# anihcsam/OpenGaussian

Measured on AMD Instinct MI355X. Metric: fwd+bwd Mpix/s at 1080p, 1M Gaussians (RGB+6-D ins_feat); k-means it/s, higher is better.
Workload: dtype f32; 1 GPU; S1M-1080p RGB(SH3)+depth+alpha (all grads) + 6-ch ins_feat (grad to ins_feat) fwd+bwd, ONE fused 9-channel pass; gaussians=1000000, width=1920, height=1080, views_cycled=8, parallelism=single

## Files before the change

include/ogs_raster.h:

```cpp
#ifndef OGS_RASTER_H
#define OGS_RASTER_H

#include <stddef.h>
#include <stdint.h>

#ifdef __cplusplus
extern "C" {
#endif

#define OGS_OK 0
#define OGS_ERR_INVALID_ARG (-1)
#define OGS_ERR_HIP (-2)
#define OGS_ERR_UNSUPPORTED (-3)
#define OGS_ERR_SCRATCH_TOO_SMALL (-4)
#define OGS_ERR_DEVICE (-5)

#define OGS_TILE 16
#define OGS_MAX_CHANNELS 12

typedef struct OgsRasterFwdArgs {
    int32_t P;
    int32_t W, H;
    int32_t C;
    int32_t sh_degree;
    int32_t sh_coeffs;
    float tanfovx, tanfovy;
    float scale_modifier;
    int32_t prefiltered;
    int32_t debug;
    const float* bg;
    const float* means3D;
    const float* colors_precomp;
    const float* shs;
    const float* opacities;
    const float* scales;
    const float* rotations;
    const float* cov3D_precomp;
    const float* viewmatrix;
    const float* projmatrix;
    const float* campos;
    float* out_color;
    float* out_depth;
    float* out_alpha;
    int32_t* radii;
    void* geom_buffer;
    void* geom_tmp;
    void* image_buffer;
    uint32_t* point_list;
    void* binning_tmp;
    void* sorted_rec;
    void* quad_list;
    const int32_t* group_ids;
    int32_t num_groups;
    int32_t full_binning;
} OgsRasterFwdArgs;

typedef struct OgsRasterBwdArgs {
    int32_t P, W, H, C, sh_degree, sh_coeffs;
    float tanfovx, tanfovy, scale_modifier;
    int32_t debug;
    int32_t num_rendered;
    int32_t geom_channels;
    const float* bg;
    const float* means3D;
    const float* colors_precomp;
    const float* shs;
    const float* opacities;
    const float* scales;
    const float* rotations;
    const float* cov3D_precomp;
    const float* viewmatrix;
    const float* projmatrix;
    const float* campos;
    const int32_t* radii;
    const float* out_alpha;
    const float* dL_dcolor;
    const float* dL_ddepth;
    const float* dL_dalpha;
    const void* geom_buffer;
    const void* image_buffer;
    const uint32_t* point_list;
    const void* sorted_rec;
    const void* quad_list;
    void* bwd_tmp;
    float* dL_dmeans2D;
    float* dL_dcolors;
    float* dL_dopacity;
    float* dL_dmeans3D;
    float* dL_dcov3D;
    float* dL_dsh;
    float* dL_dscales;
    float* dL_drotations;
    int32_t num_groups;
    float* dL_dsh_rgb;
} OgsRasterBwdArgs;

int ogs_version(void);
const char* ogs_last_error(void);

int ogs_check_async_status(void);

size_t ogs_raster_geom_bytes(int32_t P, int32_t C);
size_t ogs_raster_geom_tmp_bytes(int32_t P);
size_t ogs_raster_image_bytes(int32_t W, int32_t H);
size_t ogs_raster_image_bytes_grouped(int32_t W, int32_t H, int32_t num_groups);
size_t ogs_raster_binning_tmp_bytes(int64_t num_rendered, int32_t W, int32_t H);
size_t ogs_raster_backward_tmp_bytes(int32_t P);
size_t ogs_raster_sorted_bytes(int64_t num_rendered, int32_t C);
size_t ogs_raster_quad_list_bytes(int64_t num_rendered);

int ogs_raster_forward_geometry(const OgsRasterFwdArgs* args, void* stream, int64_t* num_rendered_host);

int ogs_raster_forward_render(const OgsRasterFwdArgs* args, int64_t num_rendered, void* stream);

int ogs_raster_read_num_rendered_async(const OgsRasterFwdArgs* args, void* stream, uint32_t* host_pinned);
int ogs_raster_forward_render_deferred(const OgsRasterFwdArgs* args, int64_t capacity, void* stream);

size_t ogs_raster_tiny_max_points(void);
int ogs_raster_forward_tiny(const OgsRasterFwdArgs* args, void* stream);

size_t ogs_raster_tile_sort_capacity(int32_t level);

int ogs_raster_forward_reblend(const OgsRasterFwdArgs* args, void* stream);

int ogs_raster_compact_kept(int32_t W, int32_t H, int32_t C, const void* image_buffer, const void* sorted_rec,
                            const void* quad_list, void* new_image_buffer, void* new_sorted_rec, void* new_quad_list,
                            void* stream);

typedef struct OgsGroupStatsArgs {
    const int32_t* labels;
    int32_t num_labels;
    float alpha_threshold;
    float* max_alpha;
    int64_t* count;
    float* feat_sum;
    void* stats_tmp;
} OgsGroupStatsArgs;

size_t ogs_raster_stats_image_bytes(int32_t W, int32_t H, int32_t num_groups);
size_t ogs_raster_stats_tmp_bytes(int32_t num_groups, int32_t num_labels, int32_t C);
int ogs_raster_forward_group_stats(const OgsRasterFwdArgs* args, const OgsGroupStatsArgs* stats, int64_t num_rendered,
                                   void* stream);

int ogs_raster_backward(const OgsRasterBwdArgs* args, void* stream);

int ogs_mark_visible(int32_t P, const float* means3D, const float* viewmatrix, const float* projmatrix,
                     uint8_t* present, void* stream);

int ogs_sh_grad_from_views(int32_t P, int32_t V, int32_t sh_degree, int32_t sh_coeffs, const float* means3D,
                           const float* campos, const float* dL_drgb, float* dL_dsh, void* stream);

int ogs_raster_export_binning(const OgsRasterFwdArgs* args, int64_t num_rendered, uint64_t* keys_out,
                              uint32_t* ranges_out, uint32_t* n_contrib_out, void* stream);

int ogs_prof_enable(int on);
int ogs_prof_filter(const char* prefix);
int ogs_prof_collect(char* buf, size_t n);

int ogs_selftest_wave_fold16(const float* in, float* out, void* stream);
int ogs_selftest_tile_order(const uint32_t* ranges, int64_t vtiles, uint32_t* order, void* stream);
size_t ogs_selftest_radix_tmp_bytes(int64_t n);
int ogs_selftest_radix_sort(uint32_t* keys0, uint32_t* vals0, uint32_t* keys1, uint32_t* vals1, int64_t n, int32_t key_bits,
                            int32_t variant, int32_t items, const uint32_t* n_dev, void* tmp, int32_t* result_buffer,
                            void* stream);

#ifdef __cplusplus
}
#endif
#endif
```

opengaussian_amd/_lib.py:

```python
from __future__ import annotations

import ctypes as C
import os

_HERE = os.path.dirname(os.path.abspath(__file__))
LIB_PATH = os.environ.get("OGS_LIB_PATH") or os.path.join(_HERE, "lib", "libogs_hip.so")

_f32p = C.POINTER(C.c_float)
_vp = C.c_void_p


class OgsRasterFwdArgs(C.Structure):
    _fields_ = [
        ("P", C.c_int32), ("W", C.c_int32), ("H", C.c_int32), ("C", C.c_int32),
        ("sh_degree", C.c_int32), ("sh_coeffs", C.c_int32),
        ("tanfovx", C.c_float), ("tanfovy", C.c_float), ("scale_modifier", C.c_float),
        ("prefiltered", C.c_int32), ("debug", C.c_int32),
        ("bg", _vp), ("means3D", _vp), ("colors_precomp", _vp), ("shs", _vp), ("opacities", _vp),
        ("scales", _vp), ("rotations", _vp), ("cov3D_precomp", _vp),
        ("viewmatrix", _vp), ("projmatrix", _vp), ("campos", _vp),
        ("out_color", _vp), ("out_depth", _vp), ("out_alpha", _vp), ("radii", _vp),
        ("geom_buffer", _vp), ("geom_tmp", _vp), ("image_buffer", _vp), ("point_list", _vp),
        ("binning_tmp", _vp), ("sorted_rec", _vp), ("quad_list", _vp), ("group_ids", _vp), ("num_groups", C.c_int32),
        ("full_binning", C.c_int32),
    ]


class OgsRasterBwdArgs(C.Structure):
    _fields_ = [
        ("P", C.c_int32), ("W", C.c_int32), ("H", C.c_int32), ("C", C.c_int32),
        ("sh_degree", C.c_int32), ("sh_coeffs", C.c_int32),
        ("tanfovx", C.c_float), ("tanfovy", C.c_float), ("scale_modifier", C.c_float),
        ("debug", C.c_int32), ("num_rendered", C.c_int32), ("geom_channels", C.c_int32),
        ("bg", _vp), ("means3D", _vp), ("colors_precomp", _vp), ("shs", _vp), ("opacities", _vp),
        ("scales", _vp), ("rotations", _vp), ("cov3D_precomp", _vp),
        ("viewmatrix", _vp), ("projmatrix", _vp), ("campos", _vp),
        ("radii", _vp), ("out_alpha", _vp), ("dL_dcolor", _vp), ("dL_ddepth", _vp), ("dL_dalpha", _vp),
        ("geom_buffer", _vp), ("image_buffer", _vp), ("point_list", _vp), ("sorted_rec", _vp), ("quad_list", _vp), ("bwd_tmp", _vp),
        ("dL_dmeans2D", _vp), ("dL_dcolors", _vp), ("dL_dopacity", _vp), ("dL_dmeans3D", _vp),
        ("dL_dcov3D", _vp), ("dL_dsh", _vp), ("dL_dscales", _vp), ("dL_drotations", _vp), ("num_groups", C.c_int32), ("dL_dsh_rgb", _vp),
    ]


class OgsAdamTensor(C.Structure):
    _fields_ = [("param", _vp), ("grad", _vp), ("exp_avg", _vp), ("exp_avg_sq", _vp), ("numel", C.c_int64),
                ("lr", C.c_double), ("step", C.c_int64)]


class OgsRowTensor(C.Structure):
    _fields_ = [("src", _vp), ("dst", _vp), ("width", C.c_int32), ("zero_new", C.c_int32)]


class OgsDensifyArgs(C.Structure):
    _fields_ = [("N", C.c_int32), ("grad_accum", _vp), ("denom", _vp), ("scaling", _vp), ("opacity", _vp),
                ("max_grad", C.c_float), ("min_opacity", C.c_float), ("extent", C.c_float), ("percent_dense", C.c_float),
                ("prune_world_size", C.c_int32)]


class OgsGroupStatsArgs(C.Structure):
    _fields_ = [("labels", _vp), ("num_labels", C.c_int32), ("alpha_threshold", C.c_float), ("max_alpha", _vp),
                ("count", _vp), ("feat_sum", _vp), ("stats_tmp", _vp)]


SIGNATURES = {
    "ogs_version": (C.c_int, []),
    "ogs_last_error": (C.c_char_p, []),
    "ogs_raster_geom_bytes": (C.c_size_t, [C.c_int32, C.c_int32]),
    "ogs_raster_geom_tmp_bytes": (C.c_size_t, [C.c_int32]),
    "ogs_raster_image_bytes": (C.c_size_t, [C.c_int32, C.c_int32]),
    "ogs_raster_image_bytes_grouped": (C.c_size_t, [C.c_int32, C.c_int32, C.c_int32]),
    "ogs_raster_binning_tmp_bytes": (C.c_size_t, [C.c_int64, C.c_int32, C.c_int32]),
    "ogs_raster_backward_tmp_bytes": (C.c_size_t, [C.c_int32]),
    "ogs_raster_sorted_bytes": (C.c_size_t, [C.c_int64, C.c_int32]),
    "ogs_raster_quad_list_bytes": (C.c_size_t, [C.c_int64]),
    "ogs_raster_forward_geometry": (C.c_int, [C.POINTER(OgsRasterFwdArgs), _vp, C.POINTER(C.c_int64)]),
    "ogs_raster_forward_render": (C.c_int, [C.POINTER(OgsRasterFwdArgs), C.c_int64, _vp]),
    "ogs_raster_read_num_rendered_async": (C.c_int, [C.POINTER(OgsRasterFwdArgs), _vp, _vp]),
    "ogs_raster_forward_render_deferred": (C.c_int, [C.POINTER(OgsRasterFwdArgs), C.c_int64, _vp]),
    "ogs_raster_stats_image_bytes": (C.c_size_t, [C.c_int32, C.c_int32, C.c_int32]),
    "ogs_raster_stats_tmp_bytes": (C.c_size_t, [C.c_int32, C.c_int32, C.c_int32]),
    "ogs_raster_forward_group_stats": (C.c_int, [C.POINTER(OgsRasterFwdArgs), C.POINTER(OgsGroupStatsArgs), C.c_int64, _vp]),
    "ogs_raster_backward": (C.c_int, [C.POINTER(OgsRasterBwdArgs), _vp]),
    "ogs_raster_tiny_max_points": (C.c_size_t, []),
    "ogs_raster_tile_sort_capacity": (C.c_size_t, [C.c_int32]),
    "ogs_raster_forward_tiny": (C.c_int, [C.POINTER(OgsRasterFwdArgs), _vp]),
    "ogs_raster_forward_reblend": (C.c_int, [C.POINTER(OgsRasterFwdArgs), _vp]),
    "ogs_raster_compact_kept": (C.c_int, [C.c_int32, C.c_int32, C.c_int32, _vp, _vp, _vp, _vp, _vp, _vp, _vp]),
    "ogs_mark_visible": (C.c_int, [C.c_int32, _vp, _vp, _vp, _vp, _vp]),
    "ogs_sh_grad_from_views": (C.c_int, [C.c_int32, C.c_int32, C.c_int32, C.c_int32, _vp, _vp, _vp, _vp, _vp]),
    "ogs_raster_export_binning": (C.c_int, [C.POINTER(OgsRasterFwdArgs), C.c_int64, _vp, _vp, _vp, _vp]),
    "ogs_selftest_wave_fold16": (C.c_int, [_vp, _vp, _vp]),
    "ogs_selftest_tile_order": (C.c_int, [_vp, C.c_int64, _vp, _vp]),
    "ogs_selftest_radix_tmp_bytes": (C.c_size_t, [C.c_int64]),
    "ogs_selftest_radix_sort": (C.c_int, [_vp, _vp, _vp, _vp, C.c_int64, C.c_int32, C.c_int32, C.c_int32, _vp, _vp, _vp, _vp]),
    "ogs_check_async_status": (C.c_int, []),
    "ogs_prof_enable": (C.c_int, [C.c_int]),
    "ogs_prof_filter": (C.c_int, [C.c_char_p]),
    "ogs_prof_collect": (C.c_int, [C.c_char_p, C.c_size_t]),
    "ogs_kmeans_tmp_bytes": (C.c_size_t, [C.c_int64, C.c_int32, C.c_int32]),
    "ogs_kmeans_lloyd": (C.c_int, [_vp, C.c_int64, C.c_int32, _vp, C.c_int32, C.c_int32, C.c_int32, C.c_int32,
                                   _vp, C.c_int64, _vp, _vp]),
    "ogs_kmeans_assign": (C.c_int, [_vp, C.c_int64, C.c_int32, _vp, C.c_int32, _vp, C.c_int64, _vp]),
    "ogs_mask_feature_sums": (C.c_int, [_vp, _vp, _vp, C.c_int32, C.c_int32, C.c_int64, C.c_int32, _vp, _vp]),
    "ogs_mask_feature_sqdev": (C.c_int, [_vp, _vp, _vp, _vp, C.c_int32, C.c_int32, C.c_int64, _vp, _vp]),
    "ogs_mask_feature_sums_backward": (C.c_int, [_vp, _vp, _vp, _vp, _vp, C.c_int32, C.c_int32, C.c_int64, _vp, _vp, _vp]),
    "ogs_mask_cohesion": (C.c_int, [_vp, _vp, _vp, C.c_int32, C.c_int32, C.c_int64, _vp, _vp]),
    "ogs_mask_cohesion_backward": (C.c_int, [_vp, _vp, _vp, _vp, C.c_int32, C.c_int32, C.c_int64, _vp, _vp, _vp]),
    "ogs_label_feature_sums": (C.c_int, [_vp, _vp, _vp, C.c_int32, C.c_int32, C.c_int64, C.c_int32, _vp, _vp]),
    "ogs_label_feature_sqdev": (C.c_int, [_vp, _vp, _vp, _vp, C.c_int32, C.c_int32, C.c_int64, _vp, _vp]),
    "ogs_label_feature_sums_backward": (C.c_int, [_vp, _vp, _vp, _vp, _vp, C.c_int32, C.c_int32, C.c_int64, _vp, _vp, _vp]),
    "ogs_label_cohesion": (C.c_int, [_vp, _vp, _vp, C.c_int32, C.c_int32, C.c_int64, _vp, _vp]),
    "ogs_label_cohesion_backward": (C.c_int, [_vp, _vp, _vp, _vp, C.c_int32, C.c_int32, C.c_int64, _vp, _vp, _vp]),
    "ogs_separation_loss": (C.c_int, [_vp, C.c_int32, C.c_int32, C.c_int32, _vp, _vp, _vp, _vp]),
    "ogs_adam_step": (C.c_int, [C.POINTER(OgsAdamTensor), C.c_int32, C.c_double, C.c_double, C.c_double, _vp]),
    "ogs_rows_gather": (C.c_int, [C.POINTER(OgsRowTensor), C.c_int32, _vp, _vp, C.c_int64, _vp]),
    "ogs_densify_tmp_bytes": (C.c_size_t, [C.c_int32]),
    "ogs_densify_plan": (C.c_int, [C.POINTER(OgsDensifyArgs), _vp, C.POINTER(C.c_uint32), _vp]),
    "ogs_densify_map": (C.c_int, [C.c_int32, _vp, _vp, _vp, _vp, _vp]),
    "ogs_densify_split_children": (C.c_int, [C.c_int64, _vp, _vp, _vp, _vp, _vp, _vp, _vp, _vp, _vp, _vp]),
    "ogs_densify_stats": (C.c_int, [C.c_int32, _vp, C.c_int32, _vp, _vp, _vp, _vp, _vp, _vp]),
    "ogs_kmeans_accumulate": (C.c_int, [_vp, C.c_int64, C.c_int32, _vp, C.c_int32, C.c_int32, _vp, _vp, _vp]),
    "ogs_kmeans_update": (C.c_int, [_vp, C.c_int32, C.c_int32, C.c_int32, _vp, _vp, _vp]),
    "ogs_kmeans_gather": (C.c_int, [_vp, _vp, C.c_int64, C.c_int32, C.c_int32, _vp, _vp]),
    "ogs_refine_wave_table_capacity": (C.c_size_t, []),
    "ogs_refine_wave_max_pixels": (C.c_size_t, []),
    "ogs_refine_block_scratch_words": (C.c_size_t, [C.c_int32]),
    "ogs_refine_visibility": (C.c_int, [C.c_int32, _vp, _vp, _vp, _vp, C.c_int32, C.c_int32, C.c_float, C.c_float, _vp,
                                        C.c_float, C.c_float, _vp, _vp]),
    "ogs_refine_footprint_labels": (C.c_int, [C.c_int32, _vp, _vp, C.c_int32, C.c_int32, C.c_int32, _vp, C.c_int32, _vp, _vp,
                                              _vp]),
    "ogs_refine_footprint_labels_block": (C.c_int, [C.c_int32, _vp, _vp, C.c_int32, C.c_int32, C.c_int32, _vp, C.c_int32, _vp,
                                                    _vp, _vp, _vp]),
    "ogs_refine_vote": (C.c_int, [C.c_int64, C.c_int32, _vp, _vp, _vp]),
    "ogs_refine_expand": (C.c_int, [C.c_int32, _vp, _vp, _vp, _vp, C.c_int32, C.c_int32, C.c_int32, _vp, C.c_int32, _vp, _vp,
                                    C.c_int32, _vp]),
    "ogs_refine_finalize": (C.c_int, [C.c_int64, C.c_int32, _vp, _vp, _vp, C.c_int32, C.c_float, _vp, _vp]),
    "ogs_loss_photometric_tmp_bytes": (C.c_size_t, [C.c_int32, C.c_int32, C.c_int32]),
    "ogs_loss_photometric_forward": (C.c_int, [_vp, _vp, C.c_int32, C.c_int32, C.c_int32, C.c_float, _vp, _vp, _vp]),
    "ogs_loss_photometric_backward": (C.c_int, [_vp, _vp, _vp, _vp, _vp, C.c_float, C.c_int32, C.c_int32, C.c_int32, _vp,
                                                _vp]),
    "ogs_loss_masked_tmp_bytes": (C.c_size_t, []),
    "ogs_loss_masked_forward": (C.c_int, [_vp, _vp, _vp, _vp, C.c_int32, C.c_int32, C.c_int32, C.c_int64, _vp, _vp, _vp]),
    "ogs_loss_masked_backward": (C.c_int, [_vp, _vp, _vp, _vp, C.c_int32, C.c_int32, C.c_int32, C.c_int64, _vp, _vp, _vp,
                                           _vp]),
    "ogs_knn_tile_points": (C.c_size_t, []),
    "ogs_knn_group_ksum": (C.c_int, [C.c_int64, _vp, C.c_int32, _vp, _vp, _vp, _vp, _vp, _vp]),
}

_lib = None


class OgsError(RuntimeError):
    pass


def lib() -> C.CDLL:
    global _lib
    if _lib is None:
        if not os.path.exists(LIB_PATH):
            raise OgsError(f"{LIB_PATH} not found -- build it with `python -m opengaussian_amd.build` "
                           "(the product path has no CPU fallback)")
        l = C.CDLL(LIB_PATH)
        for name, (res, args) in SIGNATURES.items():
            fn = getattr(l, name)
            fn.restype = res
            fn.argtypes = args
        _lib = l
    return _lib


def check(rc: int, what: str):
    if rc != 0:
        raise OgsError(f"{what} failed (code {rc}): {lib().ogs_last_error().decode()}")


def prof_filter(prefix: str):
    check(lib().ogs_prof_filter(prefix.encode()), "ogs_prof_filter")


def prof_enable(mode):
    check(lib().ogs_prof_enable(int(mode)), "ogs_prof_enable")


def prof_collect() -> dict:
    import json
    buf = C.create_string_buffer(1 << 16)
    check(lib().ogs_prof_collect(buf, len(buf)), "ogs_prof_collect")
    return json.loads(buf.value.decode())


def ptr(t):
    return None if t is None else t.data_ptr()
```

opengaussian_amd/csrc/blend_fwd.hip:

```cpp
#include "ogs_common.h"

namespace ogs {

namespace {

constexpr float kAlphaMin = 1.0f / 255.0f;
typedef float v2f __attribute__((ext_vector_type(2)));

__device__ __forceinline__ uint64_t shfl_up_u64(uint64_t v, int d) {
    const uint32_t lo = __shfl_up((uint32_t)v, d, kWave), hi = __shfl_up((uint32_t)(v >> 32), d, kWave);
    return ((uint64_t)hi << 32) | lo;
}


template <int C>
struct RowRec {
    static constexpr int NV4 = stream_vec4(C);
    float4 v[NV4];
    __device__ __forceinline__ void load_lds(const float4* __restrict__ p) {
#pragma unroll
        for (int k = 0; k < NV4; ++k) v[k] = p[k];
    }
    __device__ __forceinline__ float at(int i) const {
        const float4 q = v[i >> 2];
        return (i & 3) == 0 ? q.x : (i & 3) == 1 ? q.y : (i & 3) == 2 ? q.z : q.w;
    }
    __device__ __forceinline__ float feat(int c) const { return at(8 + c); }
};

constexpr int kRowSlots = 65;
constexpr int kRowListLen = 72;
template <int C>
struct RowsLds {
    float4 s_rec[kBlock / kWave][kRowSlots * stream_vec4(C)];
    uint32_t s_list[kBlock / kWave][4][kRowListLen];
};

template <int C, int RF = -1>
__device__ __forceinline__ void blend_rows_tile(
    const uint2 range, int n, int n_kept, const float* __restrict__ stream,
    const uint32_t* __restrict__ quad_list, int W, int H, int gx, int img, int timg, const float* __restrict__ bg, float* __restrict__ out_color,
    float* __restrict__ out_depth, float* __restrict__ out_alpha, uint32_t* __restrict__ n_contrib,
    float* __restrict__ final_T, int pf_lines, RowsLds<C>& lds, const float* __restrict__ feats = nullptr) {
    constexpr int NV4 = stream_vec4(C);
    constexpr int RS = NV4 * 4;
    constexpr int kListLen = kRowListLen;
    auto& s_rec = lds.s_rec;
    auto& s_list = lds.s_list;
    const int tx = timg % gx, ty = timg / gx;
    const int tid = threadIdx.x, lane = tid & 63, wave = __builtin_amdgcn_readfirstlane(tid >> 6);
    const int row = lane >> 4, l16 = lane & 15;
    const int qx0 = tx * kTile + (wave & 1) * 8, qy0 = ty * kTile + (wave >> 1) * 8;
    const int px = qx0 + 4 * (row & 1) + (l16 & 3);
    const int py = qy0 + 4 * (row >> 1) + (l16 >> 2);
    const bool inside = px < W && py < H;
    const float fy = (float)py;

    const int n_tile = (int)(range.y - range.x);
    const float* __restrict__ tb = stream + (size_t)range.x * RS;
    const uint32_t* __restrict__ qi = quad_list + ((size_t)range.x * 5 + (size_t)wave * n_tile);
    const uint32_t lim = n_kept > 0 ? (uint32_t)n_kept - 1u : 0u;
    RecordPrefetch pf;
    pf.issue(tb, n_kept, RS, tid, pf_lines);

    float4* __restrict__ recs = s_rec[wave];
    uint32_t* __restrict__ mylist = s_list[wave][row];
    if (lane == 0) {
#pragma unroll
        for (int k = 0; k < NV4; ++k) recs[64 * NV4 + k] = float4{0.f, 0.f, 0.f, 0.f};
        recs[64 * NV4 + 1] = float4{0.f, -1.f, 0.f, 0.f};
    }
    float fxe = inside ? (float)px : kFar;
    float T = 1.0f;
    constexpr int NPF = (C + 2) / 2;
    v2f accp[NPF];
#pragma unroll
    for (int k = 0; k < NPF; ++k) accp[k] = (v2f){0.f, 0.f};
    float wacc = 0.f;
    uint32_t last = 0;
    bool all_done = false;

    constexpr uint32_t kNoEntry = 0xFFFFFFFFu;
    uint32_t last_e = kNoEntry;
    auto consume = [&](const RowRec<C>& rec, uint32_t entry) {
        const v2f d = (v2f){rec.at(0), rec.at(1)} - (v2f){fxe, fy};
        const v2f m = (v2f){rec.at(2), rec.at(3)} * d;
        const float u = fmaf(rec.at(4), d.y, m.x);
        const float power = fmaf(m.y, d.y, u * d.x);
        const float h = rec.at(5);
        const bool cand = fabsf(power + h) <= h;
        if (__ballot(cand) != 0ull) {
            const float araw = fminf(0.99f, rec.at(6) * __expf(power));
            const bool act = cand && araw >= kAlphaMin;
            const float alpha = act ? araw : 0.f;
            const float test_T = T * (1.0f - alpha);
            const bool stop = test_T < 0.0001f;
            const float w = stop ? 0.f : alpha * T;
            const v2f w2 = {w, w};
#pragma unroll
            for (int k = 0; k < NPF; ++k)
                accp[k] = __builtin_elementwise_fma((v2f){rec.feat(2 * k), rec.feat(2 * k + 1)}, w2, accp[k]);
            wacc += w;
            T = stop ? T : test_T;
            last_e = (act && !stop) ? entry : last_e;
            fxe = stop ? kFar : fxe;
            if (__ballot(stop) != 0ull) all_done = __ballot(fxe < kFarTest) == 0ull;
        }
    };

    const float bx0 = (float)(qx0 + 4 * 0), by0 = (float)qy0;
    for (int c0 = 0; c0 < n && !all_done; c0 += kWave) {
        const int cnt = min(kWave, n - c0);
        const bool have = lane < cnt;
        const uint32_t ridx = have ? min(qi[c0 + lane], lim) : 0u;
        const float4* __restrict__ rp = reinterpret_cast<const float4*>(tb + (size_t)ridx * RS);
        float4 r[NV4];
#pragma unroll
        for (int k = 0; k < NV4; ++k) r[k] = rp[k];
        if constexpr (RF >= 0) {
            constexpr int E = C - RF;
            const float* __restrict__ fp = feats + (size_t)__float_as_uint(r[1].w) * E;
            float fv[E];
#pragma unroll
            for (int k = 0; k < E; ++k) fv[k] = fp[k];
            float* rf = reinterpret_cast<float*>(r);
#pragma unroll
            for (int k = 0; k < E; ++k) rf[8 + RF + k] = fv[k];
        }
#pragma unroll
        for (int k = 0; k < NV4; ++k) recs[lane * NV4 + k] = r[k];
        bool reach[4];
        {
            const float gxp = r[0].x, gyp = r[0].y;
            const float A = -2.f * r[0].z, B = -r[1].x, Cc = -2.f * r[0].w, thr = -2.f * r[1].y;
            const float nbA = -B / A, nbC = -B / Cc;
#pragma unroll
            for (int b = 0; b < 4; ++b) {
                const float ox = bx0 + 4.f * (float)(b & 1), oy = by0 + 4.f * (float)(b >> 1);
                const float m = max_power_in_box(A, B, Cc, nbA, nbC, gxp - ox - 3.f, gxp - ox, gyp - oy - 3.f, gyp - oy);
                reach[b] = have && m >= thr;
            }
        }
        constexpr uint32_t kDummy = (64u << 16) | (64u * NV4 * 16u);
#pragma unroll
        for (int b = 0; b < 4; ++b) s_list[wave][b][lane] = kDummy;
        if (lane < kListLen - kWave) {
#pragma unroll
            for (int b = 0; b < 4; ++b) s_list[wave][b][kWave + lane] = kDummy;
        }
        int maxlen = 0;
#pragma unroll
        for (int b = 0; b < 4; ++b) {
            const uint64_t mask = __ballot(reach[b]);
            const int pos = (int)__builtin_amdgcn_mbcnt_hi((uint32_t)(mask >> 32), __builtin_amdgcn_mbcnt_lo((uint32_t)mask, 0u));
            if (reach[b]) s_list[wave][b][pos] = ((uint32_t)lane << 16) | ((uint32_t)lane * NV4 * 16u);
            maxlen = max(maxlen, (int)__popcll(mask));
        }
        __builtin_amdgcn_fence(__ATOMIC_RELEASE, "wavefront");
        __builtin_amdgcn_wave_barrier();
        RowRec<C> ra, rb;
        auto rec_of = [&](uint32_t e) {
            return reinterpret_cast<const float4*>(reinterpret_cast<const char*>(recs) + (e & 0xFFFFu));
        };
        uint32_t e0 = mylist[0], e1 = mylist[1];
        ra.load_lds(rec_of(e0));
        for (int t = 0; t < maxlen && !all_done; t += 2) {
            const uint32_t e2 = mylist[t + 2], e3 = mylist[t + 3];
            rb.load_lds(rec_of(e1));
            consume(ra, e0);
            ra.load_lds(rec_of(e2));
            if (t + 1 < maxlen) consume(rb, e1);
            e0 = e2; e1 = e3;
        }
        if (last_e != kNoEntry) last = (uint32_t)c0 + (last_e >> 16) + 1u;
        last_e = kNoEntry;
        __builtin_amdgcn_wave_barrier();
    }

    if (inside) {
        const size_t plane = (size_t)W * H;
        const size_t pix = (size_t)img * plane + (size_t)py * W + px;
        float* oc = out_color + (size_t)img * (C - 1) * plane;
#pragma unroll
        for (int c = 0; c < C; ++c) oc[c * plane + pix] = ((c & 1) ? accp[c / 2].y : accp[c / 2].x) + T * bg[c];
        out_depth[pix] = (C & 1) ? accp[C / 2].y : accp[C / 2].x;
        out_alpha[pix] = wacc;
        n_contrib[pix] = last;
        final_T[pix] = T;
    }
    pf.retire(n_contrib, W);
}

template <int C, int RF = -1>
__global__ __launch_bounds__(kBlock) void blend_forward_rows_kernel(
    const uint2* __restrict__ ranges, const uint32_t* __restrict__ qcount, const float* __restrict__ stream,
    const uint32_t* __restrict__ quad_list, int W, int H, int gx, int tiles, const float* __restrict__ bg, float* __restrict__ out_color,
    float* __restrict__ out_depth, float* __restrict__ out_alpha, uint32_t* __restrict__ n_contrib,
    float* __restrict__ final_T, int pf_lines, const uint32_t* __restrict__ tile_order, const float* __restrict__ feats) {
    __shared__ RowsLds<C> lds;
    const int tile = tile_order ? (int)tile_order[blockIdx.x] : (int)blockIdx.x;
    const int img = tile / tiles, timg = tile - img * tiles;
    const int wave = __builtin_amdgcn_readfirstlane((int)threadIdx.x >> 6);
    blend_rows_tile<C, RF>(ranges[tile], (int)qcount[tile * 5 + wave], (int)qcount[tile * 5 + 4], stream, quad_list, W, H, gx, img, timg,
                           bg, out_color, out_depth, out_alpha, n_contrib, final_T, pf_lines, lds, feats);
}

template <int C>
struct ChunkLds {
    static constexpr int SV = stream_vec4(C);
    uint64_t wave_tot[kBlock / kWave];
    uint32_t done[kBlock / kWave];
    float4 s_rec[(kBlock + 1) * SV];
    uint32_t s_list[kBlock / kWave][4][kRowListLen];
    uint8_t s_qnew[4][kBlock];
};

struct GroupStatsOut {
    const int32_t* labels;
    int32_t L;
    float thr;
    uint32_t* max_alpha;
    unsigned long long* count;
    unsigned long long* fsum;
};

constexpr float kFixedScale = 4294967296.0f;

__device__ __forceinline__ unsigned long long shfl_xor_u64(unsigned long long v, int m) {
    const uint32_t lo = __shfl_xor((uint32_t)v, m, kWave), hi = __shfl_xor((uint32_t)(v >> 32), m, kWave);
    return ((unsigned long long)hi << 32) | lo;
}

template <int C>
__device__ __forceinline__ void group_stats_epilogue(const GroupStatsOut& st, float* __restrict__ s_buf, int img, int W, int pix,
                                                     float alpha, const float (&colour)[C]) {
    float* s_val = s_buf;
    float* s_alpha = s_buf + C * kBlock;
    int* s_key = reinterpret_cast<int*>(s_buf + (C + 1) * kBlock);
    const int tid = threadIdx.x, lane = tid & 63;
    int key = -1;
    if (pix >= 0 && alpha > st.thr) {
        const int l = st.labels[pix];
        key = (l >= 0 && l < st.L) ? l : st.L;
    }
    s_key[tid] = key;
    s_alpha[tid] = pix >= 0 ? alpha : 0.f;
#pragma unroll
    for (int c = 0; c < C; ++c) s_val[c * kBlock + tid] = colour[c];
    lds_barrier();
    if (tid >= kWave) return;
    int k[kBlock / kWave];
    float m = 0.f;
#pragma unroll
    for (int j = 0; j < kBlock / kWave; ++j) {
        k[j] = s_key[lane + kWave * j];
        m = fmaxf(m, s_alpha[lane + kWave * j]);
    }
#pragma unroll
    for (int off = kWave / 2; off > 0; off >>= 1) m = fmaxf(m, __shfl_xor(m, off, kWave));
    if (lane == 0 && m > 0.f) atomicMax(st.max_alpha + img, __float_as_uint(m));
    const size_t row0 = (size_t)img * (size_t)(st.L + 1);
    for (;;) {
        int cand = -1;
#pragma unroll
        for (int j = kBlock / kWave - 1; j >= 0; --j) cand = k[j] >= 0 ? k[j] : cand;
        const uint64_t pending = __ballot(cand >= 0);
        if (pending == 0ull) break;
        const int K = __shfl(cand, __ffsll((unsigned long long)pending) - 1, kWave);
        unsigned long long cnt = 0, sum[C];
#pragma unroll
        for (int c = 0; c < C; ++c) sum[c] = 0ull;
#pragma unroll
        for (int j = 0; j < kBlock / kWave; ++j) {
            if (k[j] == K) {
                ++cnt;
#pragma unroll
                for (int c = 0; c < C; ++c) sum[c] += (unsigned long long)__float2ll_rn(s_val[c * kBlock + lane + kWave * j] * kFixedScale);
                k[j] = -1;
            }
        }
#pragma unroll
        for (int off = kWave / 2; off > 0; off >>= 1) {
            cnt += (unsigned long long)__shfl_xor((uint32_t)cnt, off, kWave);
#pragma unroll
            for (int c = 0; c < C; ++c) sum[c] += shfl_xor_u64(sum[c], off);
        }
        if (lane == 0) {
            const size_t r = row0 + (size_t)K;
            atomicAdd(st.count + r, cnt);
#pragma unroll
            for (int c = 0; c < C; ++c) atomicAdd(st.fsum + r * C + c, sum[c]);
        }
    }
}

__global__ __launch_bounds__(256) void group_stats_finish_kernel(const long long* __restrict__ fsum, float* __restrict__ out, size_t n) {
    const size_t i = (size_t)blockIdx.x * 256 + threadIdx.x;
    if (i < n) out[i] = (float)((double)fsum[i] * (1.0 / 4294967296.0));
}

template <int C, bool STATS = false>
__global__ __launch_bounds__(kBlock) __attribute__((amdgpu_waves_per_eu(6, 8)))
void pack_blend_chunked_kernel(
    const uint2* __restrict__ ranges, const uint32_t* __restrict__ point_list, const float4* __restrict__ rec,
    float4* __restrict__ stream, uint32_t* __restrict__ quad_list, uint32_t* __restrict__ qcount, int W, int H, int gx, int tiles,
    const float* __restrict__ bg, float* __restrict__ out_color, float* __restrict__ out_depth, float* __restrict__ out_alpha,
    uint32_t* __restrict__ n_contrib, float* __restrict__ final_T, const uint32_t* __restrict__ tile_order,
    GroupStatsOut st = GroupStatsOut{}) {
    constexpr int NV = rec_vec4(C);
    constexpr int SV = stream_vec4(C);
    constexpr int kListLen = kRowListLen;
    __shared__ ChunkLds<C> lds;
    const int tile = tile_order ? (int)tile_order[blockIdx.x] : (int)blockIdx.x;
    const int img = tile / tiles, timg = tile - img * tiles;
    const uint2 range = ranges[tile];
    const int n = (int)(range.y - range.x);
    const int tx = timg % gx, ty = timg / gx;
    const int tid = threadIdx.x, lane = tid & 63, wave = __builtin_amdgcn_readfirstlane(tid >> 6);
    const float X0 = (float)(tx * kTile), Y0 = (float)(ty * kTile);
    const int row = lane >> 4, l16 = lane & 15;
    const int qx0 = tx * kTile + (wave & 1) * 8, qy0 = ty * kTile + (wave >> 1) * 8;
    const int px = qx0 + 4 * (row & 1) + (l16 & 3);
    const int py = qy0 + 4 * (row >> 1) + (l16 >> 2);
    const bool inside = px < W && py < H;
    const float fy = (float)py;
    float fxe = inside ? (float)px : kFar;
    float T = 1.0f;
    constexpr int NPF = (C + 2) / 2;
    v2f accp[NPF];
#pragma unroll
    for (int k = 0; k < NPF; ++k) accp[k] = (v2f){0.f, 0.f};
    float wacc = 0.f;
    uint32_t last = 0;
    uint64_t alive = __ballot(inside);

    const float4* __restrict__ recs = lds.s_rec;
    uint32_t* __restrict__ mylist = lds.s_list[wave][row];
    if (tid == 0) {
#pragma unroll
        for (int k = 0; k < SV; ++k) lds.s_rec[kBlock * SV + k] = float4{0.f, 0.f, 0.f, 0.f};
        lds.s_rec[kBlock * SV + 1] = float4{0.f, -1.f, 0.f, 0.f};
    }

    constexpr uint32_t kNoEntry = 0xFFFFFFFFu;
    uint32_t last_e = kNoEntry;
    auto consume = [&](const RowRec<C>& r, uint32_t entry) {
        const v2f d = (v2f){r.at(0), r.at(1)} - (v2f){fxe, fy};
        const v2f m = (v2f){r.at(2), r.at(3)} * d;
        const float u = fmaf(r.at(4), d.y, m.x);
        const float power = fmaf(m.y, d.y, u * d.x);
        const float h = r.at(5);
        const bool cand = fabsf(power + h) <= h;
        if (__ballot(cand) != 0ull) {
            const float araw = fminf(0.99f, r.at(6) * __expf(power));
            const bool act = cand && araw >= kAlphaMin;
            const float alpha = act ? araw : 0.f;
            const float test_T = T * (1.0f - alpha);
            const bool stop = test_T < 0.0001f;
            float w = alpha * T;
            bool contributes = act;
            if (__ballot(stop) != 0ull) {
                w = stop ? 0.f : w;
                T = stop ? T : test_T;
                fxe = stop ? kFar : fxe;
                alive = __ballot(fxe < kFarTest);
                contributes = act && !stop;
            } else {
                T = test_T;
            }
            const v2f w2 = {w, w};
#pragma unroll
            for (int k = 0; k < NPF; ++k)
                accp[k] = __builtin_elementwise_fma((v2f){r.feat(2 * k), r.feat(2 * k + 1)}, w2, accp[k]);
            wacc += w;
            last_e = contributes ? entry : last_e;
        }
    };

    uint32_t running[5];
#pragma unroll
    for (int q = 0; q < 5; ++q) running[q] = 0u;
    const float bx0 = (float)qx0, by0 = (float)qy0;

    for (int base = 0; base < n; base += kBlock) {
        const int i = base + tid;
        uint32_t mask = 0;
        float4 a = make_float4(0, 0, 0, 0), b = a;
        float h = 0.f;
        uint32_t gid_of_thread = 0;
        const uint32_t sv = i < n ? point_list[range.x + i] : 0u;
        if (sv >> kReachBit) {
            const uint32_t gid = sv & kGidMask;
            gid_of_thread = gid;
            const float4* src = rec + (size_t)gid * NV;
            a = src[0]; b = src[1];
            h = 0.5f * (__logf(255.0f * b.w) + kThrMargin);
            const float thr = -2.0f * h;
            const float nbA = -b.y / b.x, nbC = -b.y / b.z;
#pragma unroll
            for (int q = 0; q < 4; ++q) {
                const float qx = X0 + (float)((q & 1) * 8), qy = Y0 + (float)((q >> 1) * 8);
                const float m = max_power_in_box(b.x, b.y, b.z, nbA, nbC, a.x - qx - 7.f, a.x - qx, a.y - qy - 7.f, a.y - qy);
                if (m >= thr) mask |= 1u << q;
            }
        }
        const uint64_t mine = (uint64_t)(mask & 1u) | ((uint64_t)((mask >> 1) & 1u) << 12) |
                              ((uint64_t)((mask >> 2) & 1u) << 24) | ((uint64_t)((mask >> 3) & 1u) << 36) |
                              ((uint64_t)(mask != 0u ? 1u : 0u) << 48);
        uint64_t inc = mine;
#pragma unroll
        for (int d = 1; d < kWave; d <<= 1) {
            const uint64_t t = shfl_up_u64(inc, d);
            if (lane >= d) inc += t;
        }
        if (lane == kWave - 1) lds.wave_tot[wave] = inc;
        lds_barrier();
        uint64_t before = 0, total = 0;
#pragma unroll
        for (int w = 0; w < kBlock / kWave; ++w) {
            const uint64_t t = lds.wave_tot[w];
            if (w < wave) before += t;
            total += t;
        }
        const uint64_t pos = before + inc - mine;
        if (mask) {
            const uint32_t c_loc = (uint32_t)(pos >> 48) & 0xFFFu;
            const uint32_t c_idx = running[4] + c_loc;
            float4* dst = lds.s_rec + c_loc * SV;
            dst[0] = make_float4(a.x, a.y, -0.5f * b.x, -0.5f * b.z);
            dst[1] = make_float4(-b.y, h, b.w, __uint_as_float(gid_of_thread));
            const float4* src = rec + (size_t)gid_of_thread * NV;
            float f[(SV - 2) * 4];
#pragma unroll
            for (int k = 0; k < (SV - 2) * 4; ++k) f[k] = 0.f;
#pragma unroll
            for (int v = 0; v < NV - 2; ++v) {
                const float4 t = src[2 + v];
                f[4 * v] = t.x; f[4 * v + 1] = t.y; f[4 * v + 2] = t.z; f[4 * v + 3] = t.w;
            }
            f[C] = a.z;
#pragma unroll
            for (int v = 0; v < SV - 2; ++v) dst[2 + v] = make_float4(f[4 * v], f[4 * v + 1], f[4 * v + 2], f[4 * v + 3]);
#pragma unroll
            for (int q = 0; q < 4; ++q) {
                if (mask & (1u << q)) {
                    const uint32_t pq = (uint32_t)(pos >> (12 * q)) & 0xFFFu;
                    if constexpr (!STATS) quad_list[(size_t)range.x * 5 + (size_t)q * n + running[q] + pq] = c_idx;
                    lds.s_qnew[q][pq] = (uint8_t)c_loc;
                }
            }
            if constexpr (!STATS) quad_list[(size_t)range.x * 5 + (size_t)4 * n + c_idx] = (uint32_t)i;
        }
        lds_barrier();
        if constexpr (!STATS) {
            const int kept4 = (int)((uint32_t)(total >> 48) & 0xFFFu) * SV;
            float4* __restrict__ out = stream + ((size_t)range.x + (size_t)running[4]) * SV;
            for (int e = tid; e < kept4; e += kBlock) out[e] = lds.s_rec[e];
        }
        const int cnt_q = (int)((uint32_t)(total >> (12 * wave)) & 0xFFFu);
        const uint32_t j0 = wave == 0 ? running[0] : wave == 1 ? running[1] : wave == 2 ? running[2] : running[3];
        for (int c0 = 0; c0 < cnt_q && alive != 0ull; c0 += kWave) {
            const int cnt = min(kWave, cnt_q - c0);
            const bool have = lane < cnt;
            const uint32_t cl = have ? (uint32_t)lds.s_qnew[wave][c0 + lane] : (uint32_t)kBlock;
            const float4 r0 = recs[cl * SV], r1 = recs[cl * SV + 1];
            bool reach[4];
            {
                const float gxp = r0.x, gyp = r0.y;
                const float A = -2.f * r0.z, B = -r1.x, Cc = -2.f * r0.w, thr = -2.f * r1.y;
                const float nbA = -B / A, nbC = -B / Cc;
#pragma unroll
                for (int bb = 0; bb < 4; ++bb) {
                    const float ox = bx0 + 4.f * (float)(bb & 1), oy = by0 + 4.f * (float)(bb >> 1);
                    const float m = max_power_in_box(A, B, Cc, nbA, nbC, gxp - ox - 3.f, gxp - ox, gyp - oy - 3.f, gyp - oy);
                    reach[bb] = have && m >= thr;
                }
            }
            constexpr uint32_t kDummy = (64u << 16) | ((uint32_t)kBlock * SV * 16u);
#pragma unroll
            for (int bb = 0; bb < 4; ++bb) lds.s_list[wave][bb][lane] = kDummy;
            if (lane < kListLen - kWave) {
#pragma unroll
                for (int bb = 0; bb < 4; ++bb) lds.s_list[wave][bb][kWave + lane] = kDummy;
            }
            int maxlen = 0;
#pragma unroll
            for (int bb = 0; bb < 4; ++bb) {
                const uint64_t m64 = __ballot(reach[bb]);
                const int p = (int)__builtin_amdgcn_mbcnt_hi((uint32_t)(m64 >> 32), __builtin_amdgcn_mbcnt_lo((uint32_t)m64, 0u));
                if (reach[bb]) lds.s_list[wave][bb][p] = ((uint32_t)lane << 16) | (cl * SV * 16u);
                maxlen = max(maxlen, (int)__popcll(m64));
            }
            __builtin_amdgcn_fence(__ATOMIC_RELEASE, "wavefront");
            __builtin_amdgcn_wave_barrier();
            RowRec<C> ra, rb;
            auto rec_of = [&](uint32_t e) {
                return reinterpret_cast<const float4*>(reinterpret_cast<const char*>(recs) + (e & 0xFFFFu));
            };
            uint32_t e0 = mylist[0], e1 = mylist[1];
            ra.load_lds(rec_of(e0));
            const uint32_t jbase = j0 + (uint32_t)c0 + 1u;
            for (int t = 0; t < maxlen && alive != 0ull; t += 2) {
                const uint32_t e2 = mylist[t + 2], e3 = mylist[t + 3];
                rb.load_lds(rec_of(e1));
                consume(ra, e0);
                ra.load_lds(rec_of(e2));
                if (t + 1 < maxlen) consume(rb, e1);
                e0 = e2; e1 = e3;
            }
            if (last_e != kNoEntry) last = jbase + (last_e >> 16);
            last_e = kNoEntry;
            __builtin_amdgcn_wave_barrier();
        }
#pragma unroll
        for (int q = 0; q < 5; ++q) running[q] += (uint32_t)(total >> (12 * q)) & 0xFFFu;
        if (lane == 0) lds.done[wave] = alive == 0ull ? 1u : 0u;
        lds_barrier();
        if ((lds.done[0] & lds.done[1] & lds.done[2] & lds.done[3]) != 0u) break;
    }
    if constexpr (STATS) {
        float colour[C];
#pragma unroll
        for (int c = 0; c < C; ++c) colour[c] = ((c & 1) ? accp[c / 2].y : accp[c / 2].x) + T * bg[c];
        group_stats_epilogue<C>(st, reinterpret_cast<float*>(lds.s_rec), img, W, inside ? py * W + px : -1, wacc, colour);
    } else {
        if (tid == 0) {
#pragma unroll
            for (int q = 0; q < 5; ++q) qcount[tile * 5 + q] = running[q];
        }
        if (inside) {
            const size_t plane = (size_t)W * H;
            const size_t pix = (size_t)img * plane + (size_t)py * W + px;
            float* oc = out_color + (size_t)img * (C - 1) * plane;
#pragma unroll
            for (int c = 0; c < C; ++c) oc[c * plane + pix] = ((c & 1) ? accp[c / 2].y : accp[c / 2].x) + T * bg[c];
            out_depth[pix] = (C & 1) ? accp[C / 2].y : accp[C / 2].x;
            out_alpha[pix] = wacc;
            n_contrib[pix] = last;
            final_T[pix] = T;
        }
    }
}

template <int C>
__global__ __launch_bounds__(kBlock) void export_n_contrib_kernel(const uint2* __restrict__ ranges,
                                                                  const uint32_t* __restrict__ point_list,
                                                                  const uint32_t* __restrict__ quad_list, int W, int H,
                                                                  int gx, int tiles, const uint32_t* __restrict__ n_contrib,
                                                                  uint32_t* __restrict__ out) {
    const int tile = blockIdx.x;
    const int img = tile / tiles, timg = tile - img * tiles;
    const int tx = timg % gx, ty = timg / gx;
    const int tid = threadIdx.x, lane = tid & 63, wave = tid >> 6;
    const int px = tx * kTile + (wave & 1) * 8 + (lane & 7);
    const int py = ty * kTile + (wave >> 1) * 8 + (lane >> 3);
    if (px >= W || py >= H) return;
    const uint2 range = ranges[tile];
    const int n_tile = (int)(range.y - range.x);
    n_contrib += (size_t)img * W * H;
    out += (size_t)img * W * H;
    const uint32_t last = n_contrib[(size_t)py * W + px];
    uint32_t res = 0;
    if (last > 0) {
        const uint32_t c_idx = quad_list[(size_t)range.x * 5 + (size_t)wave * n_tile + (last - 1)];
        res = quad_list[(size_t)range.x * 5 + (size_t)4 * n_tile + c_idx] + 1u;
    }
    out[(size_t)py * W + px] = res;
}

template <int C>
__global__ __launch_bounds__(kBlock) void tiny_blend_kernel(int P, const uint32_t* __restrict__ order,
                                                            const float4* __restrict__ rec, int W, int H, int gx,
                                                            const float* __restrict__ bg, float* __restrict__ out_color,
                                                            float* __restrict__ out_depth, float* __restrict__ out_alpha) {
    constexpr int NV = rec_vec4(C);
    constexpr int RS = 8 + (C + 1 + 3) / 4 * 4;
    static_assert(kTinyMaxP == kBlock, "one staging round");
    __shared__ float s_rec[kTinyMaxP * RS];
    __shared__ uint32_t s_wave_cnt[kBlock / kWave];
    const int tile = blockIdx.x;
    const int tx = tile % gx, ty = tile / gx;
    const int tid = threadIdx.x, lane = tid & 63, wave = tid >> 6;
    const int gy = (H + kTile - 1) / kTile;

    bool keep = false;
    float4 a = make_float4(0, 0, 0, 0), b = a;
    uint32_t gid = 0;
    if (tid < P) {
        gid = order[tid];
        const float4* src = rec + (size_t)gid * NV;
        a = src[0]; b = src[1];
        const int radius = __float_as_int(a.w);
        if (radius > 0) {
            const float rf = (float)radius;
            auto tr = [](float v) -> int {
                if (!(fabsf(v) < 3.0e38f)) v = 0.f;
                v = fminf(fmaxf(v, -2.0e9f), 2.0e9f);
                return (int)v;
            };
            const int rminx = min(gx, max(0, tr((a.x - rf) / (float)kTile)));
            const int rminy = min(gy, max(0, tr((a.y - rf) / (float)kTile)));
            const int rmaxx = min(gx, max(0, tr((a.x + rf + (float)kTile - 1.0f) / (float)kTile)));
            const int rmaxy = min(gy, max(0, tr((a.y + rf + (float)kTile - 1.0f) / (float)kTile)));
            keep = tx >= rminx && tx < rmaxx && ty >= rminy && ty < rmaxy;
        }
    }
    const uint64_t bal = __ballot(keep);
    if (lane == 0) s_wave_cnt[wave] = (uint32_t)__popcll(bal);
    __syncthreads();
    uint32_t before = 0, n = 0;
#pragma unroll
    for (int w = 0; w < kBlock / kWave; ++w) {
        const uint32_t c = s_wave_cnt[w];
        if (w < wave) before += c;
        n += c;
    }
    if (keep) {
        const uint32_t pos = before + (uint32_t)__popcll(bal & ((1ull << lane) - 1ull));
        float* dst = s_rec + pos * RS;
        dst[0] = a.x; dst[1] = a.y; dst[2] = -0.5f * b.x; dst[3] = -b.y; dst[4] = -0.5f * b.z;
        dst[5] = 0.5f * (__logf(255.0f * b.w) + kThrMargin);
        dst[6] = b.w; dst[7] = __uint_as_float(gid);
        const float4* src = rec + (size_t)gid * NV;
        float f[(NV - 2) * 4 + 4];
#pragma unroll
        for (int v = 0; v < NV - 2; ++v) {
            const float4 t = src[2 + v];
            f[4 * v] = t.x; f[4 * v + 1] = t.y; f[4 * v + 2] = t.z; f[4 * v + 3] = t.w;
        }
#pragma unroll
        for (int c = 0; c < C; ++c) dst[8 + c] = f[c];
        dst[8 + C] = a.z;
    }
    __syncthreads();

    const int px = tx * kTile + (wave & 1) * 8 + (lane & 7);
    const int py = ty * kTile + (wave >> 1) * 8 + (lane >> 3);
    const bool inside = px < W && py < H;
    const float fx = (float)px, fy = (float)py;
    float T = 1.0f, wacc = 0.f;
    float acc[C + 1];
#pragma unroll
    for (int c = 0; c <= C; ++c) acc[c] = 0.f;
    bool done = !inside;
    for (uint32_t j = 0; j < n; ++j) {
        if (__ballot(!done) == 0ull) break;
        const float* r = s_rec + j * RS;
        const float dx = r[0] - fx, dy = r[1] - fy;
        const float power = blend_power(r[2], r[3], r[4], dx, dy);
        const bool cand = !done && fabsf(power + r[5]) <= r[5];
        if (cand) {
            float alpha = fminf(0.99f, r[6] * __expf(power));
            alpha = alpha >= kAlphaMin ? alpha : 0.f;
            const float test_T = T * (1.0f - alpha);
            const bool stop = test_T < 0.0001f;
            const float w = stop ? 0.f : alpha * T;
#pragma unroll
            for (int c = 0; c <= C; ++c) acc[c] = fmaf(r[8 + c], w, acc[c]);
            wacc += w;
            T = stop ? T : test_T;
            done = stop;
        }
    }
    if (inside) {
        const size_t plane = (size_t)W * H;
        const size_t pix = (size_t)py * W + px;
#pragma unroll
        for (int c = 0; c < C; ++c) out_color[c * plane + pix] = acc[c] + T * bg[c];
        out_depth[pix] = acc[C];
        out_alpha[pix] = wacc;
    }
}

template <int C>
int tiny_c(const OgsRasterFwdArgs& a, const GeomState& gs, const uint32_t* order, hipStream_t s) {
    const int gx = (a.W + kTile - 1) / kTile, gy = (a.H + kTile - 1) / kTile;
    OGS_LAUNCH(tiny_blend_kernel<C>, dim3((unsigned)(gx * gy)), dim3(kBlock), 0, s, a.P, order, (const float4*)gs.rec, a.W, a.H,
               gx, a.bg, a.out_color, a.out_depth, a.out_alpha);
    OGS_LAUNCH_CHECK(a.debug, s);
    return OGS_OK;
}


constexpr int kOrderThreads = 1024;
constexpr int64_t kOrderMaxTiles = 1 << 16;
__device__ __forceinline__ uint32_t work_class(uint32_t n) {
    if (n < 8u) return 255u - n;
    const uint32_t e = 31u - (uint32_t)__builtin_clz(n);
    const uint32_t v = e * 8u + ((n >> (e - 3u)) & 7u);
    return 255u - min(v, 255u);
}
__device__ __forceinline__ uint32_t class_counter_add(uint32_t* bins, uint32_t cls, bool valid, int lane) {
    uint32_t pos = 0u;
    uint64_t todo = __ballot(valid);
    while (todo != 0ull) {
        const int leader = __ffsll((unsigned long long)todo) - 1;
        const uint32_t c0 = (uint32_t)__shfl((int)cls, leader, kWave);
        const uint64_t same = __ballot(valid && cls == c0) & todo;
        uint32_t base = 0u;
        if (lane == leader) base = atomicAdd(&bins[c0], (uint32_t)__popcll(same));
        base = (uint32_t)__shfl((int)base, leader, kWave);
        if ((same >> lane) & 1ull) pos = base + (uint32_t)__popcll(same & ((1ull << lane) - 1ull));
        todo &= ~same;
    }
    return pos;
}
__global__ __launch_bounds__(kOrderThreads) void tile_order_kernel(const uint2* __restrict__ ranges, uint32_t vtiles,
                                                                   uint32_t* __restrict__ order) {
    __shared__ uint32_t bins[256];
    __shared__ uint32_t wave_max[kOrderThreads / kWave], wave_sum[kOrderThreads / kWave];
    const uint32_t tid = threadIdx.x;
    uint32_t my_max = 0u, my_sum = 0u;
    for (uint32_t t0 = 0; t0 < vtiles; t0 += 8u * kOrderThreads) {
        uint2 r[8];
#pragma unroll
        for (int k = 0; k < 8; ++k) {
            const uint32_t t = t0 + (uint32_t)k * kOrderThreads + tid;
            r[k] = t < vtiles ? ranges[t] : make_uint2(0u, 0u);
        }
#pragma unroll
        for (int k = 0; k < 8; ++k) { my_max = max(my_max, r[k].y - r[k].x); my_sum += r[k].y - r[k].x; }
    }
#pragma unroll
    for (int d = 32; d >= 1; d >>= 1) {
        my_max = max(my_max, (uint32_t)__shfl_xor((int)my_max, d, kWave));
        my_sum += (uint32_t)__shfl_xor((int)my_sum, d, kWave);
    }
    if ((tid & 63u) == 0u) { wave_max[tid >> 6] = my_max; wave_sum[tid >> 6] = my_sum; }
    if (tid < 256u) bins[tid] = 0u;
    __syncthreads();
    uint32_t longest = 0u;
    unsigned long long total = 0ull;
#pragma unroll
    for (int w = 0; w < kOrderThreads / kWave; ++w) { longest = max(longest, wave_max[w]); total += wave_sum[w]; }
    if ((unsigned long long)longest * vtiles <= 2ull * total) {
        for (uint32_t t = tid; t < vtiles; t += kOrderThreads) order[t] = t;
        return;
    }
    for (uint32_t t0 = 0; t0 < vtiles; t0 += kOrderThreads) {
        const uint32_t t = t0 + tid;
        const bool valid = t < vtiles;
        const uint2 r = valid ? ranges[t] : make_uint2(0u, 0u);
        (void)class_counter_add(bins, work_class(r.y - r.x), valid, (int)(tid & 63u));
    }
    __syncthreads();
    if (tid < 64u) {
        uint32_t c[4], sum = 0u;
#pragma unroll
        for (int k = 0; k < 4; ++k) { c[k] = bins[tid * 4u + k]; sum += c[k]; }
        uint32_t incl = sum;
#pragma unroll
        for (int d = 1; d < 64; d <<= 1) {
            const uint32_t o = __shfl_up(incl, d, kWave);
            if ((int)tid >= d) incl += o;
        }
        uint32_t base = incl - sum;
#pragma unroll
        for (int k = 0; k < 4; ++k) { bins[tid * 4u + k] = base; base += c[k]; }
    }
    __syncthreads();
    for (uint32_t t0 = 0; t0 < vtiles; t0 += kOrderThreads) {
        const uint32_t t = t0 + tid;
        const bool valid = t < vtiles;
        const uint2 r = valid ? ranges[t] : make_uint2(0u, 0u);
        const uint32_t pos = class_counter_add(bins, work_class(r.y - r.x), valid, (int)(tid & 63u));
        if (valid) order[pos] = t;
    }
}

template <int C>
int launch_c(const OgsRasterFwdArgs& a, const GeomState& gs, const ImageState& is, int64_t D, hipStream_t s, bool order_ready) {
    const int gx = (a.W + kTile - 1) / kTile, gy = (a.H + kTile - 1) / kTile;
    const int tiles = gx * gy;
    const unsigned vtiles = (unsigned)tiles * (unsigned)num_groups_of(a.num_groups);
    if (D > 0) {
        const uint32_t* order = order_ready ? tile_order_of(is, vtiles, a.P) : launch_tile_order(is, vtiles, a.P, s, a.debug);
        static constexpr const char* const kChunked[4] = {"pack_blend_chunked_kernel<3>", "pack_blend_chunked_kernel<6>",
                                                          "pack_blend_chunked_kernel<9>", "pack_blend_chunked_kernel<12>"};
        OGS_LAUNCH_NAMED(chan_name<C>(kChunked), pack_blend_chunked_kernel<C>, dim3(vtiles), dim3(kBlock), 0, s,
                         (const uint2*)is.ranges, (const uint32_t*)a.point_list, (const float4*)gs.rec, stream_base<C>(a.sorted_rec),
                         quad_base(a.quad_list), is.qcount, a.W, a.H, gx, tiles, a.bg, a.out_color, a.out_depth, a.out_alpha,
                         is.n_contrib, is.final_T, order);
        OGS_LAUNCH_CHECK(a.debug, s);
        return OGS_OK;
    }
    OGS_HIP_CHECK(hipMemsetAsync(is.qcount, 0, (size_t)vtiles * 5 * sizeof(uint32_t), s));
    static constexpr const char* const kRows[4] = {"blend_forward_rows_kernel<3>", "blend_forward_rows_kernel<6>",
                                                   "blend_forward_rows_kernel<9>", "blend_forward_rows_kernel<12>"};
    OGS_LAUNCH_NAMED(chan_name<C>(kRows), blend_forward_rows_kernel<C>, dim3(vtiles), dim3(kBlock), 0, s,
                     (const uint2*)is.ranges, (const uint32_t*)is.qcount, (const float*)stream_base<C>(a.sorted_rec),
                     (const uint32_t*)quad_base(a.quad_list), a.W, a.H, gx, tiles, a.bg, a.out_color, a.out_depth,
                     a.out_alpha, is.n_contrib, is.final_T, blend_prefetch_lines(), (const uint32_t*)nullptr, (const float*)nullptr);
    OGS_LAUNCH_CHECK(a.debug, s);
    return OGS_OK;
}

template <int C>
int stats_c(const OgsRasterFwdArgs& a, const OgsGroupStatsArgs& sa, const GeomState& gs, const ImageState& is, hipStream_t s,
            bool order_ready) {
    const int gx = (a.W + kTile - 1) / kTile, gy = (a.H + kTile - 1) / kTile;
    const int tiles = gx * gy;
    const int G = num_groups_of(a.num_groups);
    const unsigned vtiles = (unsigned)tiles * (unsigned)G;
    const size_t rows = (size_t)G * (size_t)(sa.num_labels + 1);
    long long* fixed = static_cast<long long*>(sa.stats_tmp);
    OGS_HIP_CHECK(hipMemsetAsync(sa.max_alpha, 0, (size_t)G * sizeof(float), s));
    OGS_HIP_CHECK(hipMemsetAsync(sa.count, 0, rows * sizeof(int64_t), s));
    OGS_HIP_CHECK(hipMemsetAsync(fixed, 0, rows * C * sizeof(long long), s));
    const uint32_t* order = order_ready ? tile_order_of(is, vtiles, a.P) : launch_tile_order(is, vtiles, a.P, s, a.debug);
    GroupStatsOut st;
    st.labels = sa.labels;
    st.L = sa.num_labels;
    st.thr = sa.alpha_threshold;
    st.max_alpha = reinterpret_cast<uint32_t*>(sa.max_alpha);
    st.count = reinterpret_cast<unsigned long long*>(sa.count);
    st.fsum = reinterpret_cast<unsigned long long*>(fixed);
    static constexpr const char* const kStats[4] = {"pack_blend_chunked_kernel<3, stats>", "pack_blend_chunked_kernel<6, stats>",
                                                    "pack_blend_chunked_kernel<9, stats>", "pack_blend_chunked_kernel<12, stats>"};
    OGS_LAUNCH_NAMED(chan_name<C>(kStats), (pack_blend_chunked_kernel<C, true>), dim3(vtiles), dim3(kBlock), 0, s,
                     (const uint2*)is.ranges, (const uint32_t*)a.point_list, (const float4*)gs.rec, (float4*)nullptr,
                     (uint32_t*)nullptr, (uint32_t*)nullptr, a.W, a.H, gx, tiles, a.bg, (float*)nullptr, (float*)nullptr,
                     (float*)nullptr, (uint32_t*)nullptr, (float*)nullptr, order, st);
    OGS_LAUNCH_CHECK(a.debug, s);
    const size_t n = rows * C;
    OGS_LAUNCH(group_stats_finish_kernel, dim3((unsigned)((n + 255) / 256)), dim3(256), 0, s, (const long long*)fixed,
               sa.feat_sum, n);
    OGS_LAUNCH_CHECK(a.debug, s);
    return OGS_OK;
}

template <int C>
int reblend_c(const OgsRasterFwdArgs& a, const ImageState& is, hipStream_t s) {
    const int gx = (a.W + kTile - 1) / kTile, gy = (a.H + kTile - 1) / kTile;
    const int tiles = gx * gy;
    const unsigned vtiles = (unsigned)tiles;
    const uint32_t* order = tile_order_of(is, vtiles, a.P);
    static constexpr const char* const kRows[4] = {"blend_forward_rows_kernel<3, refresh>", "blend_forward_rows_kernel<6, refresh>",
                                                   "blend_forward_rows_kernel<9, refresh>", "blend_forward_rows_kernel<12, refresh>"};
    const float* stream = reinterpret_cast<const float*>(stream_base<C>(a.sorted_rec));
#define OGS_REBLEND(RFV)                                                                                                    \
    OGS_LAUNCH_NAMED(chan_name<C>(kRows), (blend_forward_rows_kernel<C, RFV>), dim3(vtiles), dim3(kBlock), 0, s,           \
                     (const uint2*)is.ranges, (const uint32_t*)is.qcount, stream, (const uint32_t*)quad_base(a.quad_list), a.W,  \
                     a.H, gx, tiles, a.bg, a.out_color, a.out_depth, a.out_alpha, is.n_contrib, is.final_T,                  \
                     blend_prefetch_lines(), order, a.colors_precomp)
    if (a.sh_coeffs != 0) {
        if constexpr (C > 3) {
            OGS_REBLEND(3);
        } else {
            set_error("forward_reblend: a 3-channel SH pass has no channel to replace");
            return OGS_ERR_INVALID_ARG;
        }
    } else {
        OGS_REBLEND(0);
    }
#undef OGS_REBLEND
    OGS_LAUNCH_CHECK(a.debug, s);
    return OGS_OK;
}

template <int C>
__global__ __launch_bounds__(kBlock) void compact_kept_kernel(const uint2* __restrict__ old_ranges, const uint2* __restrict__ new_ranges,
                                                              const uint32_t* __restrict__ qcount, const float4* __restrict__ old_rec,
                                                              const uint32_t* __restrict__ old_quad, float4* __restrict__ new_rec,
                                                              uint32_t* __restrict__ new_quad) {
    constexpr int SV = stream_vec4(C);
    const int tile = blockIdx.x;
    const uint2 ro = old_ranges[tile], rn = new_ranges[tile];
    const uint32_t n_old = ro.y - ro.x, k = qcount[tile * 5 + 4];
    const float4* __restrict__ src = old_rec + (size_t)ro.x * SV;
    float4* __restrict__ dst = new_rec + (size_t)rn.x * SV;
    for (uint32_t e = threadIdx.x; e < k * SV; e += kBlock) dst[e] = src[e];
#pragma unroll
    for (int q = 0; q < 4; ++q) {
        const uint32_t nq = qcount[tile * 5 + q];
        const uint32_t* __restrict__ qs = old_quad + ((size_t)ro.x * 5 + (size_t)q * n_old);
        uint32_t* __restrict__ qd = new_quad + ((size_t)rn.x * 5 + (size_t)q * k);
        for (uint32_t e = threadIdx.x; e < nq; e += kBlock) qd[e] = qs[e];
    }
}

template <int C>
int compact_c(int W, int H, const ImageState& is_old, const ImageState& is_new, const void* old_rec, const void* old_quad,
              void* new_rec, void* new_quad, hipStream_t s) {
    const int gx = (W + kTile - 1) / kTile, gy = (H + kTile - 1) / kTile;
    OGS_LAUNCH(compact_kept_kernel<C>, dim3((unsigned)(gx * gy)), dim3(kBlock), 0, s, (const uint2*)is_old.ranges,
               (const uint2*)is_new.ranges, (const uint32_t*)is_old.qcount, (const float4*)stream_base<C>(const_cast<void*>(old_rec)),
               (const uint32_t*)quad_base(const_cast<void*>(old_quad)), stream_base<C>(new_rec), quad_base(new_quad));
    OGS_LAUNCH_CHECK(0, s);
    return OGS_OK;
}

template <int C>
int export_c(const OgsRasterFwdArgs& a, const ImageState& is, uint32_t* out, hipStream_t s) {
    const int gx = (a.W + kTile - 1) / kTile, gy = (a.H + kTile - 1) / kTile;
    OGS_LAUNCH(export_n_contrib_kernel<C>, dim3((unsigned)(gx * gy) * (unsigned)num_groups_of(a.num_groups)), dim3(kBlock), 0,
               s, (const uint2*)is.ranges, (const uint32_t*)a.point_list, (const uint32_t*)quad_base(a.quad_list), a.W,
               a.H, gx, gx * gy, (const uint32_t*)is.n_contrib, out);
    OGS_LAUNCH_CHECK(0, s);
    return OGS_OK;
}

}

static bool tile_order_enabled() {
    static const bool v = [] { const char* e = getenv("OGS_TILE_ORDER"); return !(e && atoi(e) == 0); }();
    return v;
}
const uint32_t* tile_order_of(const ImageState& is, int64_t vtiles, int P) {
    return (tile_order_enabled() && vtiles > 1 && vtiles <= kOrderMaxTiles && (int64_t)P >= 4 * vtiles) ? is.tile_order : nullptr;
}
const uint32_t* launch_tile_order(const ImageState& is, int64_t vtiles, int P, hipStream_t s, int debug) {
    const uint32_t* order = tile_order_of(is, vtiles, P);
    if (!order) return nullptr;
    OGS_LAUNCH(tile_order_kernel, dim3(1), dim3(kOrderThreads), 0, s, (const uint2*)is.ranges, (uint32_t)vtiles, is.tile_order);
    if (debug) (void)hipStreamSynchronize(s);
    return order;
}

int launch_tile_order_test(const uint32_t* ranges, int64_t vtiles, uint32_t* order, hipStream_t s) {
    if (vtiles > kOrderMaxTiles) { set_error("selftest: more than %lld tiles", (long long)kOrderMaxTiles); return OGS_ERR_UNSUPPORTED; }
    OGS_LAUNCH(tile_order_kernel, dim3(1), dim3(kOrderThreads), 0, s, (const uint2*)ranges, (uint32_t)vtiles, order);
    OGS_LAUNCH_CHECK(1, s);
    return OGS_OK;
}

int launch_blend_forward(const OgsRasterFwdArgs& a, const GeomState& gs, const ImageState& is, int64_t D,
                         hipStream_t s, bool order_ready) {
    switch (a.C) {
        case 3: return launch_c<3>(a, gs, is, D, s, order_ready);
        case 6: return launch_c<6>(a, gs, is, D, s, order_ready);
        case 9: return launch_c<9>(a, gs, is, D, s, order_ready);
        case 12: return launch_c<12>(a, gs, is, D, s, order_ready);
        default: set_error("unsupported channel count C=%d", a.C); return OGS_ERR_UNSUPPORTED;
    }
}

int launch_group_stats(const OgsRasterFwdArgs& a, const OgsGroupStatsArgs& st, const GeomState& gs, const ImageState& is,
                       hipStream_t s, bool order_ready) {
    switch (a.C) {
        case 3: return stats_c<3>(a, st, gs, is, s, order_ready);
        case 6: return stats_c<6>(a, st, gs, is, s, order_ready);
        case 9: return stats_c<9>(a, st, gs, is, s, order_ready);
        case 12: return stats_c<12>(a, st, gs, is, s, order_ready);
        default: set_error("unsupported channel count C=%d", a.C); return OGS_ERR_UNSUPPORTED;
    }
}

int launch_compact_kept(int W, int H, int C, const ImageState& is_old, const ImageState& is_new, const void* old_rec,
                        const void* old_quad, void* new_rec, void* new_quad, hipStream_t s) {
    switch (C) {
        case 3: return compact_c<3>(W, H, is_old, is_new, old_rec, old_quad, new_rec, new_quad, s);
        case 6: return compact_c<6>(W, H, is_old, is_new, old_rec, old_quad, new_rec, new_quad, s);
        case 9: return compact_c<9>(W, H, is_old, is_new, old_rec, old_quad, new_rec, new_quad, s);
        case 12: return compact_c<12>(W, H, is_old, is_new, old_rec, old_quad, new_rec, new_quad, s);
        default: set_error("unsupported channel count C=%d", C); return OGS_ERR_UNSUPPORTED;
    }
}

int launch_reblend(const OgsRasterFwdArgs& a, const ImageState& is, hipStream_t s) {
    switch (a.C) {
        case 3: return reblend_c<3>(a, is, s);
        case 6: return reblend_c<6>(a, is, s);
        case 9: return reblend_c<9>(a, is, s);
        case 12: return reblend_c<12>(a, is, s);
        default: set_error("unsupported channel count C=%d", a.C); return OGS_ERR_UNSUPPORTED;
    }
}

int launch_tiny_blend(const OgsRasterFwdArgs& a, const GeomState& gs, const uint32_t* order, hipStream_t s) {
    switch (a.C) {
        case 3: return tiny_c<3>(a, gs, order, s);
        case 6: return tiny_c<6>(a, gs, order, s);
        case 9: return tiny_c<9>(a, gs, order, s);
        case 12: return tiny_c<12>(a, gs, order, s);
        default: set_error("unsupported channel count C=%d", a.C); return OGS_ERR_UNSUPPORTED;
    }
}

int launch_export_n_contrib(const OgsRasterFwdArgs& a, const ImageState& is, uint32_t* out, hipStream_t s) {
    switch (a.C) {
        case 3: return export_c<3>(a, is, out, s);
        case 6: return export_c<6>(a, is, out, s);
        case 9: return export_c<9>(a, is, out, s);
        case 12: return export_c<12>(a, is, out, s);
        default: set_error("unsupported channel count C=%d", a.C); return OGS_ERR_UNSUPPORTED;
    }
}

}
```

opengaussian_amd/csrc/capi.hip:

```cpp
#include <stdarg.h>
#include <stdlib.h>
#include <string.h>

#include <map>
#include <mutex>
#include <string>
#include <vector>

#include "ogs_common.h"

namespace ogs {

static thread_local char g_err[512] = "";

void set_error(const char* fmt, ...) {
    va_list ap;
    va_start(ap, fmt);
    vsnprintf(g_err, sizeof(g_err), fmt, ap);
    va_end(ap);
}

namespace {
struct ProfRec { const char* name; hipEvent_t start, stop; };
int g_prof_mode = 0;
char g_prof_prefix[64] = "blend_";
std::vector<ProfRec> g_prof;
std::vector<hipEvent_t> g_event_pool;
std::mutex g_prof_mu;
hipEvent_t take_event() {
    if (!g_event_pool.empty()) { hipEvent_t e = g_event_pool.back(); g_event_pool.pop_back(); return e; }
    hipEvent_t e = nullptr;
    (void)hipEventCreate(&e);
    return e;
}
}

ProfScope::ProfScope(const char* n, hipStream_t s) : name(n), stream(s), slot(-1) {
    if (g_prof_mode == 0) return;
    if (g_prof_mode == 2 && strncmp(n, g_prof_prefix, strlen(g_prof_prefix)) != 0) return;
    std::lock_guard<std::mutex> lk(g_prof_mu);
    ProfRec r{n, take_event(), take_event()};
    (void)hipEventRecord(r.start, s);
    g_prof.push_back(r);
    slot = (int)g_prof.size() - 1;
}
ProfScope::~ProfScope() {
    if (slot < 0) return;
    std::lock_guard<std::mutex> lk(g_prof_mu);
    (void)hipEventRecord(g_prof[slot].stop, stream);
}

namespace {
uint32_t* g_async_status = nullptr;
std::mutex g_async_mu;
}
uint32_t* async_status_word() {
    std::lock_guard<std::mutex> lk(g_async_mu);
    if (!g_async_status) {
        void* p = nullptr;
        const hipError_t e = hipHostMalloc(&p, 64, hipHostMallocMapped | hipHostMallocPortable);
        if (e != hipSuccess || !p) {
            set_error("hipHostMalloc of the async status word failed: %s", hipGetErrorString(e));
            return nullptr;
        }
        memset(p, 0, 64);
        g_async_status = static_cast<uint32_t*>(p);
    }
    return g_async_status;
}
int take_async_status() {
    std::lock_guard<std::mutex> lk(g_async_mu);
    if (!g_async_status) return 0;
    return (int)__atomic_exchange_n(g_async_status, 0u, __ATOMIC_ACQ_REL);
}
int check_async_status(const char* where) {
    const int st = take_async_status();
    if (st == 0) return OGS_OK;
    set_error("%s: a kernel of an earlier launch reported status 0x%x%s -- the results of the passes since the last check "
              "are not valid", where, st,
              (st & (int)kAsyncRadixSpin) ? " (one-launch radix pass: a look-back wait exceeded its bound)" : "");
    return OGS_ERR_DEVICE;
}

}
int ogs::blend_prefetch_lines() {
    static const int v = [] {
        const char* e = getenv("OGS_BLEND_PREFETCH");
        const int n = e ? atoi(e) : kPrefetchMax;
        const int lines = (n & 0xFF) > kPrefetchMax ? kPrefetchMax : (n & 0xFF);
#ifdef OGS_EXPERIMENTS
        return n < 0 ? 0 : (lines | (n & 0x300));
#else
        return n < 0 ? 0 : lines;
#endif
    }();
    return v;
}
namespace ogs {

static int bit_length(uint32_t v) {
    int n = 0;
    while (v) { ++n; v >>= 1; }
    return n;
}

static int validate_fwd(const OgsRasterFwdArgs* a, bool images = true) {
    if (!a) { set_error("args == NULL"); return OGS_ERR_INVALID_ARG; }
    if (a->P < 0 || a->W <= 0 || a->H <= 0) { set_error("bad sizes P=%d W=%d H=%d", a->P, a->W, a->H); return OGS_ERR_INVALID_ARG; }
    if (a->C != 3 && a->C != 6 && a->C != 9 && a->C != 12) { set_error("C=%d unsupported (3, 6, 9, 12)", a->C); return OGS_ERR_UNSUPPORTED; }
    if (a->shs == nullptr && a->colors_precomp == nullptr) {
        set_error("provide shs or colors_precomp"); return OGS_ERR_INVALID_ARG;
    }
    if (a->shs != nullptr && (a->colors_precomp != nullptr) != (a->C > 3)) {
        set_error("with shs: C == 3 and no colors_precomp, or C > 3 with colors_precomp holding the C-3 extra channels");
        return OGS_ERR_INVALID_ARG;
    }
    const bool sr = a->scales != nullptr && a->rotations != nullptr;
    if (sr == (a->cov3D_precomp != nullptr) || (a->scales != nullptr) != (a->rotations != nullptr)) {
        set_error("provide exactly one of (scales, rotations) / cov3D_precomp"); return OGS_ERR_INVALID_ARG;
    }
    if (a->shs) {
        if (a->sh_degree < 0 || a->sh_degree > 3 || a->sh_coeffs < (a->sh_degree + 1) * (a->sh_degree + 1)) {
            set_error("sh_degree=%d needs >= %d coefficients, got %d", a->sh_degree, (a->sh_degree + 1) * (a->sh_degree + 1), a->sh_coeffs);
            return OGS_ERR_INVALID_ARG;
        }
    }
    if (!a->bg || !a->viewmatrix || !a->projmatrix || !a->campos || (images && (!a->out_color || !a->out_depth || !a->out_alpha))) {
        set_error("NULL required pointer"); return OGS_ERR_INVALID_ARG;
    }
    if (a->P > 0 && (!a->means3D || !a->opacities || !a->radii || !a->geom_buffer || !a->geom_tmp)) {
        set_error("NULL required per-Gaussian pointer"); return OGS_ERR_INVALID_ARG;
    }
    if (a->num_groups < 0 || (a->num_groups > 1 && a->P > 0 && !a->group_ids)) {
        set_error("num_groups=%d needs group_ids", a->num_groups); return OGS_ERR_INVALID_ARG;
    }
    return OGS_OK;
}

}

using namespace ogs;

extern "C" {

int ogs_version(void) { return 403; }

int ogs_check_async_status(void) { return check_async_status("ogs_check_async_status"); }

int ogs_prof_enable(int on) {
    std::lock_guard<std::mutex> lk(g_prof_mu);
    for (auto& r : g_prof) { g_event_pool.push_back(r.start); g_event_pool.push_back(r.stop); }
    g_prof.clear();
    g_prof_mode = on;
    return OGS_OK;
}

int ogs_prof_filter(const char* prefix) {
    std::lock_guard<std::mutex> lk(g_prof_mu);
    if (!prefix || strlen(prefix) >= sizeof(g_prof_prefix)) { set_error("prof_filter: prefix NULL or longer than %zu", sizeof(g_prof_prefix) - 1); return OGS_ERR_INVALID_ARG; }
    strcpy(g_prof_prefix, prefix);
    return OGS_OK;
}

int ogs_prof_collect(char* buf, size_t n) {
    std::lock_guard<std::mutex> lk(g_prof_mu);
    std::map<std::string, std::pair<long, double>> agg;
    for (auto& r : g_prof) {
        OGS_HIP_CHECK(hipEventSynchronize(r.stop));
        float ms = 0.f;
        OGS_HIP_CHECK(hipEventElapsedTime(&ms, r.start, r.stop));
        auto& a = agg[r.name];
        a.first += 1;
        a.second += ms;
    }
    std::string out = "{";
    bool first = true;
    for (auto& kv : agg) {
        char line[384];
        std::string nm = kv.first;
        for (auto& ch : nm) if (ch == '"') ch = '\'';
        snprintf(line, sizeof(line), "%s\"%s\": {\"calls\": %ld, \"total_ms\": %.6f}", first ? "" : ", ", nm.c_str(),
                 kv.second.first, kv.second.second);
        out += line;
        first = false;
    }
    out += "}";
    if (!buf || out.size() + 1 > n) { set_error("prof_collect: buffer too small (%zu needed)", out.size() + 1); return OGS_ERR_SCRATCH_TOO_SMALL; }
    memcpy(buf, out.c_str(), out.size() + 1);
    return OGS_OK;
}
const char* ogs_last_error(void) { return g_err; }

size_t ogs_raster_geom_bytes(int32_t P, int32_t C) { return GeomState::bytes(P > 0 ? P : 1, C); }
size_t ogs_raster_geom_tmp_bytes(int32_t P) { return GeomTmp::bytes(P > 0 ? P : 1); }
size_t ogs_raster_image_bytes(int32_t W, int32_t H) { return ImageState::bytes(W, H); }
size_t ogs_raster_image_bytes_grouped(int32_t W, int32_t H, int32_t G) { return ImageState::bytes(W, H, num_groups_of(G)); }
size_t ogs_raster_binning_tmp_bytes(int64_t D, int32_t, int32_t) { return BinTmp::bytes(D > 0 ? D : 1); }
size_t ogs_raster_sorted_bytes(int64_t D, int32_t C) {
    return align_up((size_t)(D > 0 ? D : 1) * stream_vec4(C) * sizeof(float4));
}
size_t ogs_raster_quad_list_bytes(int64_t D) {
    return align_up((size_t)(5 * (D > 0 ? D : 1) + 2 * kQuadPad) * sizeof(uint32_t));
}
size_t ogs_raster_backward_tmp_bytes(int32_t P) { return align_up((size_t)(P > 0 ? P : 1) * 16 * sizeof(double)); }

int ogs_raster_forward_geometry(const OgsRasterFwdArgs* a, void* stream_, int64_t* num_rendered_host) {
    int rc = validate_fwd(a, false);
    if (rc != OGS_OK) return rc;
    hipStream_t s = static_cast<hipStream_t>(stream_);
    if (num_rendered_host) *num_rendered_host = 0;
    if (a->P == 0) return OGS_OK;
    rc = check_async_status("forward (entry)");
    if (rc != OGS_OK) return rc;
    const GeomState gs = GeomState::carve(a->geom_buffer, a->P, a->C);
    const GeomTmp gt = GeomTmp::carve(a->geom_tmp, a->P);
    if (a->P <= kSmallMaxP) {
        rc = launch_small_geometry(*a, gs, gt, s);
        if (rc != OGS_OK) return rc;
    } else if (per_tile_depth_order(*a)) {
        rc = launch_preprocess(*a, gs, gt, s);
        if (rc != OGS_OK) return rc;
        rc = exclusive_scan_u32(gt.tiles_touched, nullptr, gt.offsets, a->P, gt.num_rendered, gt.sort_tmp, s, a->debug);
        if (rc != OGS_OK) return rc;
    } else {
        rc = launch_preprocess(*a, gs, gt, s);
        if (rc != OGS_OK) return rc;
        const bool sweep = radix_onesweep_enabled(a->P);
        if (sweep) {
            const int shifts[4] = {0, 8, 16, 24}, nbits[4] = {8, 8, 8, 8};
            rc = radix_sort_begin(gt.keys[0], a->P, nullptr, 4, shifts, nbits, gt.sort_tmp, s, a->debug, true);
            if (rc != OGS_OK) return rc;
        }
        for (int pass = 0; pass < 4; ++pass) {
            const int in = pass & 1, out = in ^ 1;
            const bool drop = pass == 0;
            const uint32_t* n_pass = drop ? nullptr : gt.visible();
            rc = sweep ? radix_sort_pass(pass, 4, gt.keys[in], gt.order[in], gt.keys[out], gt.order[out], a->P, 8 * pass, 8, gt.sort_tmp, s, a->debug, n_pass, drop, drop ? gt.visible() : nullptr)
                       : radix_pass(gt.keys[in], gt.order[in], gt.keys[out], gt.order[out], a->P, 8 * pass, 8, gt.sort_tmp, s, a->debug, n_pass, drop, drop ? gt.visible() : nullptr);
            if (rc != OGS_OK) return rc;
        }
        rc = exclusive_scan_u32(gt.tiles_touched, gt.order[0], gt.offsets, a->P, gt.num_rendered, gt.sort_tmp, s, a->debug, gt.visible());
        if (rc != OGS_OK) return rc;
    }
    if (num_rendered_host) {
        uint32_t d = 0;
        OGS_HIP_CHECK(hipMemcpyAsync(&d, gt.num_rendered, sizeof(uint32_t), hipMemcpyDeviceToHost, s));
        OGS_HIP_CHECK(hipStreamSynchronize(s));
        *num_rendered_host = (int64_t)d;
        rc = check_async_status("forward geometry phase");
        if (rc != OGS_OK) return rc;
    }
    return OGS_OK;
}

int ogs_raster_read_num_rendered_async(const OgsRasterFwdArgs* a, void* stream_, uint32_t* host_pinned) {
    if (!a || !host_pinned) { set_error("read_num_rendered_async: NULL pointer"); return OGS_ERR_INVALID_ARG; }
    if (a->P == 0) { *host_pinned = 0; return OGS_OK; }
    const GeomTmp gt = GeomTmp::carve(a->geom_tmp, a->P);
    OGS_HIP_CHECK(hipMemcpyAsync(host_pinned, gt.num_rendered, sizeof(uint32_t), hipMemcpyDeviceToHost,
                                 static_cast<hipStream_t>(stream_)));
    return OGS_OK;
}

static int render_impl(const OgsRasterFwdArgs* a, int64_t D, bool deferred, hipStream_t s,
                       const OgsGroupStatsArgs* stats = nullptr) {
    int rc = validate_fwd(a, stats == nullptr);
    if (rc != OGS_OK) return rc;
    if (!a->image_buffer) { set_error("image_buffer == NULL"); return OGS_ERR_INVALID_ARG; }
    const int G = num_groups_of(a->num_groups);
    const ImageState is = stats ? ImageState::carve_stats(a->image_buffer, a->W, a->H, G)
                                : ImageState::carve(a->image_buffer, a->W, a->H, G);
    const int gx = (a->W + kTile - 1) / kTile, gy = (a->H + kTile - 1) / kTile;
    const int64_t tiles = (int64_t)gx * gy * G;
    if (tiles >= (1ll << 31)) { set_error("%d groups x %d tiles exceed 2^31 virtual tiles", G, gx * gy); return OGS_ERR_UNSUPPORTED; }
    const GeomState gs = GeomState::carve(a->geom_buffer, a->P > 0 ? a->P : 1, a->C);
    const bool per_tile = per_tile_depth_order(*a);
    bool order_ready = false;
    if (D > 0) {
        if (!a->point_list || !a->binning_tmp) { set_error("point_list / binning_tmp == NULL with num_rendered=%lld", (long long)D); return OGS_ERR_INVALID_ARG; }
        if (D >= (1ll << 31)) { set_error("num_rendered=%lld exceeds 2^31", (long long)D); return OGS_ERR_UNSUPPORTED; }
        const GeomTmp gt = GeomTmp::carve(a->geom_tmp, a->P);
        const BinTmp bt = BinTmp::carve(a->binning_tmp, D);
        const int bits = bit_length((uint32_t)(tiles - 1));
        const int passes = bits == 0 ? 1 : (bits + 7) / 8;
        const int per = bits == 0 ? 1 : (bits + passes - 1) / passes;
        uint32_t* vbuf[2];
        vbuf[passes & 1] = a->point_list;
        vbuf[(passes & 1) ^ 1] = bt.vals;
        const uint32_t* n_dev = deferred ? gt.num_rendered : nullptr;
        const bool cull = a->full_binning == 0;
        const bool zero_in_dup = tiles <= (int64_t)a->P;
        rc = launch_duplicate(*a, gs, gt, bt.tile_keys[0], vbuf[0], (uint32_t)D, cull, !per_tile, s,
                              zero_in_dup ? is.ranges : nullptr, zero_in_dup ? (int)tiles : 0);
        if (rc != OGS_OK) return rc;
        const bool sweep = radix_onesweep_enabled(D);
        int shifts[4], nbits[4];
        for (int p = 0; p < passes; ++p) {
            shifts[p] = p * per;
            nbits[p] = (p == passes - 1) ? (bits == 0 ? 1 : bits - shifts[p]) : per;
        }
        if (passes == 2 && (bits & 1)) {
            nbits[0] = bits / 2; shifts[1] = nbits[0]; nbits[1] = bits - nbits[0];
        }
        if (sweep) {
            rc = radix_sort_begin(bt.tile_keys[0], D, n_dev, passes, shifts, nbits, bt.sort_tmp, s, a->debug, cull);
            if (rc != OGS_OK) return rc;
        }
        for (int p = 0; p < passes; ++p) {
            const int in = p & 1, out = in ^ 1;
            const bool drop = cull && p == 0;
            const uint32_t* n_pass = (cull && p > 0) ? bt.kept : n_dev;
            rc = sweep ? radix_sort_pass(p, passes, bt.tile_keys[in], vbuf[in], bt.tile_keys[out], vbuf[out], D, shifts[p], nbits[p], bt.sort_tmp, s, a->debug, n_pass, drop, drop ? bt.kept : nullptr)
                       : radix_pass(bt.tile_keys[in], vbuf[in], bt.tile_keys[out], vbuf[out], D, shifts[p], nbits[p], bt.sort_tmp, s, a->debug, n_pass, drop, drop ? bt.kept : nullptr);
            if (rc != OGS_OK) return rc;
        }
        rc = launch_tile_ranges(bt.tile_keys[passes & 1], D, is.ranges, tiles, s, a->debug, cull ? bt.kept : n_dev, zero_in_dup);
        if (rc != OGS_OK) return rc;
        if (per_tile) {
            const uint32_t* order = launch_tile_order(is, tiles, a->P, s, a->debug);
            order_ready = true;
            rc = launch_tile_depth_sort(is.ranges, tiles, order, a->point_list, gt.keys[0], bt.vals, s, a->debug);
            if (rc != OGS_OK) return rc;
        }
    } else {
        OGS_HIP_CHECK(hipMemsetAsync(is.ranges, 0, (size_t)tiles * sizeof(uint2), s));
    }
    if (stats) return launch_group_stats(*a, *stats, gs, is, s, order_ready);
    if (!a->sorted_rec || !a->quad_list) { set_error("sorted_rec / quad_list == NULL"); return OGS_ERR_INVALID_ARG; }
    return launch_blend_forward(*a, gs, is, D, s, order_ready);
}

int ogs_raster_forward_render(const OgsRasterFwdArgs* a, int64_t D, void* stream_) {
    return render_impl(a, D, false, static_cast<hipStream_t>(stream_));
}

size_t ogs_raster_stats_image_bytes(int32_t W, int32_t H, int32_t G) {
    return ImageState::stats_bytes(W > 0 ? W : 1, H > 0 ? H : 1, num_groups_of(G));
}
size_t ogs_raster_stats_tmp_bytes(int32_t G, int32_t L, int32_t C) {
    return align_up((size_t)num_groups_of(G) * (size_t)((L > 0 ? L : 0) + 1) * (size_t)(C > 0 ? C : 1) * sizeof(int64_t));
}

int ogs_raster_forward_group_stats(const OgsRasterFwdArgs* a, const OgsGroupStatsArgs* st, int64_t D, void* stream_) {
    if (!a || !st) { set_error("forward_group_stats: NULL argument"); return OGS_ERR_INVALID_ARG; }
    if (st->num_labels < 0) { set_error("forward_group_stats: num_labels=%d < 0", st->num_labels); return OGS_ERR_INVALID_ARG; }
    if (!st->labels || !st->max_alpha || !st->count || !st->feat_sum || !st->stats_tmp) {
        set_error("forward_group_stats: NULL labels / output / stats_tmp pointer"); return OGS_ERR_INVALID_ARG;
    }
    if (D < 0) { set_error("forward_group_stats: num_rendered=%lld < 0", (long long)D); return OGS_ERR_INVALID_ARG; }
    if (a->P == 0) D = 0;
    return render_impl(a, D, false, static_cast<hipStream_t>(stream_), st);
}

int ogs_raster_forward_render_deferred(const OgsRasterFwdArgs* a, int64_t capacity, void* stream_) {
    if (capacity <= 0) { set_error("forward_render_deferred: capacity must be > 0"); return OGS_ERR_INVALID_ARG; }
    return render_impl(a, capacity, true, static_cast<hipStream_t>(stream_));
}

int ogs_raster_forward_reblend(const OgsRasterFwdArgs* a, void* stream_) {
    if (!a) { set_error("args == NULL"); return OGS_ERR_INVALID_ARG; }
    if (a->P <= 0 || a->W <= 0 || a->H <= 0) { set_error("forward_reblend: bad sizes P=%d W=%d H=%d", a->P, a->W, a->H); return OGS_ERR_INVALID_ARG; }
    if (a->C != 3 && a->C != 6 && a->C != 9 && a->C != 12) { set_error("C=%d unsupported (3, 6, 9, 12)", a->C); return OGS_ERR_UNSUPPORTED; }
    if (a->num_groups > 1) { set_error("forward_reblend: grouped passes are not kept"); return OGS_ERR_UNSUPPORTED; }
    if (!a->colors_precomp || !a->bg || !a->out_color || !a->out_depth || !a->out_alpha || !a->image_buffer || !a->sorted_rec ||
        !a->quad_list) {
        set_error("forward_reblend: NULL required pointer (colors_precomp, bg, out_*, image_buffer, sorted_rec, quad_list)");
        return OGS_ERR_INVALID_ARG;
    }
    const int rc = check_async_status("forward_reblend (entry)");
    if (rc != OGS_OK) return rc;
    const ImageState is = ImageState::carve(a->image_buffer, a->W, a->H, 1);
    return launch_reblend(*a, is, static_cast<hipStream_t>(stream_));
}

int ogs_raster_compact_kept(int32_t W, int32_t H, int32_t C, const void* image_buffer, const void* sorted_rec, const void* quad_list,
                            void* new_image_buffer, void* new_sorted_rec, void* new_quad_list, void* stream_) {
    if (W <= 0 || H <= 0) { set_error("compact_kept: bad sizes W=%d H=%d", W, H); return OGS_ERR_INVALID_ARG; }
    if (!image_buffer || !sorted_rec || !quad_list || !new_image_buffer || !new_sorted_rec || !new_quad_list) {
        set_error("compact_kept: NULL pointer"); return OGS_ERR_INVALID_ARG;
    }
    const ImageState is_old = ImageState::carve(const_cast<void*>(image_buffer), W, H, 1);
    const ImageState is_new = ImageState::carve(new_image_buffer, W, H, 1);
    return launch_compact_kept(W, H, C, is_old, is_new, sorted_rec, quad_list, new_sorted_rec, new_quad_list,
                               static_cast<hipStream_t>(stream_));
}

size_t ogs_raster_tiny_max_points(void) { return (size_t)kTinyMaxP; }

size_t ogs_raster_tile_sort_capacity(int32_t level) {
    return level == 0 ? (size_t)kWaveSortCap : level == 1 ? (size_t)kTileSortCap : 0;
}

int ogs_raster_forward_tiny(const OgsRasterFwdArgs* a, void* stream_) {
    int rc = validate_fwd(a);
    if (rc != OGS_OK) return rc;
    if (a->P <= 0 || a->P > kTinyMaxP) { set_error("forward_tiny: P=%d outside [1, %d]", a->P, kTinyMaxP); return OGS_ERR_INVALID_ARG; }
    if (a->num_groups > 1) { set_error("forward_tiny: grouped passes use the streaming path"); return OGS_ERR_UNSUPPORTED; }
    hipStream_t s = static_cast<hipStream_t>(stream_);
    const GeomState gs = GeomState::carve(a->geom_buffer, a->P, a->C);
    uint32_t* order = static_cast<uint32_t*>(a->geom_tmp);
    rc = launch_tiny_geometry(*a, gs, order, s);
    if (rc != OGS_OK) return rc;
    return launch_tiny_blend(*a, gs, order, s);
}

int ogs_raster_backward(const OgsRasterBwdArgs* a, void* stream_) {
    if (!a) { set_error("args == NULL"); return OGS_ERR_INVALID_ARG; }
    if (a->C != 3 && a->C != 6 && a->C != 9) { set_error("backward: C=%d unsupported (3, 6, 9)", a->C); return OGS_ERR_UNSUPPORTED; }
    if (a->P == 0) return OGS_OK;
    const bool feat_only = backward_is_features_only(*a);
    if (!a->dL_dcolor || !a->image_buffer || !a->bwd_tmp || !a->radii) {
        set_error("backward: NULL required pointer"); return OGS_ERR_INVALID_ARG;
    }
    if (!feat_only && (!a->geom_buffer || !a->bg || !a->means3D || !a->viewmatrix || !a->projmatrix || !a->campos)) {
        set_error("backward: NULL required pointer"); return OGS_ERR_INVALID_ARG;
    }
    if (!feat_only && a->num_rendered > 0 && !a->point_list) { set_error("backward: point_list == NULL"); return OGS_ERR_INVALID_ARG; }
    if ((int64_t)a->P * grad_stride(a->C) >= (1ll << 32)) {
        set_error("backward: P=%d exceeds the %lld Gaussians the 32-bit gradient-record offsets address", a->P,
                  (long long)((1ll << 32) / grad_stride(a->C)) - 1);
        return OGS_ERR_UNSUPPORTED;
    }
    {
        const int st = check_async_status("backward (entry)");
        if (st != OGS_OK) return st;
    }
    hipStream_t s = static_cast<hipStream_t>(stream_);
    const GeomState gs = GeomState::carve(const_cast<void*>(a->geom_buffer), a->P, a->C);
    if (a->num_groups < 0) { set_error("backward: num_groups=%d", a->num_groups); return OGS_ERR_INVALID_ARG; }
    const ImageState is = ImageState::carve(const_cast<void*>(a->image_buffer), a->W, a->H, num_groups_of(a->num_groups));
    void* grad_rec = a->bwd_tmp;
    const int rec_doubles = feat_only ? feat_grad_stride(a->C, a->shs ? 3 : 0) : grad_stride(a->C);
    OGS_HIP_CHECK(hipMemsetAsync(grad_rec, 0, (size_t)a->P * rec_doubles * sizeof(double), s));
    if (a->num_rendered > 0 && (!a->sorted_rec || !a->quad_list)) { set_error("backward: sorted_rec / quad_list == NULL"); return OGS_ERR_INVALID_ARG; }
    int rc = launch_blend_backward(*a, is, grad_rec, s);
    if (rc != OGS_OK) return rc;
    return launch_preprocess_backward(*a, gs, grad_rec, s);
}

int ogs_mark_visible(int32_t P, const float* means3D, const float* viewmatrix, const float*, uint8_t* present,
                     void* stream_) {
    if (P == 0) return OGS_OK;
    if (!means3D || !viewmatrix || !present) { set_error("mark_visible: NULL pointer"); return OGS_ERR_INVALID_ARG; }
    return launch_mark_visible(P, means3D, viewmatrix, present, static_cast<hipStream_t>(stream_));
}

int ogs_sh_grad_from_views(int32_t P, int32_t V, int32_t sh_degree, int32_t sh_coeffs, const float* means3D,
                           const float* campos, const float* dL_drgb, float* dL_dsh, void* stream_) {
    if (P == 0) return OGS_OK;
    if (P < 0 || V < 1 || sh_degree < 0 || sh_degree > 3 || sh_coeffs < (sh_degree + 1) * (sh_degree + 1)) {
        set_error("sh_grad_from_views: bad sizes P=%d V=%d degree=%d coeffs=%d", P, V, sh_degree, sh_coeffs);
        return OGS_ERR_INVALID_ARG;
    }
    if (!means3D || !campos || !dL_drgb || !dL_dsh) { set_error("sh_grad_from_views: NULL pointer"); return OGS_ERR_INVALID_ARG; }
    return launch_sh_grad_from_views(P, V, sh_degree, sh_coeffs, means3D, campos, dL_drgb, dL_dsh,
                                     static_cast<hipStream_t>(stream_));
}

int ogs_selftest_wave_fold16(const float* in, float* out, void* stream_) {
    if (!in || !out) { set_error("selftest: NULL pointer"); return OGS_ERR_INVALID_ARG; }
    return launch_wave_fold16_test(in, out, static_cast<hipStream_t>(stream_));
}

int ogs_selftest_tile_order(const uint32_t* ranges, int64_t vtiles, uint32_t* order, void* stream_) {
    if (!ranges || !order || vtiles <= 0) { set_error("selftest: NULL pointer / no tiles"); return OGS_ERR_INVALID_ARG; }
    return launch_tile_order_test(ranges, vtiles, order, static_cast<hipStream_t>(stream_));
}

size_t ogs_selftest_radix_tmp_bytes(int64_t n) { return sort_tmp_bytes(n > 0 ? n : 1); }

int ogs_selftest_radix_sort(uint32_t* keys0, uint32_t* vals0, uint32_t* keys1, uint32_t* vals1, int64_t n, int32_t key_bits,
                            int32_t variant, int32_t items, const uint32_t* n_dev, void* tmp, int32_t* result_buffer,
                            void* stream_) {
    if (!result_buffer) { set_error("selftest_radix_sort: NULL result_buffer"); return OGS_ERR_INVALID_ARG; }
    *result_buffer = 0;
    if (n <= 0) return OGS_OK;
    if (items != 0 && items != 4 && items != 16) { set_error("selftest_radix_sort: items=%d (0, 4 or 16)", items); return OGS_ERR_INVALID_ARG; }
    if (!keys0 || !vals0 || !keys1 || !vals1 || !tmp || key_bits < 1 || key_bits > 32) {
        set_error("selftest_radix_sort: bad arguments"); return OGS_ERR_INVALID_ARG;
    }
    hipStream_t s = static_cast<hipStream_t>(stream_);
    uint32_t* k[2] = {keys0, keys1};
    uint32_t* v[2] = {vals0, vals1};
    const int passes = (key_bits + 7) / 8, per = (key_bits + passes - 1) / passes;
    int shifts[4], nbits[4];
    for (int p = 0; p < passes; ++p) { shifts[p] = p * per; nbits[p] = p == passes - 1 ? key_bits - shifts[p] : per; }
    const bool sweep = (variant & 1) != 0, drop = (variant & 2) != 0;
    const int spin_limit = (variant & 4) ? 0 : -1;
    (void)take_async_status();
    uint32_t* kept = nullptr;
    if (drop) {
        OGS_HIP_CHECK(hipMalloc(&kept, sizeof(uint32_t)));
        OGS_HIP_CHECK(hipMemsetAsync(kept, 0xA5, sizeof(uint32_t), s));
    }
    int rc = OGS_OK;
    if (sweep) rc = radix_sort_begin(k[0], n, n_dev, passes, shifts, nbits, tmp, s, 0, drop, items);
    for (int p = 0; p < passes && rc == OGS_OK; ++p) {
        const int in = p & 1, out = in ^ 1;
        const bool d0 = drop && p == 0;
        const uint32_t* n_pass = (drop && p > 0) ? kept : n_dev;
        rc = sweep ? radix_sort_pass(p, passes, k[in], v[in], k[out], v[out], n, shifts[p], nbits[p], tmp, s, 0, n_pass, d0, d0 ? kept : nullptr, items, spin_limit)
                   : radix_pass(k[in], v[in], k[out], v[out], n, shifts[p], nbits[p], tmp, s, 0, n_pass, d0, d0 ? kept : nullptr);
    }
    uint32_t kept_host = 0;
    if (drop) {
        if (rc == OGS_OK && hipMemcpyAsync(&kept_host, kept, sizeof(uint32_t), hipMemcpyDeviceToHost, s) != hipSuccess) rc = OGS_ERR_HIP;
        (void)hipStreamSynchronize(s);
        (void)hipFree(kept);
    } else {
        (void)hipStreamSynchronize(s);
    }
    if (rc != OGS_OK) return rc;
    *result_buffer = (passes & 1) | (drop ? (int32_t)(kept_host << 1) : 0);
    return check_async_status("selftest_radix_sort");
}

int ogs_raster_export_binning(const OgsRasterFwdArgs* a, int64_t D, uint64_t* keys_out, uint32_t* ranges_out,
                              uint32_t* n_contrib_out, void* stream_) {
    if (!a) { set_error("args == NULL"); return OGS_ERR_INVALID_ARG; }
    hipStream_t s = static_cast<hipStream_t>(stream_);
    const int G = num_groups_of(a->num_groups);
    const ImageState is = ImageState::carve(a->image_buffer, a->W, a->H, G);
    const int gx = (a->W + kTile - 1) / kTile, gy = (a->H + kTile - 1) / kTile;
    if (keys_out && D > 0) {
        const GeomState gs = GeomState::carve(a->geom_buffer, a->P, a->C);
        int rc = launch_export_keys(is.ranges, gx * gy * G, a->point_list, gs.rec, rec_vec4(a->C), keys_out, s);
        if (rc != OGS_OK) return rc;
    }
    if (ranges_out)
        OGS_HIP_CHECK(hipMemcpyAsync(ranges_out, is.ranges, (size_t)gx * gy * G * sizeof(uint2), hipMemcpyDeviceToDevice, s));
    if (n_contrib_out) {
        if (D > 0) {
            int rc = launch_export_n_contrib(*a, is, n_contrib_out, s);
            if (rc != OGS_OK) return rc;
        } else {
            OGS_HIP_CHECK(hipMemsetAsync(n_contrib_out, 0, (size_t)G * a->W * a->H * sizeof(uint32_t), s));
        }
    }
    return OGS_OK;
}

}
```

opengaussian_amd/csrc/ogs_common.h:

```cpp
#pragma once

#include <hip/hip_runtime.h>
#include <stdint.h>
#include <stddef.h>
#include <stdio.h>

#include "../../include/ogs_raster.h"

namespace ogs {

constexpr int kTile = OGS_TILE;
constexpr int kBlock = 256;
constexpr int kWave = 64;
constexpr int kTinyMaxP = 256;
constexpr int kSmallMaxP = 1024;

void set_error(const char* fmt, ...);

#define OGS_HIP_CHECK(expr)                                                              \
    do {                                                                                 \
        hipError_t _e = (expr);                                                          \
        if (_e != hipSuccess) {                                                          \
            ogs::set_error("%s failed: %s (%s:%d)", #expr, hipGetErrorString(_e), __FILE__, __LINE__); \
            return OGS_ERR_HIP;                                                          \
        }                                                                                \
    } while (0)

#define OGS_LAUNCH_CHECK(debug, stream)                                                  \
    do {                                                                                 \
        OGS_HIP_CHECK(hipGetLastError());                                                \
        if (debug) OGS_HIP_CHECK(hipStreamSynchronize(stream));                          \
    } while (0)

constexpr uint32_t kAsyncRadixSpin = 1u;
uint32_t* async_status_word();
int take_async_status();
int check_async_status(const char* where);

struct ProfScope {
    const char* name;
    hipStream_t stream;
    int slot;
    ProfScope(const char* name, hipStream_t s);
    ~ProfScope();
};
#define OGS_LAUNCH(kernel, grid, block, lds, stream, ...)                      \
    do {                                                                       \
        ogs::ProfScope _ps(#kernel, stream);                                   \
        hipLaunchKernelGGL(kernel, grid, block, lds, stream, __VA_ARGS__);     \
    } while (0)

#define OGS_LAUNCH_NAMED(name, kernel, grid, block, lds, stream, ...)          \
    do {                                                                       \
        ogs::ProfScope _ps(name, stream);                                      \
        hipLaunchKernelGGL(kernel, grid, block, lds, stream, __VA_ARGS__);     \
    } while (0)
template <int C>
constexpr const char* chan_name(const char* const (&names)[4]) {
    return C == 3 ? names[0] : C == 6 ? names[1] : C == 9 ? names[2] : names[3];
}

constexpr size_t kAlign = 256;
inline size_t align_up(size_t v, size_t a = kAlign) { return (v + a - 1) / a * a; }

struct Carver {
    char* base;
    size_t off = 0;
    explicit Carver(void* p) : base(static_cast<char*>(p)) {}
    template <typename T>
    T* take(size_t n) {
        T* r = reinterpret_cast<T*>(base ? base + off : nullptr);
        off = align_up(off + n * sizeof(T));
        return r;
    }
};

__host__ __device__ constexpr int rec_vec4(int C) { return 2 + (C + 3) / 4; }

__host__ __device__ constexpr int stream_vec4(int C) { return (8 + C + 1 + 3) / 4; }

constexpr int kQuadPad = 16;
template <int C>
inline float4* stream_base(void* buf) { return static_cast<float4*>(buf); }
inline uint32_t* quad_base(void* buf) { return static_cast<uint32_t*>(buf) + kQuadPad; }
constexpr float kFar = 3.0e18f;
constexpr float kFarTest = 1.0e18f;

typedef float f8 __attribute__((ext_vector_type(8)));
template <int C>
struct StreamRec {
    static constexpr int NF4 = stream_vec4(C) - 2;
    f8 g;
    float4 f[NF4];
    __device__ __forceinline__ void load(const float* __restrict__ p) {
        g = *reinterpret_cast<const f8*>(p);
#pragma unroll
        for (int k = 0; k < NF4; ++k) f[k] = *reinterpret_cast<const float4*>(p + 8 + 4 * k);
    }
    __device__ __forceinline__ float feat(int c) const {
        const float4 v = f[c >> 2];
        return (c & 3) == 0 ? v.x : (c & 3) == 1 ? v.y : (c & 3) == 2 ? v.z : v.w;
    }
};

constexpr int kSlotDepth = 9, kSlotMoments = 10;
__host__ __device__ constexpr int grad_stride(int C) { return (C + 7 <= 16) ? 16 : 32; }
__host__ __device__ constexpr int feat_grad_stride(int C, int F0) { return (C - F0 <= 8) ? 8 : grad_stride(C); }

struct GeomState {
    float4* rec;
    uint32_t* clamped;
    static GeomState carve(void* p, int P, int C) {
        Carver c(p);
        GeomState g;
        g.rec = c.take<float4>((size_t)P * rec_vec4(C));
        g.clamped = c.take<uint32_t>(P);
        return g;
    }
    static size_t bytes(int P, int C) {
        Carver c(nullptr);
        c.take<float4>((size_t)P * rec_vec4(C));
        c.take<uint32_t>(P);
        return c.off;
    }
};

struct ImageState {
    uint2* ranges;
    uint32_t* n_contrib;
    uint32_t* qcount;
    float* final_T;
    uint32_t* tile_order;
    static ImageState carve(void* p, int W, int H, int G = 1) {
        Carver c(p);
        ImageState s;
        const size_t tiles = (size_t)G * ((W + kTile - 1) / kTile) * ((H + kTile - 1) / kTile);
        s.ranges = c.take<uint2>(tiles);
        s.n_contrib = c.take<uint32_t>((size_t)G * W * H);
        s.qcount = c.take<uint32_t>(tiles * 5);
        s.final_T = c.take<float>((size_t)G * W * H);
        s.tile_order = c.take<uint32_t>(tiles);
        return s;
    }
    static size_t bytes(int W, int H, int G = 1) {
        Carver c(nullptr);
        const size_t tiles = (size_t)G * ((W + kTile - 1) / kTile) * ((H + kTile - 1) / kTile);
        c.take<uint2>(tiles);
        c.take<uint32_t>((size_t)G * W * H);
        c.take<uint32_t>(tiles * 5);
        c.take<float>((size_t)G * W * H);
        c.take<uint32_t>(tiles);
        return c.off;
    }
    static ImageState carve_stats(void* p, int W, int H, int G) {
        Carver c(p);
        ImageState s{};
        const size_t tiles = (size_t)G * ((W + kTile - 1) / kTile) * ((H + kTile - 1) / kTile);
        s.ranges = c.take<uint2>(tiles);
        s.tile_order = c.take<uint32_t>(tiles);
        return s;
    }
    static size_t stats_bytes(int W, int H, int G) {
        Carver c(nullptr);
        const size_t tiles = (size_t)G * ((W + kTile - 1) / kTile) * ((H + kTile - 1) / kTile);
        c.take<uint2>(tiles);
        c.take<uint32_t>(tiles);
        return c.off;
    }
};
const uint32_t* launch_tile_order(const ImageState& is, int64_t vtiles, int P, hipStream_t s, int debug);
const uint32_t* tile_order_of(const ImageState& is, int64_t vtiles, int P);
int launch_export_n_contrib(const OgsRasterFwdArgs& a, const ImageState& is, uint32_t* out, hipStream_t s);

constexpr int kSortItemsLarge = 8;
inline int sort_items_for(int64_t n) { return n <= (int64_t)(3 << 20) ? 4 : kSortItemsLarge; }
inline int sort_blocks_for(int64_t n) {
    const int64_t tile = (int64_t)kBlock * sort_items_for(n);
    return (int)((n + tile - 1) / tile);
}
size_t scan_tmp_bytes(int64_t n);
size_t sort_tmp_bytes(int64_t n);

int exclusive_scan_u32(const uint32_t* in, const uint32_t* gather, uint32_t* out, int64_t n,
                       uint32_t* total, void* tmp, hipStream_t stream, int debug, const uint32_t* n_dev = nullptr);
constexpr uint32_t kDropKey = 0xFFFFFFFFu;
bool radix_onesweep_enabled(int64_t n);
int radix_sort_begin(const uint32_t* keys, int64_t n, const uint32_t* n_dev, int npass, const int* shifts, const int* bits,
                     void* tmp, hipStream_t stream, int debug, bool drop = false, int items = 0);
int radix_sort_pass(int pass, int npass, const uint32_t* keys_in, const uint32_t* vals_in, uint32_t* keys_out,
                    uint32_t* vals_out, int64_t n, int shift, int bits, void* tmp, hipStream_t stream, int debug,
                    const uint32_t* n_dev = nullptr, bool drop = false, uint32_t* kept_out = nullptr, int items = 0,
                    int spin_limit = -1);
int radix_pass(const uint32_t* keys_in, const uint32_t* vals_in, uint32_t* keys_out, uint32_t* vals_out,
               int64_t n, int shift, int bits, void* tmp, hipStream_t stream, int debug,
               const uint32_t* n_dev = nullptr, bool drop = false, uint32_t* kept_out = nullptr);

struct GeomTmp {
    uint32_t* tiles_touched;
    uint32_t* keys[2];
    uint32_t* order[2];
    uint32_t* offsets;
    uint32_t* num_rendered;
    void* sort_tmp;
    uint32_t* visible() const { return num_rendered + 1; }
    static GeomTmp carve(void* p, int P) {
        Carver c(p);
        GeomTmp g;
        g.tiles_touched = c.take<uint32_t>(P);
        g.keys[0] = c.take<uint32_t>(P);
        g.keys[1] = c.take<uint32_t>(P);
        g.order[0] = c.take<uint32_t>(P);
        g.order[1] = c.take<uint32_t>(P);
        g.offsets = c.take<uint32_t>(P);
        g.num_rendered = c.take<uint32_t>(64);
        g.sort_tmp = c.take<char>(sort_tmp_bytes(P));
        return g;
    }
    static size_t bytes(int P) {
        Carver c(nullptr);
        for (int i = 0; i < 6; ++i) c.take<uint32_t>(P);
        c.take<uint32_t>(64);
        c.take<char>(sort_tmp_bytes(P));
        return c.off;
    }
};

struct BinTmp {
    uint32_t* tile_keys[2];
    uint32_t* vals;
    uint32_t* kept;
    void* sort_tmp;
    static BinTmp carve(void* p, int64_t D) {
        Carver c(p);
        BinTmp b;
        b.tile_keys[0] = c.take<uint32_t>(D);
        b.tile_keys[1] = c.take<uint32_t>(D);
        b.vals = c.take<uint32_t>(D);
        b.kept = c.take<uint32_t>(1);
        b.sort_tmp = c.take<char>(sort_tmp_bytes(D));
        return b;
    }
    static size_t bytes(int64_t D) {
        Carver c(nullptr);
        for (int i = 0; i < 3; ++i) c.take<uint32_t>(D);
        c.take<uint32_t>(1);
        c.take<char>(sort_tmp_bytes(D));
        return c.off;
    }
};

int launch_preprocess(const OgsRasterFwdArgs& a, const GeomState& gs, const GeomTmp& gt, hipStream_t s);
int launch_tiny_geometry(const OgsRasterFwdArgs& a, const GeomState& gs, uint32_t* order, hipStream_t s);
int launch_small_geometry(const OgsRasterFwdArgs& a, const GeomState& gs, const GeomTmp& gt, hipStream_t s);
int launch_tiny_blend(const OgsRasterFwdArgs& a, const GeomState& gs, const uint32_t* order, hipStream_t s);
int launch_reblend(const OgsRasterFwdArgs& a, const ImageState& is, hipStream_t s);
int launch_compact_kept(int W, int H, int C, const ImageState& is_old, const ImageState& is_new, const void* old_rec,
                        const void* old_quad, void* new_rec, void* new_quad, hipStream_t s);
int launch_duplicate(const OgsRasterFwdArgs& a, const GeomState& gs, const GeomTmp& gt, uint32_t* tile_keys,
                     uint32_t* vals, uint32_t capacity, bool drop_unreachable, bool depth_order, hipStream_t s,
                     uint2* zero_ranges = nullptr, int n_zero = 0);
int launch_tile_ranges(const uint32_t* tile_keys_sorted, int64_t D, uint2* ranges, int64_t tiles, hipStream_t s,
                       int debug, const uint32_t* n_dev = nullptr, bool already_zeroed = false);
inline bool per_tile_depth_order(const OgsRasterFwdArgs& a) { return a.num_groups <= 1 && a.P > kSmallMaxP; }
constexpr int kTileSortItems = 16;
constexpr int kTileSortCap = kBlock * kTileSortItems;
constexpr int kWaveSortCap = kTileSortCap / (kBlock / kWave);
int launch_tile_depth_sort(const uint2* ranges, int64_t tiles, const uint32_t* tile_order, uint32_t* point_list,
                           const uint32_t* depth_keys, uint32_t* scratch, hipStream_t s, int debug);
inline int num_groups_of(int g) { return g > 1 ? g : 1; }
int launch_group_stats(const OgsRasterFwdArgs& a, const OgsGroupStatsArgs& st, const GeomState& gs, const ImageState& is,
                       hipStream_t s, bool order_ready = false);
int launch_blend_forward(const OgsRasterFwdArgs& a, const GeomState& gs, const ImageState& is, int64_t D,
                         hipStream_t s, bool order_ready = false);
int launch_blend_backward(const OgsRasterBwdArgs& a, const ImageState& is, void* grad_rec, hipStream_t s);
int launch_preprocess_backward(const OgsRasterBwdArgs& a, const GeomState& gs, const void* grad_rec, hipStream_t s);
inline bool backward_is_features_only(const OgsRasterBwdArgs& a) {
    return a.dL_dcolors != nullptr && a.colors_precomp != nullptr && !a.dL_dmeans2D && !a.dL_dopacity &&
           !a.dL_dmeans3D && !a.dL_dcov3D && !a.dL_dsh && !a.dL_dscales && !a.dL_drotations && !a.dL_dsh_rgb;
}
int launch_sh_grad_from_views(int P, int V, int sh_degree, int sh_coeffs, const float* means3D, const float* campos,
                              const float* dL_drgb, float* dL_dsh, hipStream_t s);
int launch_wave_fold16_test(const float* in, float* out, hipStream_t s);
int launch_tile_order_test(const uint32_t* ranges, int64_t vtiles, uint32_t* order, hipStream_t s);
int launch_mark_visible(int P, const float* means3D, const float* viewmatrix, uint8_t* present, hipStream_t s);
int launch_export_keys(const uint2* ranges, int tiles, const uint32_t* point_list, const float4* rec, int recv4,
                       uint64_t* keys_out, hipStream_t s);

__device__ __forceinline__ float blend_power(float a2, float b2, float c2, float dx, float dy) {
    const float u = fmaf(b2, dy, a2 * dx);
    return fmaf(c2 * dy, dy, u * dx);
}

constexpr int kPrefetchMax = 4;
struct RecordPrefetch {
    uint32_t v[kPrefetchMax];
    __device__ __forceinline__ void issue(const float* __restrict__ tile_records, int n_tile, int rec_floats, int tid,
                                          int lines) {
        const uint32_t total = (uint32_t)n_tile * (uint32_t)rec_floats;
#pragma unroll
        for (int k = 0; k < kPrefetchMax; ++k) {
            v[k] = 0u;
            const uint32_t off = ((uint32_t)(k * kBlock + tid)) * 32u;
            if (k < lines && off < total) v[k] = __float_as_uint(tile_records[off]);
        }
    }
    __device__ __forceinline__ void retire(uint32_t* __restrict__ sink, int never) const {
        const uint32_t x = v[0] ^ v[1] ^ v[2] ^ v[3];
        if (never < 0 && x == 0x7FC12345u) sink[0] = x;
    }
};
int blend_prefetch_lines();

constexpr float kThrMargin = 0.01f;
constexpr int kReachBit = 31;
constexpr uint32_t kGidMask = (1u << kReachBit) - 1u;
__device__ __forceinline__ float max_power_in_box(float A, float B, float Cc, float nbA, float nbC, float xlo, float xhi,
                                                  float ylo, float yhi) {
    if (xlo <= 0.f && xhi >= 0.f && ylo <= 0.f && yhi >= 0.f) return 0.f;
    auto q = [&](float dx, float dy) { return -0.5f * (A * dx * dx + Cc * dy * dy) - B * dx * dy; };
    float m = q(xlo, fminf(fmaxf(nbC * xlo, ylo), yhi));
    m = fmaxf(m, q(xhi, fminf(fmaxf(nbC * xhi, ylo), yhi)));
    m = fmaxf(m, q(fminf(fmaxf(nbA * ylo, xlo), xhi), ylo));
    m = fmaxf(m, q(fminf(fmaxf(nbA * yhi, xlo), xhi), yhi));
    const float X = fmaxf(fabsf(xlo), fabsf(xhi)), Y = fmaxf(fabsf(ylo), fabsf(yhi));
    return m + 8e-7f * (0.5f * (A * X * X + Cc * Y * Y) + fabsf(B) * X * Y);
}
__device__ __forceinline__ float max_power_in_box(float A, float B, float Cc, float xlo, float xhi, float ylo,
                                                  float yhi) {
    return max_power_in_box(A, B, Cc, -B / A, -B / Cc, xlo, xhi, ylo, yhi);
}

__device__ __forceinline__ void wait_scalar_loads() {
    __builtin_amdgcn_sched_barrier(0);
    __builtin_amdgcn_s_waitcnt(0xC07F);
    __builtin_amdgcn_sched_barrier(0);
}
__device__ __forceinline__ int lane_id() { return threadIdx.x & (kWave - 1); }
__device__ __forceinline__ void lds_barrier() { asm volatile("s_waitcnt lgkmcnt(0)\n\ts_barrier" ::: "memory"); }

}
```

opengaussian_amd/csrc/preprocess_fwd.hip:

```cpp
#include "ogs_common.h"

namespace ogs {

namespace {

__constant__ const float kC0 = 0.28209479177387814f;
__constant__ const float kC1 = 0.4886025119029199f;
__constant__ const float kC2[5] = {1.0925484305920792f, -1.0925484305920792f, 0.31539156525252005f,
                                   -1.0925484305920792f, 0.5462742152960396f};
__constant__ const float kC3[7] = {-0.5900435899266435f, 2.890611442640554f, -0.4570457994644658f,
                                   0.3731763325901154f, -0.4570457994644658f, 1.445305721320277f,
                                   -0.5900435899266435f};

struct Cam {
    float V[16];
    float M[16];
    float campos[3];
};

__device__ __forceinline__ void cov3d_from_scale_rot(const float* __restrict__ scales,
                                                     const float* __restrict__ rots, int idx, float mod,
                                                     float cov[6]) {
    const float sx = mod * scales[3 * idx + 0], sy = mod * scales[3 * idx + 1], sz = mod * scales[3 * idx + 2];
    const float4 q = reinterpret_cast<const float4*>(rots)[idx];
    const float r = q.x, x = q.y, y = q.z, z = q.w;
    const float R00 = 1.f - 2.f * (y * y + z * z), R01 = 2.f * (x * y - r * z), R02 = 2.f * (x * z + r * y);
    const float R10 = 2.f * (x * y + r * z), R11 = 1.f - 2.f * (x * x + z * z), R12 = 2.f * (y * z - r * x);
    const float R20 = 2.f * (x * z - r * y), R21 = 2.f * (y * z + r * x), R22 = 1.f - 2.f * (x * x + y * y);
    const float M00 = R00 * sx, M01 = R01 * sy, M02 = R02 * sz;
    const float M10 = R10 * sx, M11 = R11 * sy, M12 = R12 * sz;
    const float M20 = R20 * sx, M21 = R21 * sy, M22 = R22 * sz;
    cov[0] = M00 * M00 + M01 * M01 + M02 * M02;
    cov[1] = M00 * M10 + M01 * M11 + M02 * M12;
    cov[2] = M00 * M20 + M01 * M21 + M02 * M22;
    cov[3] = M10 * M10 + M11 * M11 + M12 * M12;
    cov[4] = M10 * M20 + M11 * M21 + M12 * M22;
    cov[5] = M20 * M20 + M21 * M21 + M22 * M22;
}

__device__ __forceinline__ void sh_to_rgb(int idx, int deg, int M, const float* __restrict__ shs, float px,
                                          float py, float pz, const float* campos, float rgb[3],
                                          uint32_t& clamped) {
    const float* sh = shs + (size_t)idx * M * 3;
    float dx = px - campos[0], dy = py - campos[1], dz = pz - campos[2];
    const float ln = sqrtf(dx * dx + dy * dy + dz * dz);
    const float x = dx / ln, y = dy / ln, z = dz / ln;
    float res[3];
#pragma unroll
    for (int c = 0; c < 3; ++c) res[c] = kC0 * sh[c];
    if (deg > 0) {
#pragma unroll
        for (int c = 0; c < 3; ++c)
            res[c] = res[c] - kC1 * y * sh[3 + c] + kC1 * z * sh[6 + c] - kC1 * x * sh[9 + c];
        if (deg > 1) {
            const float xx = x * x, yy = y * y, zz = z * z, xy = x * y, yz = y * z, xz = x * z;
#pragma unroll
            for (int c = 0; c < 3; ++c)
                res[c] = res[c] + kC2[0] * xy * sh[12 + c] + kC2[1] * yz * sh[15 + c] +
                         kC2[2] * (2.f * zz - xx - yy) * sh[18 + c] + kC2[3] * xz * sh[21 + c] +
                         kC2[4] * (xx - yy) * sh[24 + c];
            if (deg > 2) {
#pragma unroll
                for (int c = 0; c < 3; ++c)
                    res[c] = res[c] + kC3[0] * y * (3.f * xx - yy) * sh[27 + c] + kC3[1] * xy * z * sh[30 + c] +
                             kC3[2] * y * (4.f * zz - xx - yy) * sh[33 + c] +
                             kC3[3] * z * (2.f * zz - 3.f * xx - 3.f * yy) * sh[36 + c] +
                             kC3[4] * x * (4.f * zz - xx - yy) * sh[39 + c] + kC3[5] * z * (xx - yy) * sh[42 + c] +
                             kC3[6] * x * (xx - 3.f * yy) * sh[45 + c];
            }
        }
    }
    clamped = 0;
#pragma unroll
    for (int c = 0; c < 3; ++c) {
        res[c] = res[c] + 0.5f;
        if (res[c] < 0.f) clamped |= 1u << c;
        rgb[c] = fmaxf(res[c], 0.f);
    }
}

template <int C>
__device__ __forceinline__ uint32_t preprocess_one(
    int idx, int W, int H, int sh_degree, int sh_coeffs, float tanfovx, float tanfovy, float focal_x, float focal_y,
    float scale_modifier, const float* __restrict__ means3D, const float* __restrict__ colors_precomp,
    const float* __restrict__ shs, const float* __restrict__ opacities, const float* __restrict__ scales,
    const float* __restrict__ rotations, const float* __restrict__ cov3D_precomp, const float* __restrict__ viewmatrix,
    const float* __restrict__ projmatrix, const float* __restrict__ campos, float4* __restrict__ rec_row,
    uint32_t* __restrict__ clamped_out, int32_t* __restrict__ radii, uint32_t* __restrict__ tiles_touched,
    const int32_t* __restrict__ group_ids, int num_groups) {
    constexpr int NV = rec_vec4(C);
    float V[16], M[16];
#pragma unroll
    for (int i = 0; i < 16; ++i) { V[i] = viewmatrix[i]; M[i] = projmatrix[i]; }

    const float x = means3D[3 * idx + 0], y = means3D[3 * idx + 1], z = means3D[3 * idx + 2];
    const float opacity = opacities[idx];

    float feat[(C + 3) / 4 * 4];
#pragma unroll
    for (int c = 0; c < (C + 3) / 4 * 4; ++c) feat[c] = 0.f;
    uint32_t clamped = 0;

    int radius = 0;
    uint32_t touched = 0;
    float pxl = 0.f, pyl = 0.f, depth = 0.f, cA = 0.f, cB = 0.f, cC = 0.f;

    const float pvx = V[0] * x + V[4] * y + V[8] * z + V[12];
    const float pvy = V[1] * x + V[5] * y + V[9] * z + V[13];
    const float pvz = V[2] * x + V[6] * y + V[10] * z + V[14];
    bool ok = pvz > 0.2f;
    if (group_ids != nullptr) ok = ok && (uint32_t)group_ids[idx] < (uint32_t)num_groups;
    if (ok) {
        const float hx = M[0] * x + M[4] * y + M[8] * z + M[12];
        const float hy = M[1] * x + M[5] * y + M[9] * z + M[13];
        const float hw = M[3] * x + M[7] * y + M[11] * z + M[15];
        const float p_w = 1.0f / (hw + 0.0000001f);
        const float projx = hx * p_w, projy = hy * p_w;
        float cov[6];
        if (cov3D_precomp != nullptr) {
#pragma unroll
            for (int i = 0; i < 6; ++i) cov[i] = cov3D_precomp[6 * idx + i];
        } else {
            cov3d_from_scale_rot(scales, rotations, idx, scale_modifier, cov);
        }
        const float limx = 1.3f * tanfovx, limy = 1.3f * tanfovy;
        const float txtz = pvx / pvz, tytz = pvy / pvz;
        const float tx = fminf(limx, fmaxf(-limx, txtz)) * pvz;
        const float ty = fminf(limy, fmaxf(-limy, tytz)) * pvz;
        const float tz = pvz;
        const float J00 = focal_x / tz;
        const float J02 = -(focal_x * tx) / (tz * tz);
        const float J11 = focal_y / tz;
        const float J12 = -(focal_y * ty) / (tz * tz);
        const float T00 = J00 * V[0] + J02 * V[2];
        const float T01 = J00 * V[4] + J02 * V[6];
        const float T02 = J00 * V[8] + J02 * V[10];
        const float T10 = J11 * V[1] + J12 * V[2];
        const float T11 = J11 * V[5] + J12 * V[6];
        const float T12 = J11 * V[9] + J12 * V[10];
        const float a0 = T00 * cov[0] + T01 * cov[1] + T02 * cov[2];
        const float a1 = T00 * cov[1] + T01 * cov[3] + T02 * cov[4];
        const float a2 = T00 * cov[2] + T01 * cov[4] + T02 * cov[5];
        const float b0 = T10 * cov[0] + T11 * cov[1] + T12 * cov[2];
        const float b1 = T10 * cov[1] + T11 * cov[3] + T12 * cov[4];
        const float b2 = T10 * cov[2] + T11 * cov[4] + T12 * cov[5];
        const float ca = a0 * T00 + a1 * T01 + a2 * T02 + 0.3f;
        const float cb = a0 * T10 + a1 * T11 + a2 * T12;
        const float cc = b0 * T10 + b1 * T11 + b2 * T12 + 0.3f;
        const float det = ca * cc - cb * cb;
        ok = det != 0.f;
        if (ok) {
            const float det_inv = 1.f / det;
            cA = cc * det_inv;
            cB = -cb * det_inv;
            cC = ca * det_inv;
            const float mid = 0.5f * (ca + cc);
            const float sq = sqrtf(fmaxf(0.1f, mid * mid - det));
            const float lam = fmaxf(mid + sq, mid - sq);
            float rad_f = ceilf(3.f * sqrtf(lam));
            if (!(fabsf(rad_f) < 3.0e38f)) rad_f = 0.f;
            const int my_radius = (int)rad_f;
            pxl = ((projx + 1.0f) * (float)W - 1.0f) * 0.5f;
            pyl = ((projy + 1.0f) * (float)H - 1.0f) * 0.5f;
            const int gx = (W + kTile - 1) / kTile, gy = (H + kTile - 1) / kTile;
            const float rf = (float)my_radius;
            auto tr = [](float v) -> int {
                if (!(fabsf(v) < 3.0e38f)) v = 0.f;
                v = fminf(fmaxf(v, -2.0e9f), 2.0e9f);
                return (int)v;
            };
            const int rminx = min(gx, max(0, tr((pxl - rf) / (float)kTile)));
            const int rminy = min(gy, max(0, tr((pyl - rf) / (float)kTile)));
            const int rmaxx = min(gx, max(0, tr((pxl + rf + (float)kTile - 1.0f) / (float)kTile)));
            const int rmaxy = min(gy, max(0, tr((pyl + rf + (float)kTile - 1.0f) / (float)kTile)));
            const int area = (rmaxx - rminx) * (rmaxy - rminy);
            ok = area != 0 && my_radius > 0;
            if (ok) {
                radius = my_radius;
                touched = (uint32_t)area;
                depth = pvz;
            }
        }
    }

    const int coff = shs != nullptr ? 3 : 0;
    if (colors_precomp != nullptr) {
#pragma unroll
        for (int c = 0; c < C; ++c)
            if (c >= coff) feat[c] = colors_precomp[(size_t)idx * (C - coff) + (c - coff)];
    }
    if (shs != nullptr && ok) {
        float rgb[3];
        float cp[3] = {campos[0], campos[1], campos[2]};
        sh_to_rgb(idx, sh_degree, sh_coeffs, shs, x, y, z, cp, rgb, clamped);
        feat[0] = rgb[0]; feat[1] = rgb[1]; feat[2] = rgb[2];
    }

    if (!ok) { pxl = 0.f; pyl = 0.f; cA = cB = cC = 0.f; depth = 0.f; }

    float4* r = rec_row;
    r[0] = make_float4(pxl, pyl, depth, __int_as_float(radius));
    r[1] = make_float4(cA, cB, cC, opacity);
#pragma unroll
    for (int v = 0; v < NV - 2; ++v) r[2 + v] = make_float4(feat[4 * v], feat[4 * v + 1], feat[4 * v + 2], feat[4 * v + 3]);
    clamped_out[idx] = clamped;
    radii[idx] = radius;
    if (tiles_touched) tiles_touched[idx] = touched;
    return ok ? __float_as_uint(depth) : 0xFFFFFFFFu;
}

template <int C>
__global__ __launch_bounds__(kBlock) void preprocess_kernel(
    int P, int W, int H, int sh_degree, int sh_coeffs, float tanfovx, float tanfovy, float focal_x, float focal_y,
    float scale_modifier, const float* __restrict__ means3D, const float* __restrict__ colors_precomp,
    const float* __restrict__ shs, const float* __restrict__ opacities, const float* __restrict__ scales,
    const float* __restrict__ rotations, const float* __restrict__ cov3D_precomp, const float* __restrict__ viewmatrix,
    const float* __restrict__ projmatrix, const float* __restrict__ campos, float4* __restrict__ rec,
    uint32_t* __restrict__ clamped_out, int32_t* __restrict__ radii, uint32_t* __restrict__ tiles_touched,
    uint32_t* __restrict__ depth_keys, uint32_t* __restrict__ order, const int32_t* __restrict__ group_ids,
    int num_groups) {
    constexpr int NV = rec_vec4(C);
    __shared__ float4 s_rec[kBlock * NV];
    const int tid = threadIdx.x;
    const int idx = blockIdx.x * kBlock + tid;
    if (idx < P) {
        depth_keys[idx] = preprocess_one<C>(idx, W, H, sh_degree, sh_coeffs, tanfovx, tanfovy, focal_x, focal_y, scale_modifier,
                                            means3D, colors_precomp, shs, opacities, scales, rotations, cov3D_precomp, viewmatrix,
                                            projmatrix, campos, s_rec + tid * NV, clamped_out, radii, tiles_touched, group_ids,
                                            num_groups);
        if (order) order[idx] = (uint32_t)idx;
    }
    __syncthreads();
    const size_t row0 = (size_t)blockIdx.x * kBlock;
    const int n4 = min(kBlock, P - (int)row0) * NV;
    float4* __restrict__ out = rec + row0 * NV;
    for (int e = tid; e < n4; e += kBlock) out[e] = s_rec[e];
}

template <int C>
__global__ __launch_bounds__(kTinyMaxP) void tiny_geometry_kernel(
    int P, int W, int H, int sh_degree, int sh_coeffs, float tanfovx, float tanfovy, float focal_x, float focal_y,
    float scale_modifier, const float* __restrict__ means3D, const float* __restrict__ colors_precomp,
    const float* __restrict__ shs, const float* __restrict__ opacities, const float* __restrict__ scales,
    const float* __restrict__ rotations, const float* __restrict__ cov3D_precomp, const float* __restrict__ viewmatrix,
    const float* __restrict__ projmatrix, const float* __restrict__ campos, float4* __restrict__ rec,
    uint32_t* __restrict__ clamped_out, int32_t* __restrict__ radii, uint32_t* __restrict__ order) {
    __shared__ uint32_t s_key[kTinyMaxP];
    const int idx = threadIdx.x;
    uint32_t key = 0xFFFFFFFFu;
    if (idx < P)
        key = preprocess_one<C>(idx, W, H, sh_degree, sh_coeffs, tanfovx, tanfovy, focal_x, focal_y, scale_modifier, means3D,
                                colors_precomp, shs, opacities, scales, rotations, cov3D_precomp, viewmatrix, projmatrix,
                                campos, rec + (size_t)idx * rec_vec4(C), clamped_out, radii, nullptr, nullptr, 0);
    s_key[idx] = key;
    __syncthreads();
    if (idx < P) {
        int rank = 0;
        for (int j = 0; j < P; ++j) {
            const uint32_t kj = s_key[j];
            rank += (kj < key || (kj == key && j < idx)) ? 1 : 0;
        }
        order[rank] = (uint32_t)idx;
    }
}

template <int C>
__global__ __launch_bounds__(kSmallMaxP) void small_geometry_kernel(
    int P, int W, int H, int sh_degree, int sh_coeffs, float tanfovx, float tanfovy, float focal_x, float focal_y,
    float scale_modifier, const float* __restrict__ means3D, const float* __restrict__ colors_precomp,
    const float* __restrict__ shs, const float* __restrict__ opacities, const float* __restrict__ scales,
    const float* __restrict__ rotations, const float* __restrict__ cov3D_precomp, const float* __restrict__ viewmatrix,
    const float* __restrict__ projmatrix, const float* __restrict__ campos, float4* __restrict__ rec,
    uint32_t* __restrict__ clamped_out, int32_t* __restrict__ radii, uint32_t* __restrict__ order,
    uint32_t* __restrict__ offsets, uint32_t* __restrict__ num_rendered, const int32_t* __restrict__ group_ids,
    int num_groups) {
    __shared__ uint32_t s_key[kSmallMaxP];
    __shared__ uint32_t s_touched[kSmallMaxP];
    __shared__ uint32_t s_sorted[kSmallMaxP];
    __shared__ uint32_t s_wave[kSmallMaxP / kWave];
    const int idx = threadIdx.x, lane = idx & 63, wave = idx >> 6;
    uint32_t key = 0xFFFFFFFFu;
    s_touched[idx] = 0u;
    if (idx < P)
        key = preprocess_one<C>(idx, W, H, sh_degree, sh_coeffs, tanfovx, tanfovy, focal_x, focal_y, scale_modifier, means3D,
                                colors_precomp, shs, opacities, scales, rotations, cov3D_precomp, viewmatrix, projmatrix,
                                campos, rec + (size_t)idx * rec_vec4(C), clamped_out, radii, s_touched, group_ids, num_groups);
    s_key[idx] = key;
    __syncthreads();
    int rank = idx;
    if (idx < P) {
        rank = 0;
        for (int j = 0; j < P; ++j) {
            const uint32_t kj = s_key[j];
            rank += (kj < key || (kj == key && j < idx)) ? 1 : 0;
        }
        order[rank] = (uint32_t)idx;
    }
    s_sorted[rank] = s_touched[idx];
    __syncthreads();
    const uint32_t v = s_sorted[idx];
    uint32_t incl = v;
#pragma unroll
    for (int d = 1; d < kWave; d <<= 1) {
        const uint32_t o = __shfl_up(incl, d, kWave);
        if (lane >= d) incl += o;
    }
    if (lane == kWave - 1) s_wave[wave] = incl;
    __syncthreads();
    uint32_t before = 0u, total = 0u;
#pragma unroll
    for (int w = 0; w < kSmallMaxP / kWave; ++w) {
        const uint32_t t = s_wave[w];
        if (w < wave) before += t;
        total += t;
    }
    if (idx < P) offsets[idx] = before + incl - v;
    if (idx == 0) { num_rendered[0] = total; num_rendered[1] = (uint32_t)P; }
}

template <int NV>
__global__ __launch_bounds__(kBlock) void duplicate_kernel(int P_cap, const uint32_t* __restrict__ n_visible, int W, int H,
                                                           const float4* __restrict__ rec,
                                                           const uint32_t* __restrict__ order,
                                                           const uint32_t* __restrict__ offsets,
                                                           uint32_t* __restrict__ tile_keys,
                                                           uint32_t* __restrict__ vals, uint32_t capacity,
                                                           const int32_t* __restrict__ group_ids, bool drop_unreachable,
                                                           uint2* __restrict__ zero_ranges, int n_zero) {
    __shared__ uint32_t s_off[kBlock];
    __shared__ uint32_t s_gid[kBlock];
    __shared__ uint32_t s_rect[kBlock];
    __shared__ uint32_t s_first, s_total;
    __shared__ uint32_t s_key0[kBlock];
    __shared__ float4 s_ctr[kBlock];
    __shared__ float4 s_con[kBlock];
    const int tid = threadIdx.x;
    const int r = blockIdx.x * kBlock + tid;
    if (zero_ranges != nullptr && r < n_zero) zero_ranges[r] = make_uint2(0u, 0u);
    const int P = n_visible ? min(P_cap, (int)*n_visible) : P_cap;
    if ((int)blockIdx.x * kBlock >= P) return;
    const int gx = (W + kTile - 1) / kTile, gy = (H + kTile - 1) / kTile;
    uint32_t off = 0, cnt = 0, gid = 0, rect = 1u << 24, key0 = 0;
    float4 ctr = make_float4(0.f, 0.f, 0.f, 0.f);
    float4 con = make_float4(1.f, 1.f, 0.f, 0.f);
    if (r < P) {
        gid = order ? order[r] : (uint32_t)r;
        off = offsets[r];
        if (group_ids != nullptr) key0 = (uint32_t)max(group_ids[gid], 0) * (uint32_t)(gx * gy);
        const float4 a = rec[(size_t)gid * NV];
        const int radius = __float_as_int(a.w);
        if (radius > 0) {
            const float4 b = rec[(size_t)gid * NV + 1];
            ctr = make_float4(a.x, a.y, -(__logf(255.0f * b.w) + kThrMargin), b.y);
            con = make_float4(b.x, b.z, -b.y / b.x, -b.y / b.z);
            const float rf = (float)radius;
            auto tr = [](float v) -> int {
                if (!(fabsf(v) < 3.0e38f)) v = 0.f;
                v = fminf(fmaxf(v, -2.0e9f), 2.0e9f);
                return (int)v;
            };
            const int rminx = min(gx, max(0, tr((a.x - rf) / (float)kTile)));
            const int rminy = min(gy, max(0, tr((a.y - rf) / (float)kTile)));
            const int rmaxx = min(gx, max(0, tr((a.x + rf + (float)kTile - 1.0f) / (float)kTile)));
            const int rmaxy = min(gy, max(0, tr((a.y + rf + (float)kTile - 1.0f) / (float)kTile)));
            const int w = rmaxx - rminx, h = rmaxy - rminy;
            if (w > 0 && h > 0) {
                cnt = (uint32_t)(w * h);
                rect = (uint32_t)rminx | ((uint32_t)rminy << 12) | ((uint32_t)min(w, 255) << 24);
                if (w > 255) {
                    uint32_t o = off;
                    for (int ty = rminy; ty < rmaxy; ++ty)
                        for (int tx = rminx; tx < rmaxx; ++tx) {
                            if (o < capacity) { tile_keys[o] = key0 + (uint32_t)(ty * gx + tx); vals[o] = gid | (1u << kReachBit); }
                            ++o;
                        }
                    rect |= 0u;
                    gid |= 0x80000000u;
                }
            }
        }
    }
    if (tid == 0) s_first = off;
    __syncthreads();
    const uint32_t first = s_first;
    s_off[tid] = (r < P) ? off - first : 0xFFFFFFFFu;
    s_gid[tid] = gid;
    s_rect[tid] = rect;
    s_key0[tid] = key0;
    s_ctr[tid] = ctr;
    s_con[tid] = con;
    const int last = min(P - 1 - blockIdx.x * kBlock, kBlock - 1);
    if (tid == last) s_total = off - first + cnt;
    __syncthreads();
    const uint32_t total = s_total;
    for (uint32_t j = tid; j < total; j += kBlock) {
        int lo = 0, hi = kBlock;
#pragma unroll
        for (int step = kBlock / 2; step >= 1; step >>= 1) {
            const int mid = lo + step;
            if (mid < hi && s_off[mid] <= j) lo = mid;
        }
        const uint32_t g = s_gid[lo];
        if (g & 0x80000000u) continue;
        const uint32_t rc = s_rect[lo];
        const uint32_t local = j - s_off[lo];
        const uint32_t w = rc >> 24;
        const uint32_t row = local / w, col = local - row * w;
        const uint32_t o = first + j;
        if (o < capacity) {
            const uint32_t tx = (rc & 0xFFFu) + col, ty = (rc >> 12 & 0xFFFu) + row;
            const uint32_t key = s_key0[lo] + ty * (uint32_t)gx + tx;
            const float4 c = s_ctr[lo];
            const float4 k = s_con[lo];
            const float X0 = (float)(tx * kTile), Y0 = (float)(ty * kTile);
            const float m = max_power_in_box(k.x, c.w, k.y, k.z, k.w, c.x - X0 - 15.f, c.x - X0, c.y - Y0 - 15.f, c.y - Y0);
            const bool reach = m >= c.z;
            tile_keys[o] = (drop_unreachable && !reach) ? kDropKey : key;
            vals[o] = g | ((reach ? 1u : 0u) << kReachBit);
        }
    }
}

__global__ __launch_bounds__(kBlock) void mark_visible_kernel(int P, const float* __restrict__ means3D,
                                                              const float* __restrict__ V,
                                                              uint8_t* __restrict__ present) {
    const int idx = blockIdx.x * kBlock + threadIdx.x;
    if (idx >= P) return;
    const float x = means3D[3 * idx], y = means3D[3 * idx + 1], z = means3D[3 * idx + 2];
    const float pvz = V[2] * x + V[6] * y + V[10] * z + V[14];
    present[idx] = pvz > 0.2f ? 1 : 0;
}

template <int C>
int launch_preprocess_c(const OgsRasterFwdArgs& a, const GeomState& gs, const GeomTmp& gt, hipStream_t s) {
    const float focal_x = (float)a.W / (2.0f * a.tanfovx);
    const float focal_y = (float)a.H / (2.0f * a.tanfovy);
    const int grid = (a.P + kBlock - 1) / kBlock;
    static constexpr const char* const kNames[4] = {"preprocess_kernel<3>", "preprocess_kernel<6>", "preprocess_kernel<9>", "preprocess_kernel<12>"};
    OGS_LAUNCH_NAMED(chan_name<C>(kNames), preprocess_kernel<C>, dim3(grid), dim3(kBlock), 0, s, a.P, a.W, a.H, a.sh_degree, a.sh_coeffs,
                       a.tanfovx, a.tanfovy, focal_x, focal_y, a.scale_modifier, a.means3D, a.colors_precomp, a.shs,
                       a.opacities, a.scales, a.rotations, a.cov3D_precomp, a.viewmatrix, a.projmatrix, a.campos,
                       gs.rec, gs.clamped, a.radii, gt.tiles_touched, gt.keys[0],
                       per_tile_depth_order(a) ? (uint32_t*)nullptr : gt.order[0], a.num_groups > 1 ? a.group_ids : (const int32_t*)nullptr, a.num_groups);
    OGS_LAUNCH_CHECK(a.debug, s);
    return OGS_OK;
}

template <int C>
int launch_tiny_geometry_c(const OgsRasterFwdArgs& a, const GeomState& gs, uint32_t* order, hipStream_t s) {
    const float focal_x = (float)a.W / (2.0f * a.tanfovx);
    const float focal_y = (float)a.H / (2.0f * a.tanfovy);
    OGS_LAUNCH(tiny_geometry_kernel<C>, dim3(1), dim3(kTinyMaxP), 0, s, a.P, a.W, a.H, a.sh_degree, a.sh_coeffs, a.tanfovx,
               a.tanfovy, focal_x, focal_y, a.scale_modifier, a.means3D, a.colors_precomp, a.shs, a.opacities, a.scales,
               a.rotations, a.cov3D_precomp, a.viewmatrix, a.projmatrix, a.campos, gs.rec, gs.clamped, a.radii, order);
    OGS_LAUNCH_CHECK(a.debug, s);
    return OGS_OK;
}

template <int C>
int launch_small_geometry_c(const OgsRasterFwdArgs& a, const GeomState& gs, const GeomTmp& gt, hipStream_t s) {
    const float focal_x = (float)a.W / (2.0f * a.tanfovx);
    const float focal_y = (float)a.H / (2.0f * a.tanfovy);
    OGS_LAUNCH(small_geometry_kernel<C>, dim3(1), dim3(kSmallMaxP), 0, s, a.P, a.W, a.H, a.sh_degree, a.sh_coeffs, a.tanfovx,
               a.tanfovy, focal_x, focal_y, a.scale_modifier, a.means3D, a.colors_precomp, a.shs, a.opacities, a.scales,
               a.rotations, a.cov3D_precomp, a.viewmatrix, a.projmatrix, a.campos, gs.rec, gs.clamped, a.radii, gt.order[0],
               gt.offsets, gt.num_rendered, a.num_groups > 1 ? a.group_ids : (const int32_t*)nullptr, a.num_groups);
    OGS_LAUNCH_CHECK(a.debug, s);
    return OGS_OK;
}

}

int launch_small_geometry(const OgsRasterFwdArgs& a, const GeomState& gs, const GeomTmp& gt, hipStream_t s) {
    switch (a.C) {
        case 3: return launch_small_geometry_c<3>(a, gs, gt, s);
        case 6: return launch_small_geometry_c<6>(a, gs, gt, s);
        case 9: return launch_small_geometry_c<9>(a, gs, gt, s);
        case 12: return launch_small_geometry_c<12>(a, gs, gt, s);
        default: set_error("unsupported channel count C=%d (3, 6, 9 or 12)", a.C); return OGS_ERR_UNSUPPORTED;
    }
}

int launch_tiny_geometry(const OgsRasterFwdArgs& a, const GeomState& gs, uint32_t* order, hipStream_t s) {
    switch (a.C) {
        case 3: return launch_tiny_geometry_c<3>(a, gs, order, s);
        case 6: return launch_tiny_geometry_c<6>(a, gs, order, s);
        case 9: return launch_tiny_geometry_c<9>(a, gs, order, s);
        case 12: return launch_tiny_geometry_c<12>(a, gs, order, s);
        default: set_error("unsupported channel count C=%d (3, 6, 9 or 12)", a.C); return OGS_ERR_UNSUPPORTED;
    }
}

int launch_preprocess(const OgsRasterFwdArgs& a, const GeomState& gs, const GeomTmp& gt, hipStream_t s) {
    switch (a.C) {
        case 3: return launch_preprocess_c<3>(a, gs, gt, s);
        case 6: return launch_preprocess_c<6>(a, gs, gt, s);
        case 9: return launch_preprocess_c<9>(a, gs, gt, s);
        case 12: return launch_preprocess_c<12>(a, gs, gt, s);
        default: set_error("unsupported channel count C=%d (3, 6, 9 or 12)", a.C); return OGS_ERR_UNSUPPORTED;
    }
}

int launch_duplicate(const OgsRasterFwdArgs& a, const GeomState& gs, const GeomTmp& gt, uint32_t* tile_keys,
                     uint32_t* vals, uint32_t capacity, bool drop_unreachable, bool depth_order, hipStream_t s, uint2* zero_ranges,
                     int n_zero) {
    if (n_zero > a.P) { set_error("duplicate: %d ranges to clear with %d threads", n_zero, a.P); return OGS_ERR_INVALID_ARG; }
    const int grid = (a.P + kBlock - 1) / kBlock;
    const int32_t* grp = a.num_groups > 1 ? a.group_ids : nullptr;
    if ((a.W + kTile - 1) / kTile > 4095 || (a.H + kTile - 1) / kTile > 4095) {
        set_error("image %dx%d exceeds 4095 tiles per side", a.W, a.H);
        return OGS_ERR_UNSUPPORTED;
    }
    const uint32_t* order = depth_order ? gt.order[0] : nullptr;
    const uint32_t* n_visible = depth_order ? gt.visible() : nullptr;
    switch (rec_vec4(a.C)) {
        case 3: OGS_LAUNCH(duplicate_kernel<3>, dim3(grid), dim3(kBlock), 0, s, a.P, n_visible, a.W, a.H, gs.rec, order, gt.offsets, tile_keys, vals, capacity, grp, drop_unreachable, zero_ranges, n_zero); break;
        case 4: OGS_LAUNCH(duplicate_kernel<4>, dim3(grid), dim3(kBlock), 0, s, a.P, n_visible, a.W, a.H, gs.rec, order, gt.offsets, tile_keys, vals, capacity, grp, drop_unreachable, zero_ranges, n_zero); break;
        case 5: OGS_LAUNCH(duplicate_kernel<5>, dim3(grid), dim3(kBlock), 0, s, a.P, n_visible, a.W, a.H, gs.rec, order, gt.offsets, tile_keys, vals, capacity, grp, drop_unreachable, zero_ranges, n_zero); break;
        default: set_error("unsupported record size"); return OGS_ERR_UNSUPPORTED;
    }
    OGS_LAUNCH_CHECK(a.debug, s);
    return OGS_OK;
}

int launch_mark_visible(int P, const float* means3D, const float* viewmatrix, uint8_t* present, hipStream_t s) {
    const int grid = (P + kBlock - 1) / kBlock;
    OGS_LAUNCH(mark_visible_kernel, dim3(grid), dim3(kBlock), 0, s, P, means3D, viewmatrix, present);
    OGS_LAUNCH_CHECK(0, s);
    return OGS_OK;
}

}
```

opengaussian_amd/rasterizer.py:

```python
from __future__ import annotations

import ctypes as C
import functools
import os
from typing import NamedTuple, Optional

import torch
from torch import nn

from . import _lib
from ._lib import OgsRasterBwdArgs, OgsRasterFwdArgs, check, ptr

SUPPORTED_CHANNELS = (3, 6, 9, 12)
BACKWARD_CHANNELS = (3, 6, 9)
TINY_MAX_P = 256
_DEBUG_KEEP_BWD_TMP = None
_LAST_NUM_RENDERED: dict = {}
_HINT_WINDOW = 32
PASS_STATS = {"blocking": 0, "deferred": 0, "overflow": 0, "tiny": 0, "tiny_rerendered_for_backward": 0, "reblend": 0}


def _hint_capacity(key):
    hist = _LAST_NUM_RENDERED.get(key)
    if not hist:
        return None
    return int(max(hist) * 1.25) + 4096


def _hint_record(key, D):
    from collections import deque
    if len(_LAST_NUM_RENDERED) > 256:
        _LAST_NUM_RENDERED.clear()
    hist = _LAST_NUM_RENDERED.get(key)
    if hist is None:
        hist = _LAST_NUM_RENDERED[key] = deque(maxlen=_HINT_WINDOW)
    hist.append(int(D))


class GaussianRasterizationSettings(NamedTuple):
    image_height: int
    image_width: int
    tanfovx: float
    tanfovy: float
    bg: torch.Tensor
    scale_modifier: float
    viewmatrix: torch.Tensor
    projmatrix: torch.Tensor
    sh_degree: int
    campos: torch.Tensor
    prefiltered: bool
    debug: bool


_READBACK: dict = {}


def _readback_slot(dev):
    slot = _READBACK.get(dev)
    if slot is None:
        slot = (torch.empty(1, dtype=torch.int32, pin_memory=True), torch.cuda.Event())
        _READBACK[dev] = slot
    return slot


def _stream() -> int:
    return torch.cuda.current_stream().cuda_stream


def _f32c(t: Optional[torch.Tensor]) -> Optional[torch.Tensor]:
    if t is None or t.numel() == 0:
        return None
    if t.dtype is torch.float32 and t.is_contiguous():
        return t.detach() if t.requires_grad else t
    return t.detach().to(torch.float32).contiguous()


_TINY_LIMIT = None
_TINY_SCRATCH: dict = {}


def _tiny_limit() -> int:
    global _TINY_LIMIT
    if _TINY_LIMIT is None:
        _TINY_LIMIT = int(_lib.lib().ogs_raster_tiny_max_points())
    return min(TINY_MAX_P, _TINY_LIMIT)


def _tiny_scratch(dev, stream: int, lib):
    key = (dev, stream)
    sc = _TINY_SCRATCH.get(key)
    if sc is None:
        n = int(lib.ogs_raster_tiny_max_points())
        sc = (torch.empty(int(lib.ogs_raster_geom_bytes(n, 12)), dtype=torch.uint8, device=dev),
              torch.empty(int(lib.ogs_raster_geom_tmp_bytes(n)), dtype=torch.uint8, device=dev))
        _TINY_SCRATCH[key] = sc
    return sc


_BG_TILED: dict = {}


def _tiled_bg(bg: torch.Tensor, Cn: int) -> torch.Tensor:
    key = (bg.data_ptr(), bg._version, Cn, bg.device)
    hit = _BG_TILED.get(key)
    if hit is None:
        if len(_BG_TILED) > 16:
            _BG_TILED.clear()
        hit = (bg, bg.repeat(Cn // 3))
        _BG_TILED[key] = hit
    return hit[1]


def _require_gpu(t: torch.Tensor, name: str):
    if not t.is_cuda:
        raise RuntimeError(f"{name} must live on the GPU (got {t.device}); the MI355X rasterizer has no CPU path")


FULL_BINNING = os.environ.get("OGS_FULL_BINNING", "0") == "1"


class full_binning:

    def __enter__(self):
        global FULL_BINNING
        self._prev, FULL_BINNING = FULL_BINNING, True
        return self

    def __exit__(self, *exc):
        global FULL_BINNING
        FULL_BINNING = self._prev
        return False


def _fwd_args(rs, P, Cn, m3, shs, cols, opac, scl, rot, cov, bg, view, proj, campos, color, depth, alpha, radii, group_ids, G):
    a = OgsRasterFwdArgs()
    a.P, a.W, a.H, a.C = P, int(rs.image_width), int(rs.image_height), Cn
    a.sh_degree = int(rs.sh_degree)
    a.sh_coeffs = 0 if shs is None else int(shs.shape[1])
    a.tanfovx, a.tanfovy, a.scale_modifier = float(rs.tanfovx), float(rs.tanfovy), float(rs.scale_modifier)
    a.prefiltered, a.debug = int(bool(rs.prefiltered)), int(bool(rs.debug))
    a.bg, a.means3D, a.colors_precomp, a.shs, a.opacities = ptr(bg), ptr(m3), ptr(cols), ptr(shs), ptr(opac)
    a.scales, a.rotations, a.cov3D_precomp = ptr(scl), ptr(rot), ptr(cov)
    a.viewmatrix, a.projmatrix, a.campos = ptr(view), ptr(proj), ptr(campos)
    a.out_color, a.out_depth, a.out_alpha, a.radii = ptr(color), ptr(depth), ptr(alpha), ptr(radii)
    a.group_ids, a.num_groups = ptr(group_ids), G
    a.full_binning = int(FULL_BINNING)
    return a


@functools.lru_cache(maxsize=256)
def _geom_sizes(P, W, H, Cn, G):
    lib = _lib.lib()
    return (int(lib.ogs_raster_geom_bytes(P, Cn)), int(lib.ogs_raster_geom_tmp_bytes(P)),
            int(lib.ogs_raster_image_bytes_grouped(W, H, G)))


@functools.lru_cache(maxsize=1024)
def _render_sizes(count, W, H, Cn):
    lib = _lib.lib()
    return (int(lib.ogs_raster_binning_tmp_bytes(count, W, H)), int(lib.ogs_raster_sorted_bytes(count, Cn)),
            int(lib.ogs_raster_quad_list_bytes(count)))


def _streaming_render(a: OgsRasterFwdArgs, dev, lib, debug: bool):
    P, W, H, Cn, G = int(a.P), int(a.W), int(a.H), int(a.C), max(int(a.num_groups), 1)
    u8 = lambda n: torch.empty(int(n), dtype=torch.uint8, device=dev)
    gb, gtb, ib = _geom_sizes(P, W, H, Cn, G)
    geom, geom_tmp, image = u8(gb), u8(gtb), u8(ib)
    a.geom_buffer, a.geom_tmp, a.image_buffer = ptr(geom), ptr(geom_tmp), ptr(image)
    stream = _stream()

    def alloc_render(count):
        btb, srb, qlb = _render_sizes(count, W, H, Cn)
        pl = torch.empty(max(count, 1), dtype=torch.int32, device=dev)
        bt, sr, ql = u8(btb), u8(srb), u8(qlb)
        a.point_list, a.binning_tmp, a.sorted_rec, a.quad_list = ptr(pl), ptr(bt), ptr(sr), ptr(ql)
        return pl, bt, sr, ql

    key = (P, W, H, G)
    cap = None if (G > 1 or debug) else _hint_capacity(key)
    if cap is None:
        PASS_STATS["blocking"] += 1
        n = C.c_int64(0)
        check(lib.ogs_raster_forward_geometry(C.byref(a), stream, C.byref(n)), "ogs_raster_forward_geometry")
        D = int(n.value)
        point_list, bin_tmp, sorted_rec, quad_list = alloc_render(D)
        check(lib.ogs_raster_forward_render(C.byref(a), D, stream), "ogs_raster_forward_render")
    else:
        check(lib.ogs_raster_forward_geometry(C.byref(a), stream, None), "ogs_raster_forward_geometry")
        pinned, ev = _readback_slot(dev)
        check(lib.ogs_raster_read_num_rendered_async(C.byref(a), stream, pinned.data_ptr()),
              "ogs_raster_read_num_rendered_async")
        ev.record()
        PASS_STATS["deferred"] += 1
        point_list, bin_tmp, sorted_rec, quad_list = alloc_render(cap)
        check(lib.ogs_raster_forward_render_deferred(C.byref(a), cap, stream), "ogs_raster_forward_render_deferred")
        ev.synchronize()
        check(lib.ogs_check_async_status(), "ogs_check_async_status")
        D = int(pinned.item()) & 0xFFFFFFFF
        if D > cap:
            PASS_STATS["overflow"] += 1
            point_list, bin_tmp, sorted_rec, quad_list = alloc_render(D)
            check(lib.ogs_raster_forward_render(C.byref(a), D, stream), "ogs_raster_forward_render")
    _hint_record(key, D)
    return geom, image, point_list, sorted_rec, quad_list, D


class _RasterizeGaussians(torch.autograd.Function):
    @staticmethod
    def forward(ctx, means3D, means2D, sh, colors_precomp, opacities, scales, rotations, cov3Ds_precomp,
                raster_settings: GaussianRasterizationSettings, geom_channels: int = 0, sh_rgb_sink=None,
                group_ids=None, num_groups: int = 1, keep_sink=None):
        rs = raster_settings
        ctx.geom_channels = int(geom_channels)
        ctx.sh_rgb_sink = sh_rgb_sink
        ctx.set_materialize_grads(False)
        G = max(int(num_groups), 1)
        ctx.num_groups = G
        if G > 1:
            if group_ids is None or group_ids.shape[0] != means3D.shape[0]:
                raise RuntimeError("a grouped pass needs group_ids [P]")
            group_ids = group_ids.detach().to(device=means3D.device, dtype=torch.int32).contiguous()
        else:
            group_ids = None
        _require_gpu(means3D, "means3D")
        dev = means3D.device
        lib = _lib.lib()
        P = int(means3D.shape[0])
        H, W = int(rs.image_height), int(rs.image_width)
        if means3D.dim() != 2 or means3D.shape[1] != 3:
            raise RuntimeError("means3D must have dimensions (num_points, 3)")

        m3 = _f32c(means3D)
        shs = _f32c(sh)
        cols = _f32c(colors_precomp)
        opac = _f32c(opacities)
        scl = _f32c(scales)
        rot = _f32c(rotations)
        cov = _f32c(cov3Ds_precomp)
        if shs is not None and cols is not None:
            Cn = 3 + int(cols.shape[1])
        else:
            Cn = 3 if cols is None else int(cols.shape[1])
        if Cn not in SUPPORTED_CHANNELS:
            raise RuntimeError(f"the blended channel count must be 3, 6, 9 or 12, got {Cn}")
        if Cn not in BACKWARD_CHANNELS and any(ctx.needs_input_grad[:8]):
            raise RuntimeError(f"a {Cn}-channel pass is forward-only (backward supports {BACKWARD_CHANNELS} channels): "
                               "detach the inputs or split the pass")
        bg = _f32c(rs.bg.to(dev))
        if bg is None or bg.numel() != Cn:
            if bg is not None and bg.numel() == 3 and Cn > 3:
                bg = _tiled_bg(bg, Cn)
            else:
                raise RuntimeError(f"bg must have {Cn} entries")
        view = _f32c(rs.viewmatrix.to(dev))
        proj = _f32c(rs.projmatrix.to(dev))
        campos = _f32c(rs.campos.to(dev))

        alloc = torch.zeros if P == 0 else torch.empty
        lead = (G,) if G > 1 else ()
        color = alloc(*lead, Cn, H, W, dtype=torch.float32, device=dev)
        depth = alloc(*lead, 1, H, W, dtype=torch.float32, device=dev)
        alpha = alloc(*lead, 1, H, W, dtype=torch.float32, device=dev)
        radii = alloc(P, dtype=torch.int32, device=dev)
        ctx.raster_settings = rs
        ctx.P, ctx.Cn, ctx.num_rendered, ctx.tiny = P, Cn, 0, False
        ctx.full_binning = bool(FULL_BINNING)
        if P == 0:
            ctx.save_for_backward()
            ctx.mark_non_differentiable(radii)
            return color, radii, depth, alpha

        a = _fwd_args(rs, P, Cn, m3, shs, cols, opac, scl, rot, cov, bg, view, proj, campos, color, depth, alpha, radii,
                      group_ids, G)

        if G == 1 and not rs.debug and P <= _tiny_limit():
            stream = _stream()
            geom, geom_tmp = _tiny_scratch(dev, stream, lib)
            a.geom_buffer, a.geom_tmp = geom.data_ptr(), geom_tmp.data_ptr()
            check(lib.ogs_raster_forward_tiny(C.byref(a), stream), "ogs_raster_forward_tiny")
            PASS_STATS["tiny"] += 1
            ctx.tiny, ctx.num_rendered = True, -1
            ctx.save_for_backward(m3, shs, cols, opac, scl, rot, cov, bg, view, proj, campos, radii, alpha)
            ctx.mark_non_differentiable(radii)
            return color, radii, depth, alpha

        geom, image, point_list, sorted_rec, quad_list, D = _streaming_render(a, dev, lib, rs.debug)
        ctx.num_rendered = D
        ctx.save_for_backward(m3, shs, cols, opac, scl, rot, cov, bg, view, proj, campos, radii, alpha, geom, image,
                              point_list, sorted_rec, quad_list)
        ctx.mark_non_differentiable(radii)
        if keep_sink is not None and G == 1 and D > 0:
            keep_sink.append({"P": P, "W": W, "H": H, "Cn": Cn, "fused": shs is not None and cols is not None, "D": D,
                              "image": image, "sorted_rec": sorted_rec, "quad_list": quad_list, "radii": radii,
                              "full_binning": bool(FULL_BINNING)})
        return color, radii, depth, alpha

    @staticmethod
    def backward(ctx, grad_color, grad_radii, grad_depth, grad_alpha):
        rs = ctx.raster_settings
        P, Cn = ctx.P, ctx.Cn
        if P == 0:
            return (None,) * 14
        lib = _lib.lib()
        H, W = int(rs.image_height), int(rs.image_width)
        scratch = None
        if ctx.tiny:
            (m3, shs, cols, opac, scl, rot, cov, bg, view, proj, campos, radii, alpha) = ctx.saved_tensors
            dev = m3.device
            e = lambda *sh: torch.empty(*sh, dtype=torch.float32, device=dev)
            scratch = (e(Cn, H, W), e(1, H, W), e(1, H, W), torch.empty(P, dtype=torch.int32, device=dev))
            a = _fwd_args(rs, P, Cn, m3, shs, cols, opac, scl, rot, cov, bg, view, proj, campos, *scratch, None, 1)
            geom, image, point_list, sorted_rec, quad_list, D = _streaming_render(a, dev, lib, False)
            ctx.num_rendered = D
            PASS_STATS["tiny_rerendered_for_backward"] += 1
        else:
            (m3, shs, cols, opac, scl, rot, cov, bg, view, proj, campos, radii, alpha, geom, image,
             point_list, sorted_rec, quad_list) = ctx.saved_tensors
        dev = m3.device
        need = ctx.needs_input_grad
        z = lambda *s: torch.empty(*s, dtype=torch.float32, device=dev)

        g_m3 = z(P, 3) if need[0] else None
        g_m2 = z(P, 3) if need[1] else None
        sink = ctx.sh_rgb_sink if (need[2] and shs is not None) else None
        g_sh = z(*shs.shape) if (need[2] and shs is not None and sink is None) else None
        g_sh_rgb = z(P, 3) if sink is not None else None
        g_col = z(*cols.shape) if (need[3] and cols is not None) else None
        g_op = z(P, 1) if need[4] else None
        g_scl = z(P, 3) if (need[5] and scl is not None) else None
        g_rot = z(P, 4) if (need[6] and rot is not None) else None
        g_cov = z(P, 6) if (need[7] and cov is not None) else None

        gc = _f32c(grad_color)
        if gc is None:
            gc = torch.zeros(*((ctx.num_groups,) if ctx.num_groups > 1 else ()), Cn, H, W, dtype=torch.float32, device=dev)
        gd = _f32c(grad_depth)
        ga = _f32c(grad_alpha)
        bwd_tmp = torch.empty(int(lib.ogs_raster_backward_tmp_bytes(P)), dtype=torch.uint8, device=dev)

        b = OgsRasterBwdArgs()
        b.P, b.W, b.H, b.C = P, W, H, Cn
        b.sh_degree = int(rs.sh_degree)
        b.sh_coeffs = 0 if shs is None else int(shs.shape[1])
        b.tanfovx, b.tanfovy, b.scale_modifier = float(rs.tanfovx), float(rs.tanfovy), float(rs.scale_modifier)
        b.debug = int(bool(rs.debug))
        b.num_rendered = int(ctx.num_rendered)
        b.geom_channels = int(ctx.geom_channels)
        b.num_groups = int(ctx.num_groups)
        b.sorted_rec, b.quad_list = ptr(sorted_rec), ptr(quad_list)
        b.bg, b.means3D, b.colors_precomp, b.shs, b.opacities = ptr(bg), ptr(m3), ptr(cols), ptr(shs), ptr(opac)
        b.scales, b.rotations, b.cov3D_precomp = ptr(scl), ptr(rot), ptr(cov)
        b.viewmatrix, b.projmatrix, b.campos = ptr(view), ptr(proj), ptr(campos)
        b.radii, b.out_alpha = ptr(radii), ptr(alpha)
        b.dL_dcolor, b.dL_ddepth, b.dL_dalpha = ptr(gc), ptr(gd), ptr(ga)
        b.geom_buffer, b.image_buffer, b.point_list, b.bwd_tmp = ptr(geom), ptr(image), ptr(point_list), ptr(bwd_tmp)
        b.dL_dmeans2D, b.dL_dcolors, b.dL_dopacity, b.dL_dmeans3D = ptr(g_m2), ptr(g_col), ptr(g_op), ptr(g_m3)
        b.dL_dcov3D, b.dL_dsh, b.dL_dscales, b.dL_drotations = ptr(g_cov), ptr(g_sh), ptr(g_scl), ptr(g_rot)
        b.dL_dsh_rgb = ptr(g_sh_rgb)
        check(lib.ogs_raster_backward(C.byref(b), _stream()), "ogs_raster_backward")
        scratch = None
        if _DEBUG_KEEP_BWD_TMP is not None:
            _DEBUG_KEEP_BWD_TMP.append(bwd_tmp)
        if sink is not None:
            sink.append(g_sh_rgb)
        return g_m3, g_m2, g_sh, g_col, g_op, g_scl, g_rot, g_cov, None, None, None, None, None, None


class _KeptPass:
    __slots__ = ("key", "generation", "holds", "P", "W", "H", "Cn", "E", "fused", "D", "image", "sorted_rec", "quad_list", "radii",
                 "nbytes", "hits", "full_binning")


class KeptPasses:

    def __init__(self, budget_bytes=None):
        self.budget_bytes = budget_bytes
        self.slots: dict = {}
        self.nbytes = 0
        self.stats = {"hits": 0, "misses": 0, "stale": 0, "admitted": 0, "rejected_budget": 0, "dropped_old_generation": 0,
                      "rejected_out_of_memory": 0}

    def _budget(self, dev) -> int:
        if self.budget_bytes is None:
            env = os.environ.get("OGS_KEPT_PASSES_GB")
            if env is not None:
                self.budget_bytes = int(float(env) * (1 << 30))
            else:
                free, total = torch.cuda.mem_get_info(dev)
                self.budget_bytes = int(min(total // 4, free // 2))
        return self.budget_bytes

    def enabled(self, dev) -> bool:
        return self._budget(dev) > 0

    def lookup(self, slot, key):
        e = self.slots.get(slot)
        if e is None:
            self.stats["misses"] += 1
            return None
        if e.key != key:
            self.drop(slot)
            self.stats["stale"] += 1
            self.stats["misses"] += 1
            return None
        e.hits += 1
        self.stats["hits"] += 1
        return e

    def drop(self, slot):
        e = self.slots.pop(slot, None)
        if e is not None:
            self.nbytes -= e.nbytes

    def clear(self):
        self.slots.clear()
        self.nbytes = 0

    def admit(self, slot, key, holds, kept: dict, generation=None) -> bool:
        dev = kept["image"].device
        lib = _lib.lib()
        W, H, Cn = kept["W"], kept["H"], kept["Cn"]
        tiles = ((W + 15) // 16) * ((H + 15) // 16)
        image = kept["image"]
        up = lambda n: (n + 255) // 256 * 256
        o_cnt = up(tiles * 8) + up(W * H * 4)
        packed = image[o_cnt:o_cnt + tiles * 20].view(torch.int32).view(tiles, 5)[:, 4].to(torch.int64)
        ends = torch.cumsum(packed, 0)
        used = int(ends[-1].item())
        if used <= 0:
            return False
        srb, qlb = int(lib.ogs_raster_sorted_bytes(used, Cn)), int(lib.ogs_raster_quad_list_bytes(used))
        nbytes = srb + qlb + image.numel() + kept["radii"].numel() * 4
        if self.nbytes + nbytes > self._budget(dev) and generation is not None:
            for old_slot in [sl for sl, en in self.slots.items() if en.generation != generation]:
                self.drop(old_slot)
                self.stats["dropped_old_generation"] += 1
        if self.nbytes + nbytes > self._budget(dev):
            self.stats["rejected_budget"] += 1
            return False
        e = _KeptPass()
        e.key, e.holds, e.generation = key, holds, generation
        e.P, e.W, e.H, e.Cn, e.fused, e.D = kept["P"], W, H, Cn, bool(kept["fused"]), used
        e.E = Cn - 3 if e.fused else Cn
        e.full_binning = kept["full_binning"]
        e.radii = kept["radii"]
        try:
            e.image = image.clone()
            new_ranges = torch.stack((ends - packed, ends), 1).to(torch.int32).contiguous()
            e.image[: tiles * 8] = new_ranges.view(-1).view(torch.uint8)
            e.sorted_rec = torch.empty(srb, dtype=torch.uint8, device=dev)
            e.quad_list = torch.empty(qlb, dtype=torch.uint8, device=dev)
        except torch.cuda.OutOfMemoryError:
            self.stats["rejected_out_of_memory"] += 1
            return False
        check(lib.ogs_raster_compact_kept(W, H, Cn, ptr(image), ptr(kept["sorted_rec"]), ptr(kept["quad_list"]), ptr(e.image),
                                          ptr(e.sorted_rec), ptr(e.quad_list), _stream()), "ogs_raster_compact_kept")
        e.nbytes, e.hits = nbytes, 0
        self.drop(slot)
        self.slots[slot] = e
        self.nbytes += nbytes
        self.stats["admitted"] += 1
        return True


KEPT_PASSES = KeptPasses()


class KeptImages:

    def __init__(self, budget_bytes=None):
        self.budget_bytes = budget_bytes
        self.slots: dict = {}
        self.nbytes = 0
        self.stats = {"hits": 0, "misses": 0, "stale": 0, "admitted": 0, "rejected_budget": 0}

    def _budget(self, dev) -> int:
        return KEPT_PASSES._budget(dev) if self.budget_bytes is None else self.budget_bytes

    def lookup(self, slot, key):
        e = self.slots.get(slot)
        if e is None or e[0] != key:
            if e is not None:
                self.drop(slot)
                self.stats["stale"] += 1
            self.stats["misses"] += 1
            return None
        self.stats["hits"] += 1
        return tuple(t.clone() for t in e[3])

    def drop(self, slot):
        e = self.slots.pop(slot, None)
        if e is not None:
            self.nbytes -= e[4]

    def clear(self):
        self.slots.clear()
        self.nbytes = 0

    def admit(self, slot, key, holds, outputs, generation=None) -> bool:
        dev = outputs[0].device
        nbytes = sum(t.numel() * t.element_size() for t in outputs)
        if self.nbytes + nbytes > self._budget(dev) and generation is not None:
            for old_slot in [sl for sl, en in self.slots.items() if en[1] != generation]:
                self.drop(old_slot)
        if self.nbytes + nbytes > self._budget(dev):
            self.stats["rejected_budget"] += 1
            return False
        try:
            kept = tuple(t.detach().clone() for t in outputs)
        except torch.cuda.OutOfMemoryError:
            return False
        self.drop(slot)
        self.slots[slot] = (key, generation, holds, kept, nbytes)
        self.nbytes += nbytes
        self.stats["admitted"] += 1
        return True


KEPT_IMAGES = KeptImages()


def clear_kept():
    KEPT_PASSES.clear()
    KEPT_IMAGES.clear()


class _ReblendKept(torch.autograd.Function):

    @staticmethod
    def forward(ctx, extra_feats, entry: _KeptPass, raster_settings: GaussianRasterizationSettings):
        rs = raster_settings
        ctx.set_materialize_grads(False)
        _require_gpu(extra_feats, "colors_precomp")
        dev = extra_feats.device
        lib = _lib.lib()
        P, W, H, Cn = entry.P, entry.W, entry.H, entry.Cn
        cols = _f32c(extra_feats)
        if cols is None or tuple(cols.shape) != (P, entry.E):
            raise RuntimeError(f"the kept pass blends {entry.E} caller channels of {P} Gaussians, got {tuple(extra_feats.shape)}")
        bg = _f32c(rs.bg.to(dev))
        if bg is None or bg.numel() != Cn:
            if bg is not None and bg.numel() == 3 and Cn > 3:
                bg = _tiled_bg(bg, Cn)
            else:
                raise RuntimeError(f"bg must have {Cn} entries")
        color = torch.empty(Cn, H, W, dtype=torch.float32, device=dev)
        depth = torch.empty(1, H, W, dtype=torch.float32, device=dev)
        alpha = torch.empty(1, H, W, dtype=torch.float32, device=dev)
        a = OgsRasterFwdArgs()
        a.P, a.W, a.H, a.C = P, W, H, Cn
        a.sh_coeffs = 1 if entry.fused else 0
        a.debug = int(bool(rs.debug))
        a.bg, a.colors_precomp = ptr(bg), ptr(cols)
        a.out_color, a.out_depth, a.out_alpha = ptr(color), ptr(depth), ptr(alpha)
        a.image_buffer, a.sorted_rec, a.quad_list = ptr(entry.image), ptr(entry.sorted_rec), ptr(entry.quad_list)
        check(lib.ogs_raster_forward_reblend(C.byref(a), _stream()), "ogs_raster_forward_reblend")
        PASS_STATS["reblend"] += 1
        ctx.entry, ctx.raster_settings = entry, rs
        ctx.save_for_backward(cols)
        radii = entry.radii.detach()
        ctx.mark_non_differentiable(radii)
        return color, radii, depth, alpha

    @staticmethod
    def backward(ctx, grad_color, grad_radii, grad_depth, grad_alpha):
        if not ctx.needs_input_grad[0]:
            return None, None, None
        e, rs = ctx.entry, ctx.raster_settings
        (cols,) = ctx.saved_tensors
        dev = cols.device
        lib = _lib.lib()
        gc = _f32c(grad_color)
        if gc is None:
            return torch.zeros_like(cols), None, None
        g_col = torch.empty(e.P, e.E, dtype=torch.float32, device=dev)
        bwd_tmp = torch.empty(int(lib.ogs_raster_backward_tmp_bytes(e.P)), dtype=torch.uint8, device=dev)
        b = OgsRasterBwdArgs()
        b.P, b.W, b.H, b.C = e.P, e.W, e.H, e.Cn
        b.debug = int(bool(rs.debug))
        b.num_rendered, b.num_groups = int(e.D), 1
        b.colors_precomp = ptr(cols)
        b.shs = ptr(cols) if e.fused else None
        b.radii, b.dL_dcolor = ptr(e.radii), ptr(gc)
        b.image_buffer, b.sorted_rec, b.quad_list, b.bwd_tmp = ptr(e.image), ptr(e.sorted_rec), ptr(e.quad_list), ptr(bwd_tmp)
        b.dL_dcolors = ptr(g_col)
        check(lib.ogs_raster_backward(C.byref(b), _stream()), "ogs_raster_backward")
        return g_col, None, None


def rasterize_gaussians(means3D, means2D, sh, colors_precomp, opacities, scales, rotations, cov3Ds_precomp,
                        raster_settings, sh_rgb_sink=None):
    return _RasterizeGaussians.apply(means3D, means2D, sh, colors_precomp, opacities, scales, rotations,
                                     cov3Ds_precomp, raster_settings, 0, sh_rgb_sink)


def rasterize_fused(means3D, means2D, opacities, shs, extra_feats, raster_settings, scales=None, rotations=None,
                    cov3D_precomp=None, detach_extra_from_geometry=True, sh_rgb_sink=None, frozen_key=None):
    empty = torch.Tensor([])
    args = (means3D, means2D, shs, extra_feats, opacities, empty if scales is None else scales,
            empty if rotations is None else rotations, empty if cov3D_precomp is None else cov3D_precomp, raster_settings,
            3 if detach_extra_from_geometry else 0, sh_rgb_sink)
    if frozen_key is None or not means3D.is_cuda or not KEPT_PASSES.enabled(means3D.device) or raster_settings.debug or \
            (torch.is_grad_enabled() and any(t is not None and t.requires_grad for t in
                                             (means3D, means2D, opacities, shs, scales, rotations, cov3D_precomp))):
        return _RasterizeGaussians.apply(*args)
    slot, key, holds = frozen_key[:3]
    generation = frozen_key[3] if len(frozen_key) > 3 else None
    key = (key, bool(FULL_BINNING), int(extra_feats.shape[-1]))
    entry = KEPT_PASSES.lookup(slot, key)
    if entry is not None:
        return _ReblendKept.apply(extra_feats, entry, raster_settings)
    sink: list = []
    out = _RasterizeGaussians.apply(*args, None, 1, sink)
    if sink:
        KEPT_PASSES.admit(slot, key, holds, sink[0], generation)
    return out


def rasterize_groups(means3D, means2D, opacities, group_ids, num_groups, raster_settings, shs=None,
                     colors_precomp=None, scales=None, rotations=None, cov3D_precomp=None):
    empty = torch.Tensor([])
    if (shs is None) == (colors_precomp is None):
        raise Exception('Please provide excatly one of either SHs or precomputed colors!')
    return _RasterizeGaussians.apply(means3D, means2D, empty if shs is None else shs,
                                     empty if colors_precomp is None else colors_precomp, opacities,
                                     empty if scales is None else scales, empty if rotations is None else rotations,
                                     empty if cov3D_precomp is None else cov3D_precomp, raster_settings, 0, None,
                                     group_ids, int(num_groups))


def _stats_inputs(means3D, opacities, raster_settings, colors_precomp, scales, rotations, cov3D_precomp):
    if torch.is_grad_enabled() and any(t is not None and t.requires_grad
                                       for t in (means3D, opacities, colors_precomp, scales, rotations, cov3D_precomp)):
        raise RuntimeError("statistics / preprocess-only passes have no backward: detach the inputs or use torch.no_grad()")
    _require_gpu(means3D, "means3D")
    if means3D.dim() != 2 or means3D.shape[1] != 3:
        raise RuntimeError("means3D must have dimensions (num_points, 3)")
    if (scales is None) != (rotations is None) or (scales is None) == (cov3D_precomp is None):
        raise RuntimeError("provide exactly one of (scales, rotations) / cov3D_precomp")
    dev = means3D.device
    cols = _f32c(colors_precomp)
    if cols is None or cols.dim() != 2 or cols.shape[0] != means3D.shape[0]:
        if means3D.shape[0] != 0:
            raise RuntimeError("colors_precomp must be [P, C]")
    Cn = int(colors_precomp.shape[-1])
    if Cn not in SUPPORTED_CHANNELS:
        raise RuntimeError(f"the blended channel count must be 3, 6, 9 or 12, got {Cn}")
    rs = raster_settings
    bg = _f32c(rs.bg.to(dev))
    if bg is None or bg.numel() != Cn:
        if bg is not None and bg.numel() == 3 and Cn > 3:
            bg = _tiled_bg(bg, Cn)
        else:
            raise RuntimeError(f"bg must have {Cn} entries")
    return (Cn, _f32c(means3D), _f32c(opacities), cols, _f32c(scales), _f32c(rotations), _f32c(cov3D_precomp), bg,
            _f32c(rs.viewmatrix.to(dev)), _f32c(rs.projmatrix.to(dev)), _f32c(rs.campos.to(dev)))


def visible_radii(means3D, opacities, raster_settings, colors_precomp, scales=None, rotations=None, cov3D_precomp=None):
    Cn, m3, opac, cols, scl, rot, cov, bg, view, proj, campos = _stats_inputs(
        means3D, opacities, raster_settings, colors_precomp, scales, rotations, cov3D_precomp)
    P = int(means3D.shape[0])
    dev = means3D.device
    radii = torch.zeros(P, dtype=torch.int32, device=dev)
    if P == 0:
        return radii
    lib = _lib.lib()
    a = _fwd_args(raster_settings, P, Cn, m3, None, cols, opac, scl, rot, cov, bg, view, proj, campos, None, None, None,
                  radii, None, 1)
    gb, gtb, _ = _geom_sizes(P, int(a.W), int(a.H), Cn, 1)
    geom = torch.empty(gb, dtype=torch.uint8, device=dev)
    geom_tmp = torch.empty(gtb, dtype=torch.uint8, device=dev)
    a.geom_buffer, a.geom_tmp = ptr(geom), ptr(geom_tmp)
    check(lib.ogs_raster_forward_geometry(C.byref(a), _stream(), None), "ogs_raster_forward_geometry")
    return radii


def rasterize_group_stats(means3D, opacities, group_ids, num_groups, labels, num_labels, raster_settings, colors_precomp,
                          scales=None, rotations=None, cov3D_precomp=None, alpha_threshold=0.5):
    Cn, m3, opac, cols, scl, rot, cov, bg, view, proj, campos = _stats_inputs(
        means3D, opacities, raster_settings, colors_precomp, scales, rotations, cov3D_precomp)
    rs = raster_settings
    G, L = int(num_groups), int(num_labels)
    if G < 0 or L < 0:
        raise RuntimeError(f"num_groups ({G}) and num_labels ({L}) must be >= 0")
    H, W = int(rs.image_height), int(rs.image_width)
    dev = means3D.device
    P = int(means3D.shape[0])
    if labels.numel() != H * W:
        raise RuntimeError(f"labels must have H*W = {H * W} entries, got {tuple(labels.shape)}")
    lab = labels.to(device=dev, dtype=torch.int32).contiguous()
    max_alpha = torch.zeros(G, dtype=torch.float32, device=dev)
    count = torch.zeros(G, L + 1, dtype=torch.int64, device=dev)
    feat_sum = torch.zeros(G, L + 1, Cn, dtype=torch.float32, device=dev)
    radii = torch.zeros(P, dtype=torch.int32, device=dev)
    if G == 0:
        return max_alpha, count, feat_sum, radii
    gid = group_ids.to(device=dev, dtype=torch.int32).contiguous()
    if gid.numel() != P:
        raise RuntimeError("group_ids must be [P]")
    sub = None
    if G == 1:
        sub = gid == 0
        idx = lambda t: None if t is None else t[sub].contiguous()
        m3, opac, cols, scl, rot, cov = idx(m3), idx(opac), idx(cols), idx(scl), idx(rot), idx(cov)
        P_pass, gid_pass = int(m3.shape[0]), None
        sub_radii = torch.zeros(P_pass, dtype=torch.int32, device=dev)
    else:
        P_pass, gid_pass, sub_radii = P, gid, radii
    lib = _lib.lib()
    a = _fwd_args(rs, P_pass, Cn, m3, None, cols, opac, scl, rot, cov, bg, view, proj, campos, None, None, None, sub_radii,
                  gid_pass, G)
    if P_pass == 0:
        a.colors_precomp = a.scales = a.rotations = ptr(bg)
        a.cov3D_precomp = None
    u8 = lambda n: torch.empty(int(n), dtype=torch.uint8, device=dev)
    stream = _stream()
    keep = []
    D = 0
    if P_pass > 0:
        gb, gtb, _ = _geom_sizes(P_pass, W, H, Cn, 1)
        keep += [u8(gb), u8(gtb)]
        a.geom_buffer, a.geom_tmp = ptr(keep[0]), ptr(keep[1])
        n = C.c_int64(0)
        PASS_STATS["blocking"] += 1
        check(lib.ogs_raster_forward_geometry(C.byref(a), stream, C.byref(n)), "ogs_raster_forward_geometry")
        D = int(n.value)
    image = u8(lib.ogs_raster_stats_image_bytes(W, H, G))
    tmp = u8(lib.ogs_raster_stats_tmp_bytes(G, L, Cn))
    a.image_buffer = ptr(image)
    if D > 0:
        btb, _, _ = _render_sizes(D, W, H, Cn)
        pl, bt = torch.empty(D, dtype=torch.int32, device=dev), u8(btb)
        keep += [pl, bt]
        a.point_list, a.binning_tmp = ptr(pl), ptr(bt)
    st = _lib.OgsGroupStatsArgs()
    st.labels, st.num_labels, st.alpha_threshold = ptr(lab), L, float(alpha_threshold)
    st.max_alpha, st.count, st.feat_sum, st.stats_tmp = ptr(max_alpha), ptr(count), ptr(feat_sum), ptr(tmp)
    check(lib.ogs_raster_forward_group_stats(C.byref(a), C.byref(st), D, stream), "ogs_raster_forward_group_stats")
    if sub is not None:
        radii[sub] = sub_radii
    return max_alpha, count, feat_sum, radii


class GaussianRasterizer(nn.Module):
    def __init__(self, raster_settings: GaussianRasterizationSettings):
        super().__init__()
        self.raster_settings = raster_settings

    def markVisible(self, positions: torch.Tensor) -> torch.Tensor:
        _require_gpu(positions, "positions")
        rs = self.raster_settings
        with torch.no_grad():
            pos = _f32c(positions)
            P = 0 if pos is None else int(pos.shape[0])
            out = torch.zeros(P, dtype=torch.uint8, device=positions.device)
            if P:
                view = _f32c(rs.viewmatrix.to(positions.device))
                proj = _f32c(rs.projmatrix.to(positions.device))
                check(_lib.lib().ogs_mark_visible(P, ptr(pos), ptr(view), ptr(proj), ptr(out), _stream()),
                      "ogs_mark_visible")
        return out.bool()

    def forward(self, means3D, means2D, opacities, shs=None, colors_precomp=None, scales=None, rotations=None,
                cov3D_precomp=None):
        rs = self.raster_settings
        if (shs is None and colors_precomp is None) or (shs is not None and colors_precomp is not None):
            raise Exception('Please provide excatly one of either SHs or precomputed colors!')
        if ((scales is None or rotations is None) and cov3D_precomp is None) or \
                ((scales is not None or rotations is not None) and cov3D_precomp is not None):
            raise Exception('Please provide exactly one of either scale/rotation pair or precomputed 3D covariance!')
        empty = torch.Tensor([])
        shs = empty if shs is None else shs
        colors_precomp = empty if colors_precomp is None else colors_precomp
        scales = empty if scales is None else scales
        rotations = empty if rotations is None else rotations
        cov3D_precomp = empty if cov3D_precomp is None else cov3D_precomp
        return rasterize_gaussians(means3D, means2D, shs, colors_precomp, opacities, scales, rotations,
                                   cov3D_precomp, rs)
```

Measured before the change: 1445 Mpix/s.

## Zero backward grad buffer inside forward blend and replace offsets scan with block sums

The backward gradient-record buffer is now allocated during forward and zeroed by the tail of the forward blend kernel, which lets backward skip its memset. In the per-tile depth-order path without full binning, preprocess computes per-block sums of touched tiles and a single-block kernel scans them. The duplicate kernel then derives per-element offsets with an in-block wave scan, so the device-wide exclusive scan is no longer needed. The cost is holding the buffer across forward and backward, an extra store workload at the end of blending, and a serial single-block scan over about 4K entries.

```diff
diff --git a/include/ogs_raster.h b/include/ogs_raster.h
--- a/include/ogs_raster.h
+++ b/include/ogs_raster.h
@@ -53,6 +53,8 @@
     const int32_t* group_ids;
     int32_t num_groups;
     int32_t full_binning;
+    void* bwd_clear;
+    size_t bwd_clear_bytes;
 } OgsRasterFwdArgs;
 
 typedef struct OgsRasterBwdArgs {
@@ -93,6 +95,7 @@
     float* dL_drotations;
     int32_t num_groups;
     float* dL_dsh_rgb;
+    int32_t bwd_tmp_is_clear;
 } OgsRasterBwdArgs;
 
 int ogs_version(void);
diff --git a/opengaussian_amd/_lib.py b/opengaussian_amd/_lib.py
--- a/opengaussian_amd/_lib.py
+++ b/opengaussian_amd/_lib.py
@@ -23,6 +23,7 @@
         ("geom_buffer", _vp), ("geom_tmp", _vp), ("image_buffer", _vp), ("point_list", _vp),
         ("binning_tmp", _vp), ("sorted_rec", _vp), ("quad_list", _vp), ("group_ids", _vp), ("num_groups", C.c_int32),
         ("full_binning", C.c_int32),
+        ("bwd_clear", _vp), ("bwd_clear_bytes", C.c_size_t),
     ]
 
 
@@ -39,6 +40,7 @@
         ("geom_buffer", _vp), ("image_buffer", _vp), ("point_list", _vp), ("sorted_rec", _vp), ("quad_list", _vp), ("bwd_tmp", _vp),
         ("dL_dmeans2D", _vp), ("dL_dcolors", _vp), ("dL_dopacity", _vp), ("dL_dmeans3D", _vp),
         ("dL_dcov3D", _vp), ("dL_dsh", _vp), ("dL_dscales", _vp), ("dL_drotations", _vp), ("num_groups", C.c_int32), ("dL_dsh_rgb", _vp),
+        ("bwd_tmp_is_clear", C.c_int32),
     ]
 
 
diff --git a/opengaussian_amd/csrc/blend_fwd.hip b/opengaussian_amd/csrc/blend_fwd.hip
--- a/opengaussian_amd/csrc/blend_fwd.hip
+++ b/opengaussian_amd/csrc/blend_fwd.hip
@@ -306,7 +306,7 @@
     float4* __restrict__ stream, uint32_t* __restrict__ quad_list, uint32_t* __restrict__ qcount, int W, int H, int gx, int tiles,
     const float* __restrict__ bg, float* __restrict__ out_color, float* __restrict__ out_depth, float* __restrict__ out_alpha,
     uint32_t* __restrict__ n_contrib, float* __restrict__ final_T, const uint32_t* __restrict__ tile_order,
-    GroupStatsOut st = GroupStatsOut{}) {
+    uint4* __restrict__ clear, unsigned long long clear_units, GroupStatsOut st = GroupStatsOut{}) {
     constexpr int NV = rec_vec4(C);
     constexpr int SV = stream_vec4(C);
     constexpr int kListLen = kRowListLen;
@@ -539,6 +539,11 @@
             n_contrib[pix] = last;
             final_T[pix] = T;
         }
+        if (clear != nullptr) {
+            const unsigned long long per = (clear_units + gridDim.x - 1) / gridDim.x;
+            const unsigned long long u0 = min(clear_units, (unsigned long long)blockIdx.x * per), u1 = min(clear_units, u0 + per);
+            for (unsigned long long u = u0 + (unsigned)tid; u < u1; u += kBlock) clear[u] = uint4{0u, 0u, 0u, 0u};
+        }
     }
 }
 
@@ -773,6 +778,8 @@
     const int gx = (a.W + kTile - 1) / kTile, gy = (a.H + kTile - 1) / kTile;
     const int tiles = gx * gy;
     const unsigned vtiles = (unsigned)tiles * (unsigned)num_groups_of(a.num_groups);
+    const bool host_clear = a.bwd_clear != nullptr && D > 0 && per_tile_depth_order(a);
+    if (a.bwd_clear != nullptr && !host_clear) OGS_HIP_CHECK(hipMemsetAsync(a.bwd_clear, 0, a.bwd_clear_bytes, s));
     if (D > 0) {
         const uint32_t* order = order_ready ? tile_order_of(is, vtiles, a.P) : launch_tile_order(is, vtiles, a.P, s, a.debug);
         static constexpr const char* const kChunked[4] = {"pack_blend_chunked_kernel<3>", "pack_blend_chunked_kernel<6>",
@@ -780,7 +787,8 @@
         OGS_LAUNCH_NAMED(chan_name<C>(kChunked), pack_blend_chunked_kernel<C>, dim3(vtiles), dim3(kBlock), 0, s,
                          (const uint2*)is.ranges, (const uint32_t*)a.point_list, (const float4*)gs.rec, stream_base<C>(a.sorted_rec),
                          quad_base(a.quad_list), is.qcount, a.W, a.H, gx, tiles, a.bg, a.out_color, a.out_depth, a.out_alpha,
-                         is.n_contrib, is.final_T, order);
+                         is.n_contrib, is.final_T, order, host_clear ? static_cast<uint4*>(a.bwd_clear) : (uint4*)nullptr,
+                         (unsigned long long)(a.bwd_clear_bytes / 16));
         OGS_LAUNCH_CHECK(a.debug, s);
         return OGS_OK;
     }
@@ -820,7 +828,7 @@
     OGS_LAUNCH_NAMED(chan_name<C>(kStats), (pack_blend_chunked_kernel<C, true>), dim3(vtiles), dim3(kBlock), 0, s,
                      (const uint2*)is.ranges, (const uint32_t*)a.point_list, (const float4*)gs.rec, (float4*)nullptr,
                      (uint32_t*)nullptr, (uint32_t*)nullptr, a.W, a.H, gx, tiles, a.bg, (float*)nullptr, (float*)nullptr,
-                     (float*)nullptr, (uint32_t*)nullptr, (float*)nullptr, order, st);
+                     (float*)nullptr, (uint32_t*)nullptr, (float*)nullptr, order, (uint4*)nullptr, 0ull, st);
     OGS_LAUNCH_CHECK(a.debug, s);
     const size_t n = rows * C;
     OGS_LAUNCH(group_stats_finish_kernel, dim3((unsigned)((n + 255) / 256)), dim3(256), 0, s, (const long long*)fixed,
diff --git a/opengaussian_amd/csrc/capi.hip b/opengaussian_amd/csrc/capi.hip
--- a/opengaussian_amd/csrc/capi.hip
+++ b/opengaussian_amd/csrc/capi.hip
@@ -143,7 +143,7 @@
 
 extern "C" {
 
-int ogs_version(void) { return 403; }
+int ogs_version(void) { return 404; }
 
 int ogs_check_async_status(void) { return check_async_status("ogs_check_async_status"); }
 
@@ -220,7 +220,8 @@
     } else if (per_tile_depth_order(*a)) {
         rc = launch_preprocess(*a, gs, gt, s);
         if (rc != OGS_OK) return rc;
-        rc = exclusive_scan_u32(gt.tiles_touched, nullptr, gt.offsets, a->P, gt.num_rendered, gt.sort_tmp, s, a->debug);
+        rc = block_sum_offsets(*a) ? launch_block_offsets(*a, gt, s)
+                                   : exclusive_scan_u32(gt.tiles_touched, nullptr, gt.offsets, a->P, gt.num_rendered, gt.sort_tmp, s, a->debug);
         if (rc != OGS_OK) return rc;
     } else {
         rc = launch_preprocess(*a, gs, gt, s);
@@ -267,6 +268,9 @@
     int rc = validate_fwd(a, stats == nullptr);
     if (rc != OGS_OK) return rc;
     if (!a->image_buffer) { set_error("image_buffer == NULL"); return OGS_ERR_INVALID_ARG; }
+    if (a->bwd_clear && !stats && (((uintptr_t)a->bwd_clear | a->bwd_clear_bytes) & 15u) != 0) {
+        set_error("bwd_clear / bwd_clear_bytes must be multiples of 16"); return OGS_ERR_INVALID_ARG;
+    }
     const int G = num_groups_of(a->num_groups);
     const ImageState is = stats ? ImageState::carve_stats(a->image_buffer, a->W, a->H, G)
                                 : ImageState::carve(a->image_buffer, a->W, a->H, G);
@@ -431,7 +435,7 @@
     const ImageState is = ImageState::carve(const_cast<void*>(a->image_buffer), a->W, a->H, num_groups_of(a->num_groups));
     void* grad_rec = a->bwd_tmp;
     const int rec_doubles = feat_only ? feat_grad_stride(a->C, a->shs ? 3 : 0) : grad_stride(a->C);
-    OGS_HIP_CHECK(hipMemsetAsync(grad_rec, 0, (size_t)a->P * rec_doubles * sizeof(double), s));
+    if (!a->bwd_tmp_is_clear) OGS_HIP_CHECK(hipMemsetAsync(grad_rec, 0, (size_t)a->P * rec_doubles * sizeof(double), s));
     if (a->num_rendered > 0 && (!a->sorted_rec || !a->quad_list)) { set_error("backward: sorted_rec / quad_list == NULL"); return OGS_ERR_INVALID_ARG; }
     int rc = launch_blend_backward(*a, is, grad_rec, s);
     if (rc != OGS_OK) return rc;
diff --git a/opengaussian_amd/csrc/ogs_common.h b/opengaussian_amd/csrc/ogs_common.h
--- a/opengaussian_amd/csrc/ogs_common.h
+++ b/opengaussian_amd/csrc/ogs_common.h
@@ -202,6 +202,7 @@
     uint32_t* offsets;
     uint32_t* num_rendered;
     void* sort_tmp;
+    uint32_t* block_sum;
     uint32_t* visible() const { return num_rendered + 1; }
     static GeomTmp carve(void* p, int P) {
         Carver c(p);
@@ -214,6 +215,7 @@
         g.offsets = c.take<uint32_t>(P);
         g.num_rendered = c.take<uint32_t>(64);
         g.sort_tmp = c.take<char>(sort_tmp_bytes(P));
+        g.block_sum = c.take<uint32_t>((size_t)(P + kBlock - 1) / kBlock);
         return g;
     }
     static size_t bytes(int P) {
@@ -221,6 +223,7 @@
         for (int i = 0; i < 6; ++i) c.take<uint32_t>(P);
         c.take<uint32_t>(64);
         c.take<char>(sort_tmp_bytes(P));
+        c.take<uint32_t>((size_t)(P + kBlock - 1) / kBlock);
         return c.off;
     }
 };
@@ -250,6 +253,7 @@
 };
 
 int launch_preprocess(const OgsRasterFwdArgs& a, const GeomState& gs, const GeomTmp& gt, hipStream_t s);
+int launch_block_offsets(const OgsRasterFwdArgs& a, const GeomTmp& gt, hipStream_t s);
 int launch_tiny_geometry(const OgsRasterFwdArgs& a, const GeomState& gs, uint32_t* order, hipStream_t s);
 int launch_small_geometry(const OgsRasterFwdArgs& a, const GeomState& gs, const GeomTmp& gt, hipStream_t s);
 int launch_tiny_blend(const OgsRasterFwdArgs& a, const GeomState& gs, const uint32_t* order, hipStream_t s);
@@ -262,6 +266,7 @@
 int launch_tile_ranges(const uint32_t* tile_keys_sorted, int64_t D, uint2* ranges, int64_t tiles, hipStream_t s,
                        int debug, const uint32_t* n_dev = nullptr, bool already_zeroed = false);
 inline bool per_tile_depth_order(const OgsRasterFwdArgs& a) { return a.num_groups <= 1 && a.P > kSmallMaxP; }
+inline bool block_sum_offsets(const OgsRasterFwdArgs& a) { return per_tile_depth_order(a) && a.full_binning == 0; }
 constexpr int kTileSortItems = 16;
 constexpr int kTileSortCap = kBlock * kTileSortItems;
 constexpr int kWaveSortCap = kTileSortCap / (kBlock / kWave);
diff --git a/opengaussian_amd/csrc/preprocess_fwd.hip b/opengaussian_amd/csrc/preprocess_fwd.hip
--- a/opengaussian_amd/csrc/preprocess_fwd.hip
+++ b/opengaussian_amd/csrc/preprocess_fwd.hip
@@ -87,7 +87,7 @@
     const float* __restrict__ rotations, const float* __restrict__ cov3D_precomp, const float* __restrict__ viewmatrix,
     const float* __restrict__ projmatrix, const float* __restrict__ campos, float4* __restrict__ rec_row,
     uint32_t* __restrict__ clamped_out, int32_t* __restrict__ radii, uint32_t* __restrict__ tiles_touched,
-    const int32_t* __restrict__ group_ids, int num_groups) {
+    const int32_t* __restrict__ group_ids, int num_groups, uint32_t* touched_ret = nullptr) {
     constexpr int NV = rec_vec4(C);
     float V[16], M[16];
 #pragma unroll
@@ -206,6 +206,7 @@
     clamped_out[idx] = clamped;
     radii[idx] = radius;
     if (tiles_touched) tiles_touched[idx] = touched;
+    if (touched_ret) *touched_ret = touched;
     return ok ? __float_as_uint(depth) : 0xFFFFFFFFu;
 }
 
@@ -218,19 +219,33 @@
     const float* __restrict__ projmatrix, const float* __restrict__ campos, float4* __restrict__ rec,
     uint32_t* __restrict__ clamped_out, int32_t* __restrict__ radii, uint32_t* __restrict__ tiles_touched,
     uint32_t* __restrict__ depth_keys, uint32_t* __restrict__ order, const int32_t* __restrict__ group_ids,
-    int num_groups) {
+    int num_groups, uint32_t* __restrict__ block_sum) {
     constexpr int NV = rec_vec4(C);
     __shared__ float4 s_rec[kBlock * NV];
+    __shared__ uint32_t s_wave_sum[kBlock / kWave];
     const int tid = threadIdx.x;
     const int idx = blockIdx.x * kBlock + tid;
+    uint32_t touched = 0;
     if (idx < P) {
         depth_keys[idx] = preprocess_one<C>(idx, W, H, sh_degree, sh_coeffs, tanfovx, tanfovy, focal_x, focal_y, scale_modifier,
                                             means3D, colors_precomp, shs, opacities, scales, rotations, cov3D_precomp, viewmatrix,
                                             projmatrix, campos, s_rec + tid * NV, clamped_out, radii, tiles_touched, group_ids,
-                                            num_groups);
+                                            num_groups, &touched);
         if (order) order[idx] = (uint32_t)idx;
     }
+    if (block_sum != nullptr) {
+        uint32_t t = touched;
+#pragma unroll
+        for (int d = kWave / 2; d >= 1; d >>= 1) t += __shfl_down(t, d, kWave);
+        if ((tid & (kWave - 1)) == 0) s_wave_sum[tid / kWave] = t;
+    }
     __syncthreads();
+    if (block_sum != nullptr && tid == 0) {
+        uint32_t t = 0;
+#pragma unroll
+        for (int w = 0; w < kBlock / kWave; ++w) t += s_wave_sum[w];
+        block_sum[blockIdx.x] = t;
+    }
     const size_t row0 = (size_t)blockIdx.x * kBlock;
     const int n4 = min(kBlock, P - (int)row0) * NV;
     float4* __restrict__ out = rec + row0 * NV;
@@ -323,10 +338,13 @@
                                                            const float4* __restrict__ rec,
                                                            const uint32_t* __restrict__ order,
                                                            const uint32_t* __restrict__ offsets,
+                                                           const uint32_t* __restrict__ tiles_touched,
+                                                           const uint32_t* __restrict__ block_base,
                                                            uint32_t* __restrict__ tile_keys,
                                                            uint32_t* __restrict__ vals, uint32_t capacity,
                                                            const int32_t* __restrict__ group_ids, bool drop_unreachable,
                                                            uint2* __restrict__ zero_ranges, int n_zero) {
+    __shared__ uint32_t s_wave_sum[kBlock / kWave];
     __shared__ uint32_t s_off[kBlock];
     __shared__ uint32_t s_gid[kBlock];
     __shared__ uint32_t s_rect[kBlock];
@@ -340,12 +358,14 @@
     const int P = n_visible ? min(P_cap, (int)*n_visible) : P_cap;
     if ((int)blockIdx.x * kBlock >= P) return;
     const int gx = (W + kTile - 1) / kTile, gy = (H + kTile - 1) / kTile;
-    uint32_t off = 0, cnt = 0, gid = 0, rect = 1u << 24, key0 = 0;
+    uint32_t off = 0, cnt = 0, gid = 0, rect = 1u << 24, key0 = 0, touched = 0;
     float4 ctr = make_float4(0.f, 0.f, 0.f, 0.f);
     float4 con = make_float4(1.f, 1.f, 0.f, 0.f);
+    int wide_x0 = 0, wide_x1 = 0, wide_y0 = 0, wide_y1 = 0;
     if (r < P) {
         gid = order ? order[r] : (uint32_t)r;
-        off = offsets[r];
+        if (block_base != nullptr) touched = tiles_touched[r];
+        else off = offsets[r];
         if (group_ids != nullptr) key0 = (uint32_t)max(group_ids[gid], 0) * (uint32_t)(gx * gy);
         const float4 a = rec[(size_t)gid * NV];
         const int radius = __float_as_int(a.w);
@@ -367,22 +387,42 @@
             if (w > 0 && h > 0) {
                 cnt = (uint32_t)(w * h);
                 rect = (uint32_t)rminx | ((uint32_t)rminy << 12) | ((uint32_t)min(w, 255) << 24);
-                if (w > 255) {
-                    uint32_t o = off;
-                    for (int ty = rminy; ty < rmaxy; ++ty)
-                        for (int tx = rminx; tx < rmaxx; ++tx) {
-                            if (o < capacity) { tile_keys[o] = key0 + (uint32_t)(ty * gx + tx); vals[o] = gid | (1u << kReachBit); }
-                            ++o;
-                        }
-                    rect |= 0u;
-                    gid |= 0x80000000u;
-                }
+                if (w > 255) { wide_x0 = rminx; wide_x1 = rmaxx; wide_y0 = rminy; wide_y1 = rmaxy; }
             }
         }
     }
-    if (tid == 0) s_first = off;
+    uint32_t before = 0;
+    if (block_base != nullptr) {
+        const int lane = tid & (kWave - 1);
+        uint32_t incl = touched;
+#pragma unroll
+        for (int d = 1; d < kWave; d <<= 1) {
+            const uint32_t o = __shfl_up(incl, d, kWave);
+            if (lane >= d) incl += o;
+        }
+        if (lane == kWave - 1) s_wave_sum[tid / kWave] = incl;
+        before = incl - touched;
+        if (tid == 0) s_first = block_base[blockIdx.x];
+    } else if (tid == 0) {
+        s_first = off;
+    }
     __syncthreads();
     const uint32_t first = s_first;
+    if (block_base != nullptr) {
+#pragma unroll
+        for (int w = 0; w < kBlock / kWave; ++w)
+            if (w < tid / kWave) before += s_wave_sum[w];
+        off = first + before;
+    }
+    if (wide_x1 > wide_x0) {
+        uint32_t o = off;
+        for (int ty = wide_y0; ty < wide_y1; ++ty)
+            for (int tx = wide_x0; tx < wide_x1; ++tx) {
+                if (o < capacity) { tile_keys[o] = key0 + (uint32_t)(ty * gx + tx); vals[o] = gid | (1u << kReachBit); }
+                ++o;
+            }
+        gid |= 0x80000000u;
+    }
     s_off[tid] = (r < P) ? off - first : 0xFFFFFFFFu;
     s_gid[tid] = gid;
     s_rect[tid] = rect;
@@ -421,6 +461,51 @@
     }
 }
 
+constexpr int kOffsThreads = 1024, kOffsItems = 8, kOffsChunk = kOffsThreads * kOffsItems;
+__global__ __launch_bounds__(kOffsThreads) void block_offsets_kernel(uint32_t* __restrict__ block_sum, int nb,
+                                                                     uint32_t* __restrict__ total_out) {
+    __shared__ uint32_t s_val[kOffsChunk];
+    __shared__ uint32_t s_wave_sum[kOffsThreads / kWave];
+    const int tid = threadIdx.x, lane = tid & (kWave - 1), wave = tid / kWave;
+    uint32_t carry = 0;
+    for (int c0 = 0; c0 < nb; c0 += kOffsChunk) {
+        const int n = min(kOffsChunk, nb - c0);
+#pragma unroll
+        for (int k = 0; k < kOffsItems; ++k) {
+            const int e = k * kOffsThreads + tid;
+            s_val[e] = e < n ? block_sum[c0 + e] : 0u;
+        }
+        __syncthreads();
+        uint32_t v[kOffsItems], sum = 0;
+#pragma unroll
+        for (int k = 0; k < kOffsItems; ++k) { v[k] = s_val[tid * kOffsItems + k]; sum += v[k]; }
+        uint32_t incl = sum;
+#pragma unroll
+        for (int d = 1; d < kWave; d <<= 1) {
+            const uint32_t o = __shfl_up(incl, d, kWave);
+            if (lane >= d) incl += o;
+        }
+        if (lane == kWave - 1) s_wave_sum[wave] = incl;
+        __syncthreads();
+        uint32_t run = carry + incl - sum, total = 0;
+#pragma unroll
+        for (int w = 0; w < kOffsThreads / kWave; ++w) {
+            const uint32_t t = s_wave_sum[w];
+            if (w < wave) run += t;
+            total += t;
+        }
+#pragma unroll
+        for (int k = 0; k < kOffsItems; ++k) {
+            const int e = tid * kOffsItems + k;
+            if (e < n) block_sum[c0 + e] = run;
+            run += v[k];
+        }
+        carry += total;
+        __syncthreads();
+    }
+    if (tid == 0) total_out[0] = carry;
+}
+
 __global__ __launch_bounds__(kBlock) void mark_visible_kernel(int P, const float* __restrict__ means3D,
                                                               const float* __restrict__ V,
                                                               uint8_t* __restrict__ present) {
@@ -441,7 +526,8 @@
                        a.tanfovx, a.tanfovy, focal_x, focal_y, a.scale_modifier, a.means3D, a.colors_precomp, a.shs,
                        a.opacities, a.scales, a.rotations, a.cov3D_precomp, a.viewmatrix, a.projmatrix, a.campos,
                        gs.rec, gs.clamped, a.radii, gt.tiles_touched, gt.keys[0],
-                       per_tile_depth_order(a) ? (uint32_t*)nullptr : gt.order[0], a.num_groups > 1 ? a.group_ids : (const int32_t*)nullptr, a.num_groups);
+                       per_tile_depth_order(a) ? (uint32_t*)nullptr : gt.order[0], a.num_groups > 1 ? a.group_ids : (const int32_t*)nullptr, a.num_groups,
+                       block_sum_offsets(a) ? gt.block_sum : (uint32_t*)nullptr);
     OGS_LAUNCH_CHECK(a.debug, s);
     return OGS_OK;
 }
@@ -501,9 +587,16 @@
     }
 }
 
+int launch_block_offsets(const OgsRasterFwdArgs& a, const GeomTmp& gt, hipStream_t s) {
+    OGS_LAUNCH(block_offsets_kernel, dim3(1), dim3(kOffsThreads), 0, s, gt.block_sum, (a.P + kBlock - 1) / kBlock, gt.num_rendered);
+    OGS_LAUNCH_CHECK(a.debug, s);
+    return OGS_OK;
+}
+
 int launch_duplicate(const OgsRasterFwdArgs& a, const GeomState& gs, const GeomTmp& gt, uint32_t* tile_keys,
                      uint32_t* vals, uint32_t capacity, bool drop_unreachable, bool depth_order, hipStream_t s, uint2* zero_ranges,
                      int n_zero) {
+    const uint32_t* base = (!depth_order && block_sum_offsets(a)) ? gt.block_sum : nullptr;
     if (n_zero > a.P) { set_error("duplicate: %d ranges to clear with %d threads", n_zero, a.P); return OGS_ERR_INVALID_ARG; }
     const int grid = (a.P + kBlock - 1) / kBlock;
     const int32_t* grp = a.num_groups > 1 ? a.group_ids : nullptr;
@@ -514,9 +607,9 @@
     const uint32_t* order = depth_order ? gt.order[0] : nullptr;
     const uint32_t* n_visible = depth_order ? gt.visible() : nullptr;
     switch (rec_vec4(a.C)) {
-        case 3: OGS_LAUNCH(duplicate_kernel<3>, dim3(grid), dim3(kBlock), 0, s, a.P, n_visible, a.W, a.H, gs.rec, order, gt.offsets, tile_keys, vals, capacity, grp, drop_unreachable, zero_ranges, n_zero); break;
-        case 4: OGS_LAUNCH(duplicate_kernel<4>, dim3(grid), dim3(kBlock), 0, s, a.P, n_visible, a.W, a.H, gs.rec, order, gt.offsets, tile_keys, vals, capacity, grp, drop_unreachable, zero_ranges, n_zero); break;
-        case 5: OGS_LAUNCH(duplicate_kernel<5>, dim3(grid), dim3(kBlock), 0, s, a.P, n_visible, a.W, a.H, gs.rec, order, gt.offsets, tile_keys, vals, capacity, grp, drop_unreachable, zero_ranges, n_zero); break;
+        case 3: OGS_LAUNCH(duplicate_kernel<3>, dim3(grid), dim3(kBlock), 0, s, a.P, n_visible, a.W, a.H, gs.rec, order, gt.offsets, gt.tiles_touched, base, tile_keys, vals, capacity, grp, drop_unreachable, zero_ranges, n_zero); break;
+        case 4: OGS_LAUNCH(duplicate_kernel<4>, dim3(grid), dim3(kBlock), 0, s, a.P, n_visible, a.W, a.H, gs.rec, order, gt.offsets, gt.tiles_touched, base, tile_keys, vals, capacity, grp, drop_unreachable, zero_ranges, n_zero); break;
+        case 5: OGS_LAUNCH(duplicate_kernel<5>, dim3(grid), dim3(kBlock), 0, s, a.P, n_visible, a.W, a.H, gs.rec, order, gt.offsets, gt.tiles_touched, base, tile_keys, vals, capacity, grp, drop_unreachable, zero_ranges, n_zero); break;
         default: set_error("unsupported record size"); return OGS_ERR_UNSUPPORTED;
     }
     OGS_LAUNCH_CHECK(a.debug, s);
diff --git a/opengaussian_amd/rasterizer.py b/opengaussian_amd/rasterizer.py
--- a/opengaussian_amd/rasterizer.py
+++ b/opengaussian_amd/rasterizer.py
@@ -130,6 +130,18 @@
         global FULL_BINNING
         FULL_BINNING = self._prev
         return False
+
+
+HOST_BWD_CLEAR = True
+
+
+def _grad_record_bytes(need, P, Cn, shs, cols, scl, rot, cov) -> int:
+    want_cols = bool(need[3]) and cols is not None
+    other = (need[0] or need[1] or (need[2] and shs is not None) or need[4] or (need[5] and scl is not None)
+             or (need[6] and rot is not None) or (need[7] and cov is not None))
+    feat_only = want_cols and not other
+    feat_sums = Cn - (3 if shs is not None else 0)
+    return P * (64 if (feat_only and feat_sums <= 8) else 128)
 
 
 def _fwd_args(rs, P, Cn, m3, shs, cols, opac, scl, rot, cov, bg, view, proj, campos, color, depth, alpha, radii, group_ids, G):
@@ -265,6 +277,7 @@
         radii = alloc(P, dtype=torch.int32, device=dev)
         ctx.raster_settings = rs
         ctx.P, ctx.Cn, ctx.num_rendered, ctx.tiny = P, Cn, 0, False
+        ctx.bwd_tmp, ctx.bwd_clear_bytes = None, 0
         ctx.full_binning = bool(FULL_BINNING)
         if P == 0:
             ctx.save_for_backward()
@@ -285,8 +298,14 @@
             ctx.mark_non_differentiable(radii)
             return color, radii, depth, alpha
 
+        need = ctx.needs_input_grad
+        if HOST_BWD_CLEAR and G == 1 and not rs.debug and any(need[:8]):
+            bwd_tmp = torch.empty(int(lib.ogs_raster_backward_tmp_bytes(P)), dtype=torch.uint8, device=dev)
+            a.bwd_clear, a.bwd_clear_bytes = ptr(bwd_tmp), _grad_record_bytes(need, P, Cn, shs, cols, scl, rot, cov)
         geom, image, point_list, sorted_rec, quad_list, D = _streaming_render(a, dev, lib, rs.debug)
         ctx.num_rendered = D
+        if a.bwd_clear:
+            ctx.bwd_tmp, ctx.bwd_clear_bytes = bwd_tmp, int(a.bwd_clear_bytes)
         ctx.save_for_backward(m3, shs, cols, opac, scl, rot, cov, bg, view, proj, campos, radii, alpha, geom, image,
                               point_list, sorted_rec, quad_list)
         ctx.mark_non_differentiable(radii)
@@ -337,9 +356,15 @@
             gc = torch.zeros(*((ctx.num_groups,) if ctx.num_groups > 1 else ()), Cn, H, W, dtype=torch.float32, device=dev)
         gd = _f32c(grad_depth)
         ga = _f32c(grad_alpha)
-        bwd_tmp = torch.empty(int(lib.ogs_raster_backward_tmp_bytes(P)), dtype=torch.uint8, device=dev)
+        bwd_tmp, is_clear = ctx.bwd_tmp, False
+        if bwd_tmp is not None:
+            is_clear = ctx.bwd_clear_bytes >= _grad_record_bytes(need, P, Cn, shs, cols, scl, rot, cov)
+            ctx.bwd_tmp, ctx.bwd_clear_bytes = None, 0
+        else:
+            bwd_tmp = torch.empty(int(lib.ogs_raster_backward_tmp_bytes(P)), dtype=torch.uint8, device=dev)
 
         b = OgsRasterBwdArgs()
+        b.bwd_tmp_is_clear = int(is_clear)
         b.P, b.W, b.H, b.C = P, W, H, Cn
         b.sh_degree = int(rs.sh_degree)
         b.sh_coeffs = 0 if shs is None else int(shs.shape[1])
```

Measured after the change: 1463 Mpix/s, median of 6. +1.2%, better.
